# mythos-bio/mythos

Hardware: AMD Instinct MI355X
Metric: MD steps/sec (and ns/day) per GPU, oxDNA2 12 kbp duplex (higher is better)
Workload: dtype f32; 1 GPU; oxDNA2 12000 bp duplex (24000 nt), Debye-Hueckel salt 0.5, Langevin dt 0.005, free space, 1 replica/GPU; half_charged_ends=True, replicas=1, repeats=1, warmup_steps_done=10205, precision=headline f32 (north_star: fp32 at 1e-3); the other precision: --full, full=False

## Files before the change

### include/mythos_hip.h

```cpp
#ifndef MYTHOS_HIP_H
#define MYTHOS_HIP_H

#include <stdint.h>

#ifdef __cplusplus
extern "C" {
#endif

typedef struct mythos_system mythos_system_t;
typedef struct mythos_sim mythos_sim_t;
typedef struct mythos_martini mythos_martini_t;
typedef struct mythos_martini_sim mythos_martini_sim_t;
typedef struct mythos_obs mythos_obs_t;
typedef void* mythos_stream_t;

enum mythos_status {
  MYTHOS_OK = 0,
  MYTHOS_ERR_INVALID_ARGUMENT = -1,
  MYTHOS_ERR_HIP = -2,
  MYTHOS_ERR_NO_DEVICE = -3,
  MYTHOS_ERR_NOT_READY = -4,
  MYTHOS_ERR_OVERFLOW = -5,
  MYTHOS_ERR_NUMERIC = -6
};

enum mythos_dtype { MYTHOS_F32 = 0, MYTHOS_F64 = 1 };

#define MYTHOS_OXDNA_N_TERMS 8

const char* mythos_version(void);
const char* mythos_last_error(void);
int mythos_device_count(void);

int mythos_oxdna_param_count(void);
const char* mythos_oxdna_param_name(int index);

mythos_system_t* mythos_oxdna_create(int model, int n, const int32_t* seq, const uint8_t* is_end, int n_bonded,
                                     const int32_t* bonded, const double* box, int dtype, int device);
void mythos_oxdna_destroy(mythos_system_t* sys);

int mythos_oxdna_set_params(mythos_system_t* sys, const double* flat_params, int n_params);

int mythos_oxdna_set_nucleotide_types(mythos_system_t* sys, const uint8_t* is_rna);

int mythos_oxdna_set_pseq(mythos_system_t* sys, const double* marginals, const int32_t* unit, int n_bp,
                          const double* bp_probs, int terms);

int mythos_oxdna_energy_dpseq(mythos_system_t* sys, const void* center, const void* quat, int n_frames, double* e_terms,
                              void* dU_dcenter, void* dU_dquat, double* dU_dparams, double* dU_dmarginals, double* dU_dbp,
                              mythos_stream_t stream);

int mythos_oxdna_set_neighbors(mythos_system_t* sys, const int32_t* pairs, int n_pairs);

int mythos_oxdna_build_neighbors(mythos_system_t* sys, const void* center, double r_cut, double skin,
                                 mythos_stream_t stream);
int mythos_oxdna_neighbor_stats(mythos_system_t* sys, int* max_row, double* mean_row);

int mythos_oxdna_energy(mythos_system_t* sys, const void* center, const void* quat, int n_frames, double* e_terms,
                        void* dU_dcenter, void* dU_dquat, double* dU_dparams, mythos_stream_t stream);

mythos_obs_t* mythos_observables_create(int model, int n, const double* geometry, const double* box, int n_bp,
                                        const int32_t* base_pairs, int n_quartets, const int32_t* quartets, int skip_ends,
                                        int dtype, int device);
void mythos_observables_destroy(mythos_obs_t* obs);
int mythos_observables_width(const mythos_obs_t* obs);
int mythos_observables_eval(mythos_obs_t* obs, const void* center, const void* quat, int n_frames, double* out,
                            mythos_stream_t stream);
int mythos_oxdna_energy_obs(mythos_system_t* sys, const void* center, const void* quat, int n_frames, double* e_terms,
                            void* dU_dcenter, void* dU_dquat, double* dU_dparams, mythos_obs_t* obs, double* obs_out,
                            mythos_stream_t stream);

mythos_sim_t* mythos_langevin_create(mythos_system_t* sys, double dt, double kT, double gamma_t, double gamma_r,
                                     double mass, const double* inertia, uint64_t seed);
void mythos_langevin_destroy(mythos_sim_t* sim);

int mythos_langevin_set_neighbor_policy(mythos_sim_t* sim, double r_cut, double skin, int every);

int mythos_langevin_init_momenta(mythos_sim_t* sim, void* p_lin, void* p_ang, mythos_stream_t stream);

int mythos_langevin_run(mythos_sim_t* sim, void* center, void* quat, void* p_lin, void* p_ang, int n_steps,
                        int save_every, void* traj_center, void* traj_quat, double* e_trace,
                        mythos_stream_t stream);
int mythos_langevin_load(mythos_sim_t* sim, const void* center, const void* quat, const void* p_lin, const void* p_ang,
                         mythos_stream_t stream);
int mythos_langevin_advance(mythos_sim_t* sim, int n_steps, int save_every, void* traj_center, void* traj_quat,
                            double* e_trace, mythos_stream_t stream);
int mythos_langevin_store(mythos_sim_t* sim, void* center, void* quat, void* p_lin, void* p_ang, mythos_stream_t stream);

int64_t mythos_langevin_get_step(const mythos_sim_t* sim);
int mythos_langevin_set_step(mythos_sim_t* sim, int64_t step);
int mythos_langevin_set_seed(mythos_sim_t* sim, uint64_t seed);

enum mythos_langevin_option { MYTHOS_LANGEVIN_UNFUSED = 0 };
int mythos_langevin_set_option(mythos_sim_t* sim, int option, int64_t value);

int mythos_langevin_set_timing(mythos_sim_t* sim, int samples);
int mythos_langevin_last_kernel_ms(const mythos_sim_t* sim, double* kernel_ms, double* loop_ms_per_launch,
                                   int* launches, int* samples);

int mythos_langevin_last_recoveries(const mythos_sim_t* sim, int* recoveries);
int mythos_langevin_last_rebuilds(const mythos_sim_t* sim, int* scheduled);

int mythos_oxdna_read_trajectory(const char* path, int n, int max_frames, double* times, double* box, double* energies,
                                 double* frames, int* n_frames);

int mythos_oxdna_write_trajectory(const char* path, int n, int n_frames, const double* times, const double* box,
                                  const double* energies, const double* frames, int append);

enum mythos_debug_key {
  MYTHOS_DEBUG_CELL_BUCKET_CAP = 0,
  MYTHOS_DEBUG_ENERGY_LIST_CAP = 1,
  MYTHOS_DEBUG_MD_SEGMENT = 2,
  MYTHOS_DEBUG_MD_OVERFLOW_AT = 3,
  MYTHOS_DEBUG_MD_DENSE = 4,
  MYTHOS_DEBUG_MD_ITEMS_BIG = 5,
  MYTHOS_DEBUG_MD_LANES = 6,
  MYTHOS_DEBUG_KEYS = 7
};
int mythos_debug_set(int key, int64_t value);
int64_t mythos_debug_get(int key);

#define MYTHOS_MARTINI_N_TERMS 3
mythos_martini_t* mythos_martini_create(int n, const int32_t* types, int n_types, const double* sigma,
                                        const double* eps, int n_bonds, const int32_t* bonds, const double* bond_k,
                                        const double* bond_r0, int n_angles, const int32_t* angles,
                                        const double* angle_k, const double* angle_t0, int angle_kind, double r_cut,
                                        int dtype, int device);
void mythos_martini_destroy(mythos_martini_t* m);
int mythos_martini_energy(mythos_martini_t* m, const void* pos, const void* box, int n_frames, double* e_terms,
                          void* dU_dpos, mythos_stream_t stream);

int mythos_martini_param_grads(mythos_martini_t* m, const void* pos, const void* box, int n_frames, double* d_sigma,
                               double* d_eps, double* d_bond_k, double* d_bond_r0, double* d_angle_k,
                               double* d_angle_t0, mythos_stream_t stream);

mythos_martini_sim_t* mythos_martini_langevin_create(mythos_martini_t* sys, double dt, double kT, double gamma,
                                                     const double* mass, uint64_t seed);
void mythos_martini_langevin_destroy(mythos_martini_sim_t* sim);
int mythos_martini_langevin_set_neighbor_policy(mythos_martini_sim_t* sim, double skin, int rebuild_every);
int mythos_martini_langevin_set_inner_list(mythos_martini_sim_t* sim, double margin, int every);
int mythos_martini_langevin_init_velocities(mythos_martini_sim_t* sim, void* vel, mythos_stream_t stream);
int mythos_martini_langevin_run(mythos_martini_sim_t* sim, void* pos, void* vel, const double* box, int n_steps,
                                int save_every, void* traj_pos, double* e_trace, mythos_stream_t stream);
int mythos_martini_langevin_load(mythos_martini_sim_t* sim, const void* pos, const void* vel, const double* box,
                                 mythos_stream_t stream);
int mythos_martini_langevin_advance(mythos_martini_sim_t* sim, int n_steps, int save_every, void* traj_pos, double* e_trace,
                                    mythos_stream_t stream);
int mythos_martini_langevin_store(mythos_martini_sim_t* sim, void* pos, void* vel, mythos_stream_t stream);
int64_t mythos_martini_langevin_get_step(const mythos_martini_sim_t* sim);
int mythos_martini_langevin_last_rebuilds(const mythos_martini_sim_t* sim, int* scheduled);
int mythos_martini_langevin_last_kernel_ms(const mythos_martini_sim_t* sim, double* kernel_ms,
                                           double* loop_ms_per_launch, int* launches, int* samples);
int mythos_martini_langevin_set_timing(mythos_martini_sim_t* sim, int samples);
int mythos_martini_langevin_last_recoveries(const mythos_martini_sim_t* sim, int* recoveries);
int mythos_martini_langevin_neighbor_stats(const mythos_martini_sim_t* sim, int* max_row, double* mean_row);
int mythos_martini_langevin_get_rows(const mythos_martini_sim_t* sim, int which, int32_t* rows, int32_t* row_len, int* stride);

typedef struct mythos_martini_obs mythos_martini_obs_t;
mythos_martini_obs_t* mythos_martini_obs_create(int n, int n_groups, const int32_t* beads_per_item, const int32_t* members,
                                                const int32_t* index, int device);
void mythos_martini_obs_destroy(mythos_martini_obs_t* obs);
int64_t mythos_martini_obs_count(const mythos_martini_obs_t* obs);
int mythos_martini_obs_eval(mythos_martini_obs_t* obs, const void* pos, const void* box, int dtype, int n_frames, double* out,
                            mythos_stream_t stream);

typedef struct mythos_w1_plan mythos_w1_plan_t;
mythos_w1_plan_t* mythos_w1_plan_create(int n_groups, const int32_t* n_frames, const int32_t* members, const double* samples,
                                        const int64_t* n_ref, const double* ref, const double* ref_weights,
                                        const uint8_t* has_ref_weights, const int64_t* order, int device,
                                        mythos_stream_t stream);
void mythos_w1_plan_destroy(mythos_w1_plan_t* plan);
int mythos_w1_eval(mythos_w1_plan_t* plan, const double* weights, double* w1, double* dw1_dweights, mythos_stream_t stream);

#define MYTHOS_MEMBRANE_ROW 7
typedef struct mythos_membrane mythos_membrane_t;
mythos_membrane_t* mythos_membrane_create(int n, int n_lipids, const int32_t* lipid_start, const int32_t* lipid_beads, int n_thick,
                                          const int32_t* thick_beads, const int32_t* thick_lipid, int device);
void mythos_membrane_destroy(mythos_membrane_t* mem);
int mythos_membrane_n_lipids(const mythos_membrane_t* mem);
int mythos_membrane_eval(mythos_membrane_t* mem, const void* pos, const void* box, int dtype, int n_frames, double* out,
                         int8_t* leaflets, mythos_stream_t stream);

#ifdef __cplusplus
}
#endif
#endif
```

### mythos_amd/_lib.py

```python

from __future__ import annotations

import ctypes as C
import os
from pathlib import Path

_LIB_PATH = Path(__file__).resolve().parent / "lib" / "libmythos_hip.so"

c_int_p = C.POINTER(C.c_int32)
c_double_p = C.POINTER(C.c_double)
c_uint8_p = C.POINTER(C.c_uint8)


class MythosHipError(RuntimeError):
    """An error reported by libmythos_hip.so."""


_lib = None


def lib_path() -> Path:
    return Path(os.environ.get("MYTHOS_HIP_LIB", _LIB_PATH))


def load() -> C.CDLL:
    global _lib
    if _lib is not None:
        return _lib
    path = lib_path()
    if not path.exists():
        raise MythosHipError(
            f"{path} not found: the HIP extension is not built (run __graft_entry__.build()). "
            "mythos_amd has no CPU fallback."
        )
    lib = C.CDLL(str(path))
    V = C.c_void_p
    sigs = {
        "mythos_version": (C.c_char_p, []),
        "mythos_last_error": (C.c_char_p, []),
        "mythos_device_count": (C.c_int, []),
        "mythos_debug_set": (C.c_int, [C.c_int, C.c_int64]),
        "mythos_debug_get": (C.c_int64, [C.c_int]),
        "mythos_oxdna_param_count": (C.c_int, []),
        "mythos_oxdna_param_name": (C.c_char_p, [C.c_int]),
        "mythos_oxdna_create": (V, [C.c_int, C.c_int, c_int_p, c_uint8_p, C.c_int, c_int_p, c_double_p, C.c_int, C.c_int]),
        "mythos_oxdna_destroy": (None, [V]),
        "mythos_oxdna_set_params": (C.c_int, [V, c_double_p, C.c_int]),
        "mythos_oxdna_set_pseq": (C.c_int, [V, c_double_p, c_int_p, C.c_int, c_double_p, C.c_int]),
        "mythos_oxdna_set_nucleotide_types": (C.c_int, [V, c_uint8_p]),
        "mythos_oxdna_set_neighbors": (C.c_int, [V, c_int_p, C.c_int]),
        "mythos_oxdna_build_neighbors": (C.c_int, [V, V, C.c_double, C.c_double, V]),
        "mythos_oxdna_neighbor_stats": (C.c_int, [V, C.POINTER(C.c_int), c_double_p]),
        "mythos_oxdna_energy": (C.c_int, [V, V, V, C.c_int, V, V, V, V, V]),
        "mythos_oxdna_energy_obs": (C.c_int, [V, V, V, C.c_int, V, V, V, V, V, V, V]),
        "mythos_oxdna_energy_dpseq": (C.c_int, [V, V, V, C.c_int, V, V, V, V, V, V, V]),
        "mythos_observables_create": (V, [C.c_int, C.c_int, c_double_p, c_double_p, C.c_int, c_int_p, C.c_int, c_int_p, C.c_int, C.c_int, C.c_int]),
        "mythos_observables_destroy": (None, [V]),
        "mythos_observables_width": (C.c_int, [V]),
        "mythos_observables_eval": (C.c_int, [V, V, V, C.c_int, V, V]),
        "mythos_langevin_create": (V, [V, C.c_double, C.c_double, C.c_double, C.c_double, C.c_double, c_double_p, C.c_uint64]),
        "mythos_langevin_destroy": (None, [V]),
        "mythos_langevin_set_neighbor_policy": (C.c_int, [V, C.c_double, C.c_double, C.c_int]),
        "mythos_langevin_init_momenta": (C.c_int, [V, V, V, V]),
        "mythos_langevin_run": (C.c_int, [V, V, V, V, V, C.c_int, C.c_int, V, V, V, V]),
        "mythos_langevin_load": (C.c_int, [V, V, V, V, V, V]),
        "mythos_langevin_advance": (C.c_int, [V, C.c_int, C.c_int, V, V, V, V]),
        "mythos_langevin_store": (C.c_int, [V, V, V, V, V, V]),
        "mythos_langevin_get_step": (C.c_int64, [V]),
        "mythos_langevin_set_step": (C.c_int, [V, C.c_int64]),
        "mythos_langevin_set_seed": (C.c_int, [V, C.c_uint64]),
        "mythos_langevin_last_kernel_ms": (C.c_int, [V, c_double_p, c_double_p, C.POINTER(C.c_int), C.POINTER(C.c_int)]),
        "mythos_langevin_set_option": (C.c_int, [V, C.c_int, C.c_int64]),
        "mythos_langevin_set_timing": (C.c_int, [V, C.c_int]),
        "mythos_martini_langevin_set_timing": (C.c_int, [V, C.c_int]),
        "mythos_langevin_last_recoveries": (C.c_int, [V, C.POINTER(C.c_int)]),
        "mythos_langevin_last_rebuilds": (C.c_int, [V, C.POINTER(C.c_int)]),
        "mythos_oxdna_read_trajectory": (C.c_int, [C.c_char_p, C.c_int, C.c_int, c_double_p, c_double_p, c_double_p, c_double_p, C.POINTER(C.c_int)]),
        "mythos_oxdna_write_trajectory": (C.c_int, [C.c_char_p, C.c_int, C.c_int, c_double_p, c_double_p, c_double_p, c_double_p, C.c_int]),
        "mythos_martini_create": (
            V,
            [C.c_int, c_int_p, C.c_int, c_double_p, c_double_p, C.c_int, c_int_p, c_double_p, c_double_p, C.c_int,
             c_int_p, c_double_p, c_double_p, C.c_int, C.c_double, C.c_int, C.c_int],
        ),
        "mythos_martini_destroy": (None, [V]),
        "mythos_martini_energy": (C.c_int, [V, V, V, C.c_int, V, V, V]),
        "mythos_martini_param_grads": (C.c_int, [V, V, V, C.c_int, V, V, V, V, V, V, V]),
        "mythos_martini_langevin_create": (V, [V, C.c_double, C.c_double, C.c_double, c_double_p, C.c_uint64]),
        "mythos_martini_langevin_destroy": (None, [V]),
        "mythos_martini_langevin_set_neighbor_policy": (C.c_int, [V, C.c_double, C.c_int]),
        "mythos_martini_langevin_set_inner_list": (C.c_int, [V, C.c_double, C.c_int]),
        "mythos_martini_langevin_init_velocities": (C.c_int, [V, V, V]),
        "mythos_martini_langevin_run": (C.c_int, [V, V, V, c_double_p, C.c_int, C.c_int, V, V, V]),
        "mythos_martini_langevin_load": (C.c_int, [V, V, V, c_double_p, V]),
        "mythos_martini_langevin_advance": (C.c_int, [V, C.c_int, C.c_int, V, V, V]),
        "mythos_martini_langevin_store": (C.c_int, [V, V, V, V]),
        "mythos_martini_langevin_get_step": (C.c_int64, [V]),
        "mythos_martini_langevin_last_rebuilds": (C.c_int, [V, C.POINTER(C.c_int)]),
        "mythos_martini_langevin_last_kernel_ms": (C.c_int, [V, c_double_p, c_double_p, C.POINTER(C.c_int), C.POINTER(C.c_int)]),
        "mythos_martini_langevin_last_recoveries": (C.c_int, [V, C.POINTER(C.c_int)]),
        "mythos_martini_langevin_neighbor_stats": (C.c_int, [V, C.POINTER(C.c_int), c_double_p]),
        "mythos_martini_langevin_get_rows": (C.c_int, [V, C.c_int, C.POINTER(C.c_int32), C.POINTER(C.c_int32), C.POINTER(C.c_int)]),
        "mythos_martini_obs_create": (V, [C.c_int, C.c_int, c_int_p, c_int_p, c_int_p, C.c_int]),
        "mythos_martini_obs_destroy": (None, [V]),
        "mythos_martini_obs_count": (C.c_int64, [V]),
        "mythos_martini_obs_eval": (C.c_int, [V, V, V, C.c_int, C.c_int, V, V]),
        "mythos_w1_plan_create": (V, [C.c_int, c_int_p, c_int_p, V, C.POINTER(C.c_int64), V, V, c_uint8_p, V, C.c_int, V]),
        "mythos_w1_plan_destroy": (None, [V]),
        "mythos_w1_eval": (C.c_int, [V, V, V, V, V]),
        "mythos_membrane_create": (V, [C.c_int, C.c_int, c_int_p, c_int_p, C.c_int, c_int_p, c_int_p, C.c_int]),
        "mythos_membrane_destroy": (None, [V]),
        "mythos_membrane_n_lipids": (C.c_int, [V]),
        "mythos_membrane_eval": (C.c_int, [V, V, V, C.c_int, C.c_int, V, V, V]),
    }
    for name, (res, args) in sigs.items():
        fn = getattr(lib, name)
        fn.restype = res
        fn.argtypes = args
    _lib = lib
    return lib


DECLARED_SYMBOLS = (
    "mythos_version",
    "mythos_last_error",
    "mythos_device_count",
    "mythos_debug_set",
    "mythos_debug_get",
    "mythos_oxdna_param_count",
    "mythos_oxdna_param_name",
    "mythos_oxdna_create",
    "mythos_oxdna_destroy",
    "mythos_oxdna_set_params",
    "mythos_oxdna_set_pseq",
    "mythos_oxdna_set_nucleotide_types",
    "mythos_oxdna_set_neighbors",
    "mythos_oxdna_build_neighbors",
    "mythos_oxdna_neighbor_stats",
    "mythos_oxdna_energy",
    "mythos_oxdna_energy_obs",
    "mythos_oxdna_energy_dpseq",
    "mythos_observables_create",
    "mythos_observables_destroy",
    "mythos_observables_width",
    "mythos_observables_eval",
    "mythos_langevin_create",
    "mythos_langevin_destroy",
    "mythos_langevin_set_neighbor_policy",
    "mythos_langevin_init_momenta",
    "mythos_langevin_run",
    "mythos_langevin_load",
    "mythos_langevin_advance",
    "mythos_langevin_store",
    "mythos_langevin_get_step",
    "mythos_langevin_set_step",
    "mythos_langevin_set_seed",
    "mythos_langevin_last_kernel_ms",
    "mythos_langevin_last_recoveries",
    "mythos_langevin_last_rebuilds",
    "mythos_langevin_set_option",
    "mythos_langevin_set_timing",
    "mythos_martini_langevin_set_timing",
    "mythos_oxdna_read_trajectory",
    "mythos_oxdna_write_trajectory",
    "mythos_martini_create",
    "mythos_martini_destroy",
    "mythos_martini_energy",
    "mythos_martini_param_grads",
    "mythos_martini_langevin_create",
    "mythos_martini_langevin_destroy",
    "mythos_martini_langevin_set_neighbor_policy",
    "mythos_martini_langevin_set_inner_list",
    "mythos_martini_langevin_init_velocities",
    "mythos_martini_langevin_run",
    "mythos_martini_langevin_load",
    "mythos_martini_langevin_advance",
    "mythos_martini_langevin_store",
    "mythos_martini_langevin_get_step",
    "mythos_martini_langevin_last_rebuilds",
    "mythos_martini_langevin_last_kernel_ms",
    "mythos_martini_langevin_neighbor_stats",
    "mythos_martini_langevin_get_rows",
    "mythos_martini_langevin_last_recoveries",
    "mythos_martini_obs_create",
    "mythos_martini_obs_destroy",
    "mythos_martini_obs_count",
    "mythos_martini_obs_eval",
    "mythos_w1_plan_create",
    "mythos_w1_plan_destroy",
    "mythos_w1_eval",
    "mythos_membrane_create",
    "mythos_membrane_destroy",
    "mythos_membrane_n_lipids",
    "mythos_membrane_eval",
)


MEMBRANE_ROW = 7


def last_error() -> str:
    return load().mythos_last_error().decode()


def check(rc: int, what: str = "") -> None:
    if rc == 0:
        return
    msg = f"{what}: {last_error()} (status {rc})"
    if rc == -1:
        raise ValueError(msg)
    if rc == -6:
        raise FloatingPointError(msg)
    raise MythosHipError(msg)


DEBUG_KEYS = {"cell_bucket_cap": 0, "energy_list_cap": 1, "md_segment": 2, "md_overflow_at": 3, "md_dense": 4, "md_items_big": 5, "md_lanes": 6}


def debug_set(key: str, value: int) -> None:
    check(load().mythos_debug_set(DEBUG_KEYS[key], int(value)), f"debug_set({key})")


def debug_get(key: str) -> int:
    return int(load().mythos_debug_get(DEBUG_KEYS[key]))


_PARAM_NAMES: list[str] = []


def param_names() -> list[str]:
    if not _PARAM_NAMES:
        lib = load()
        _PARAM_NAMES.extend(lib.mythos_oxdna_param_name(i).decode() for i in range(lib.mythos_oxdna_param_count()))
    return list(_PARAM_NAMES)


def device_count() -> int:
    return int(load().mythos_device_count())


def ptr(t):
    if t is None:
        return None
    if hasattr(t, "data_ptr"):
        return C.c_void_p(t.data_ptr())
    return C.c_void_p(t.ctypes.data)
```

### mythos_amd/csrc/langevin.hip

```cpp
#include "langevin_core.inc"

MYTHOS_MD_DEFINE_PRECISION(float)

extern "C" {

mythos_sim_t* mythos_langevin_create(mythos_system_t* sys, double dt, double kT, double gamma_t, double gamma_r,
                                     double mass, const double* inertia, uint64_t seed) {
  if (!sys || !(dt > 0) || !(kT >= 0) || gamma_t < 0 || gamma_r < 0 || !(mass > 0)) {
    set_error("mythos_langevin_create: invalid argument");
    return nullptr;
  }
  if (hipSetDevice(sys->device) != hipSuccess) {
    set_error("mythos_langevin_create: hipSetDevice failed");
    return nullptr;
  }
  auto* s = new mythos_sim();
  s->sys = sys;
  s->dt = dt;
  s->kT = kT;
  s->gamma_t = gamma_t;
  s->gamma_r = gamma_r;
  s->mass = mass;
  for (int k = 0; k < 3; ++k) s->inertia[k] = inertia ? inertia[k] : 1.0;
  s->seed = seed;
  const size_t v4 = (sys->dtype == MYTHOS_F32 ? sizeof(float4) : sizeof(double4)) * (size_t)sys->n;
  bool ok = md_run_create(*s);
  for (int k = 0; k < 2; ++k)
    for (int a = 0; a < mythos_sim::kFrameArrays; ++a) ok = ok && hipMalloc(&s->frame[k][a], v4) == hipSuccess;
  ok = ok && hipMalloc(&s->keep_hi, v4) == hipSuccess && hipMalloc(&s->keep_lo, v4) == hipSuccess;
  ok = ok && hipMalloc((void**)&s->d_epart, (size_t)((sys->n + 15) / 16) * kTraceWidth * sizeof(double)) == hipSuccess;
  if (ok && !sys->d_ref_pos) ok = hipMalloc(&sys->d_ref_pos, v4) == hipSuccess;
  if (ok && !sys->d_ref_off) ok = hipMalloc(&sys->d_ref_off, v4) == hipSuccess;
  if (ok && !sys->d_ref_a1) ok = hipMalloc(&sys->d_ref_a1, v4) == hipSuccess;
  if (!ok) {
    set_error("mythos_langevin_create: device allocation failed");
    mythos_langevin_destroy(s);
    return nullptr;
  }
  return s;
}

void mythos_langevin_destroy(mythos_sim_t* s) {
  if (!s) return;
  for (int k = 0; k < 2; ++k)
    for (int a = 0; a < mythos_sim::kFrameArrays; ++a)
      if (s->frame[k][a]) (void)hipFree(s->frame[k][a]);
  for (void* u : {s->u_c, s->u_q, s->u_p, s->u_l, s->u_gc, s->u_gq, s->u_ref, (void*)s->u_e})
    if (u) (void)hipFree(u);
  if (s->keep_hi) (void)hipFree(s->keep_hi);
  if (s->keep_lo) (void)hipFree(s->keep_lo);
  if (s->d_chunk_order) (void)hipFree(s->d_chunk_order);
  if (s->d_chunk_keys) (void)hipFree(s->d_chunk_keys);
  if (s->d_epart) (void)hipFree(s->d_epart);
  md_run_destroy(*s);
  delete s;
}

int mythos_langevin_set_neighbor_policy(mythos_sim_t* s, double r_cut, double skin, int every) {
  if (!s || (every > 0 && (!(r_cut > 0) || !(skin > 0)))) {
    set_error("mythos_langevin_set_neighbor_policy: invalid argument");
    return MYTHOS_ERR_INVALID_ARGUMENT;
  }
  s->r_cut = r_cut;
  s->skin = skin;
  s->rebuild_every = every;
  s->list_fitted = false;
  s->list_valid = false;
  return MYTHOS_OK;
}

int mythos_langevin_init_momenta(mythos_sim_t* s, void* p_lin, void* p_ang, mythos_stream_t stream) {
  if (!s || !p_lin || !p_ang) {
    set_error("mythos_langevin_init_momenta: invalid argument");
    return MYTHOS_ERR_INVALID_ARGUMENT;
  }
  MYTHOS_HIP_TRY(hipSetDevice(s->sys->device));
  return s->sys->dtype == MYTHOS_F32 ? mythos_md_init_momenta<float>(s, p_lin, p_ang, (hipStream_t)stream)
                                     : mythos_md_init_momenta<double>(s, p_lin, p_ang, (hipStream_t)stream);
}

namespace {

int md_ready_state(mythos_sim_t* s, const char* who) {
  mythos_system* sys = s->sys;
  if (!sys->params_set) {
    set_error(std::string(who) + ": parameters must be set first");
    return MYTHOS_ERR_NOT_READY;
  }
  if (sys->model == 4 && !sys->types_set) {
    set_error(std::string(who) + ": an oxNA system needs its nucleotide types (mythos_oxdna_set_nucleotide_types)");
    return MYTHOS_ERR_NOT_READY;
  }
  MYTHOS_HIP_TRY(hipSetDevice(sys->device));
  return MYTHOS_OK;
}

int md_ready(mythos_sim_t* s, const char* who) {
  mythos_system* sys = s->sys;
  if (int rc = md_ready_state(s, who)) return rc;
  if (!sys->nbrs_set && s->rebuild_every <= 0) {
    set_error(std::string(who) + ": parameters and neighbours (or a neighbour policy) must be set first");
    return MYTHOS_ERR_NOT_READY;
  }
  if (s->rebuild_every > 0 && sys->list.stride == 0)
    if (int rc = rows_reserve(sys->list, sys->n, 64)) return rc;
  if (s->list_epoch != sys->list_epoch) {
    s->list_valid = false;
    s->list_epoch = sys->list_epoch;
  }
  return MYTHOS_OK;
}


int md_load(mythos_sim_t* s, void* c, void* q, void* p, void* l, hipStream_t st) {
  s->unfused = s->want_unfused && s->sys->model == 4;
  return s->sys->dtype == MYTHOS_F32 ? mythos_md_load<float>(s, c, q, p, l, st) : mythos_md_load<double>(s, c, q, p, l, st);
}

int md_advance(mythos_sim_t* s, int n_steps, int save_every, bool close, void* tc, void* tq, double* e_trace, hipStream_t st) {
  const size_t q_align = s->sys->dtype == MYTHOS_F32 ? sizeof(float4) : sizeof(double4);
  if (save_every > 0 && tq && (reinterpret_cast<uintptr_t>(tq) % q_align) != 0) {
    set_error("mythos_langevin_run / advance: traj_quat must be aligned to 4 elements (" + std::to_string(q_align) + " bytes)");
    return MYTHOS_ERR_INVALID_ARGUMENT;
  }
  return s->sys->dtype == MYTHOS_F32 ? mythos_md_advance<float>(s, n_steps, save_every, close, tc, tq, e_trace, st)
                                     : mythos_md_advance<double>(s, n_steps, save_every, close, tc, tq, e_trace, st);
}

int md_store(mythos_sim_t* s, void* c, void* q, void* p, void* l, hipStream_t st) {
  return s->sys->dtype == MYTHOS_F32 ? mythos_md_store<float>(s, c, q, p, l, st) : mythos_md_store<double>(s, c, q, p, l, st);
}

}

int mythos_langevin_run(mythos_sim_t* s, void* center, void* quat, void* p_lin, void* p_ang, int n_steps,
                        int save_every, void* traj_center, void* traj_quat, double* e_trace,
                        mythos_stream_t stream) {
  if (!s || !center || !quat || !p_lin || !p_ang || n_steps < 0 || save_every < 0) {
    set_error("mythos_langevin_run: invalid argument");
    return MYTHOS_ERR_INVALID_ARGUMENT;
  }
  if (int rc = md_ready(s, "mythos_langevin_run")) return rc;
  hipStream_t st = (hipStream_t)stream;
  if (int rc = md_load(s, center, quat, p_lin, p_ang, st)) return rc;
  const int rc = md_advance(s, n_steps, save_every, true, traj_center, traj_quat, e_trace, st);
  if (int rs = md_store(s, center, quat, p_lin, p_ang, st)) return rc ? rc : rs;
  return rc;
}

int mythos_langevin_load(mythos_sim_t* s, const void* center, const void* quat, const void* p_lin, const void* p_ang,
                         mythos_stream_t stream) {
  if (!s || !center || !quat || !p_lin || !p_ang) {
    set_error("mythos_langevin_load: invalid argument");
    return MYTHOS_ERR_INVALID_ARGUMENT;
  }
  if (int rc = md_ready_state(s, "mythos_langevin_load")) return rc;
  return md_load(s, (void*)center, (void*)quat, (void*)p_lin, (void*)p_ang, (hipStream_t)stream);
}

int mythos_langevin_advance(mythos_sim_t* s, int n_steps, int save_every, void* traj_center, void* traj_quat,
                            double* e_trace, mythos_stream_t stream) {
  if (!s || n_steps < 0 || save_every < 0) {
    set_error("mythos_langevin_advance: invalid argument");
    return MYTHOS_ERR_INVALID_ARGUMENT;
  }
  if (!s->resident) {
    set_error("mythos_langevin_advance: no resident state (call mythos_langevin_load first; a run that ended in a numeric "
              "error drops its state)");
    return MYTHOS_ERR_NOT_READY;
  }
  if (int rc = md_ready(s, "mythos_langevin_advance")) return rc;
  return md_advance(s, n_steps, save_every, false, traj_center, traj_quat, e_trace, (hipStream_t)stream);
}

int mythos_langevin_store(mythos_sim_t* s, void* center, void* quat, void* p_lin, void* p_ang, mythos_stream_t stream) {
  if (!s || !center || !quat || !p_lin || !p_ang) {
    set_error("mythos_langevin_store: invalid argument");
    return MYTHOS_ERR_INVALID_ARGUMENT;
  }
  if (!s->resident) {
    set_error("mythos_langevin_store: no resident state");
    return MYTHOS_ERR_NOT_READY;
  }
  if (s->open) {
    if (int rc = md_ready(s, "mythos_langevin_store")) return rc;
  } else {
    MYTHOS_HIP_TRY(hipSetDevice(s->sys->device));
  }
  return md_store(s, center, quat, p_lin, p_ang, (hipStream_t)stream);
}

int64_t mythos_langevin_get_step(const mythos_sim_t* s) { return md_get_step(s); }

int mythos_langevin_set_step(mythos_sim_t* s, int64_t step) {
  if (!s || step < 0) {
    set_error("mythos_langevin_set_step: invalid argument");
    return MYTHOS_ERR_INVALID_ARGUMENT;
  }
  s->step = step;
  return MYTHOS_OK;
}

int mythos_langevin_set_seed(mythos_sim_t* s, uint64_t seed) {
  if (!s) {
    set_error("mythos_langevin_set_seed: invalid argument");
    return MYTHOS_ERR_INVALID_ARGUMENT;
  }
  s->seed = seed;
  return MYTHOS_OK;
}

int mythos_langevin_last_kernel_ms(const mythos_sim_t* s, double* kernel_ms, double* loop_ms_per_launch,
                                   int* launches, int* samples) {
  return md_last_kernel_ms(s, kernel_ms, loop_ms_per_launch, launches, samples, "mythos_langevin_last_kernel_ms");
}

int mythos_langevin_last_recoveries(const mythos_sim_t* s, int* recoveries) {
  return md_last_count(s, &MdRun::last_recoveries, recoveries, "mythos_langevin_last_recoveries");
}

int mythos_langevin_last_rebuilds(const mythos_sim_t* s, int* scheduled) {
  return md_last_count(s, &MdRun::last_rebuilds, scheduled, "mythos_langevin_last_rebuilds");
}

int mythos_langevin_set_option(mythos_sim_t* s, int option, int64_t value) {
  if (!s || option != MYTHOS_LANGEVIN_UNFUSED || (value != 0 && value != 1)) {
    set_error("mythos_langevin_set_option: invalid argument");
    return MYTHOS_ERR_INVALID_ARGUMENT;
  }
  if (value == 1 && s->sys->model != 4) {
    set_error("mythos_langevin_set_option: the unfused path exists for oxNA systems (model 4) only");
    return MYTHOS_ERR_INVALID_ARGUMENT;
  }
  s->want_unfused = value == 1;
  return MYTHOS_OK;
}

int mythos_langevin_set_timing(mythos_sim_t* s, int samples) { return md_set_timing(s, samples, "mythos_langevin_set_timing"); }

}
```

### mythos_amd/csrc/langevin_core.inc

```
#include <algorithm>
#include <cmath>
#include <type_traits>

#include <hip/hip_ext.h>

#ifndef MYTHOS_LEAN_MATH
#define MYTHOS_LEAN_MATH 1
#endif

#include "cell_list.h"
#include "chunk_order.h"
#include "md_driver.h"
#include "oxdna_gather.h"
#include "philox.h"

namespace mythos {

template <typename R>
struct LangevinConst {
  R dt, half_dt;
  R inv_mass;
  R inv_inertia[3];
  R c1_t, c2_t;
  R c1_r, c2_r[3];
// ... 651 lines not shown
  MD_PRIO(3);

  SelfGrad<R> sg;
  sg.dc = sg.g1 = sg.g2 = sg.g3 = V3<R>{R(0), R(0), R(0)};
  const int fw = kPooled ? (int)(threadIdx.x >> 6) : 0;
  const int rb = kPooled ? row_base[fw][grp] : 0;
  const bool pool_ok = !kPooled || row_base[fw][PPB] <= kPool;
  const int n_bonded_fold = extra_bonds ? ROW_BONDED_SLOTS : 2;
  if (valid && pool_ok) {
    const int total = kPooled ? row_base[fw][grp + 1] - rb : n_bonded_fold + item_cnt[0][grp] + item_cnt[1][grp];
    for (int u = lane; u < total; u += G) {
      const R* rr = kPooled ? pool_row(rb + u) : fixed_row(grp, u);
      sg.dc = sg.dc + V3<R>{rr[0], rr[1], rr[2]};
      sg.g1 = sg.g1 + V3<R>{rr[3], rr[4], rr[5]};
      sg.g2 = sg.g2 + V3<R>{rr[6], rr[7], rr[8]};
      sg.g3 = sg.g3 + V3<R>{rr[9], rr[10], rr[11]};
      if constexpr (SAVE) {
#pragma unroll
        for (int k = 0; k < T_COUNT; ++k) e[k] += rr[12 + k];
      }
    }
  }
  if (lane == 0) {
    const R* rl = rad_lds[grp];
    const V3<R> rbk{rl[0], rl[1], rl[2]}, rba{rl[3], rl[4], rl[5]};
    sg.dc = sg.dc - (rbk + rba);
    if constexpr (MODEL == 4) {
      const bool r = self.rna != 0;
      axpy(sg.g1, -(r ? Prna[GEO_BACK_A1] : P[GEO_BACK_A1]), rbk);
      axpy(sg.g1, -(r ? Prna[GEO_BASE] : P[GEO_BASE]), rba);
      axpy(sg.g2, r ? R(0) : -P[GEO_BACK_A2], rbk);
      axpy(sg.g3, r ? -Prna[GEO_BACK_A2] : R(0), rbk);
    } else {
    axpy(sg.g1, -P[GEO_BACK_A1], rbk);
    axpy(sg.g1, -P[GEO_BASE], rba);
    if constexpr (MODEL == 2) axpy(sg.g2, -P[GEO_BACK_A2], rbk);
    if constexpr (MODEL == 3) axpy(sg.g3, -P[GEO_BACK_A2], rbk);
    }
  }
  if constexpr (SAVE) {
    group_reduce<G, R, true>(e, sg);
  } else {
    group_reduce_v3<G>(sg.dc);
    group_reduce_v3<G>(sg.g1);
    group_reduce_v3<G>(sg.g2);
    group_reduce_v3<G>(sg.g3);
  }

  if (lane == 0) {
    Nuc<R> own;
    const R* ms = self_lds[grp];
    own.a1 = V3<R>{ms[3], ms[4], ms[5]};
    own.a3 = V3<R>{ms[6], ms[7], ms[8]};
    own.a2 = cross(own.a3, own.a1);
    const V3<R> tl = axes_grad_to_torque(own, sg);
    R* fr = kPooled ? pool_row(pool_ok ? rb : grp * 2) : fixed_row(grp, 0);
    fr[0] = -sg.dc.x, fr[1] = -sg.dc.y, fr[2] = -sg.dc.z;
    fr[3] = dot(own.a1, tl), fr[4] = dot(own.a2, tl), fr[5] = dot(own.a3, tl);
  }
  __syncthreads();
  MD_PRIO(4);
  double ke_t = 0.0, ke_r = 0.0;
  if (integrates) {
    const int i = i_int;
    Nuc<R> self;
    {
      const R* ms = self_lds[il];
      self.c = V3<R>{ms[0], ms[1], ms[2]};
      self.a1 = V3<R>{ms[3], ms[4], ms[5]};
      self.a3 = V3<R>{ms[6], ms[7], ms[8]};
      self.a2 = cross(self.a3, self.a1);
    }
    const R* fr = kPooled ? pool_row(row_base[fw][PPB] <= kPool ? row_base[fw][il] : il * 2) : fixed_row(il, 0);
    const V3<R> F{fr[0], fr[1], fr[2]};
    const R tb[3] = {fr[3], fr[4], fr[5]};
    const bool int_rna = (MODEL == 4) && ((((int)self_lds[il][9]) >> 3) & 1);
    const R g_k1 = int_rna ? Prna[GEO_BACK_A1] : P[GEO_BACK_A1];
    const R g_k2 = (MODEL >= 2) ? (int_rna ? Prna[GEO_BACK_A2] : P[GEO_BACK_A2]) : R(0);
    R p[3] = {pm.x, pm.y, pm.z}, L[3] = {lm.x, lm.y, lm.z};
    R qs[4] = {qv.x, qv.y, qv.z, qv.w};
    const R kc = kick_close * K.dt;
    p[0] += kc * F.x;
    p[1] += kc * F.y;
    p[2] += kc * F.z;
    L[0] += kc * tb[0];
    L[1] += kc * tb[1];
    L[2] += kc * tb[2];
    if constexpr (SAVE) {
      ke_t = 0.5 * double(K.inv_mass) * (double(p[0]) * p[0] + double(p[1]) * p[1] + double(p[2]) * p[2]);
      ke_r = 0.5 * (double(K.inv_inertia[0]) * L[0] * L[0] + double(K.inv_inertia[1]) * L[1] * L[1] +
                    double(K.inv_inertia[2]) * L[2] * L[2]);
      if (traj_c) {
        traj_c[3 * i + 0] = self.c.x;
        traj_c[3 * i + 1] = self.c.y;
        traj_c[3 * i + 2] = self.c.z;
      }
      if (traj_q) {
        traj_q[4 * i + 0] = qs[0];
        traj_q[4 * i + 1] = qs[1];
        traj_q[4 * i + 2] = qs[2];
        traj_q[4 * i + 3] = qs[3];
      }
    }
    R x[3] = {self.c.x, self.c.y, self.c.z};
    R xl[3] = {self_lds[il][10], self_lds[il][11], self_lds[il][12]};
    R dxa[3] = {R(0), R(0), R(0)};
    R* const xd = kHiLo<R> ? dxa : x;
    V3<R> n1 = self.a1, n2 = self.a2, n3 = self.a3;
    const bool bk3 = MODEL == 3 || int_rna;
    V3<R> nbk{bk3 ? n3.x : n2.x, bk3 ? n3.y : n2.y, bk3 ? n3.z : n2.z};
    if (do_step) {
      p[0] += K.half_dt * F.x;
      p[1] += K.half_dt * F.y;
      p[2] += K.half_dt * F.z;
      L[0] += K.half_dt * tb[0];
      L[1] += K.half_dt * tb[1];
      L[2] += K.half_dt * tb[2];
      drift(xd, qs, p, L, K.half_dt, K);
      p[0] = K.c1_t * p[0] + K.c2_t * z[0];
      p[1] = K.c1_t * p[1] + K.c2_t * z[1];
      p[2] = K.c1_t * p[2] + K.c2_t * z[2];
      L[0] = K.c1_r * L[0] + K.c2_r[0] * z[3];
      L[1] = K.c1_r * L[1] + K.c2_r[1] * z[4];
      L[2] = K.c1_r * L[2] + K.c2_r[2] * z[5];
      drift(xd, qs, p, L, K.half_dt, K);
      if constexpr (kHiLo<R>) {
#pragma unroll
        for (int k = 0; k < 3; ++k) {
          const R sdl = xl[k] + dxa[k];
          const R t = x[k] + sdl;
          xl[k] = sdl - (t - x[k]);
          x[k] = t;
        }
      }
      const R inv = m_rsqrt(qs[0] * qs[0] + qs[1] * qs[1] + qs[2] * qs[2] + qs[3] * qs[3]);
      qs[0] *= inv;
      qs[1] *= inv;
      qs[2] *= inv;
      qs[3] *= inv;
      if (!(x[0] == x[0]) || !(qs[0] == qs[0])) atomicOr(flags, 2);
      quat_axes(qs[0], qs[1], qs[2], qs[3], n1, n2, n3);
      nbk = V3<R>{bk3 ? n3.x : n2.x, bk3 ? n3.y : n2.y, bk3 ? n3.z : n2.z};
      if (K.skin_half_sq > R(0)) {
        const R dx = x[0] - r0.x, dy = x[1] - r0.y, dz = x[2] - r0.z;
        const R bx = dx + (g_k1 * n1.x + g_k2 * nbk.x - f0.x), by = dy + (g_k1 * n1.y + g_k2 * nbk.y - f0.y),
                bz = dz + (g_k1 * n1.z + g_k2 * nbk.z - f0.z);
        const R gb = int_rna ? Prna[GEO_BASE] : P[GEO_BASE];
        const R sx = dx + gb * (n1.x - a0.x), sy = dy + gb * (n1.y - a0.y), sz = dz + gb * (n1.z - a0.z);
        if (dx * dx + dy * dy + dz * dz > K.skin_half_sq || bx * bx + by * by + bz * bz > K.skin_half_sq ||
            sx * sx + sy * sy + sz * sz > K.skin_half_sq)
          atomicMax(flags + 1, k_index + 1);
      }
    }
    if constexpr (!SAVE) {
      if (traj_c) {
        traj_c[3 * i + 0] = x[0];
        traj_c[3 * i + 1] = x[1];
        traj_c[3 * i + 2] = x[2];
      }
      if (traj_q) reinterpret_cast<V4*>(traj_q)[i] = V4{qs[0], qs[1], qs[2], qs[3]};
    }
    out.p0[i] = V4{x[0], x[1], x[2], self_lds[il][9]};
    if constexpr (kHiLo<R>) out.pl[i] = V4{xl[0], xl[1], xl[2], R(0)};
    out.p1[i] = V4{n1.x, n1.y, n1.z, R(0)};
    out.p2[i] = V4{n3.x, n3.y, n3.z, R(0)};
    out.p3[i] = do_step ? V4{g_k1 * n1.x + g_k2 * nbk.x, g_k1 * n1.y + g_k2 * nbk.y, g_k1 * n1.z + g_k2 * nbk.z, R(0)} : in.p3[i];
    out.q[i] = V4{qs[0], qs[1], qs[2], qs[3]};
    out.mom[i] = V4{p[0], p[1], p[2], R(0)};
    out.ang[i] = V4{L[0], L[1], L[2], R(0)};
  }
  if constexpr (SAVE) {
    if (lane == 0) {
#pragma unroll
      for (int k = 0; k < T_COUNT; ++k) e_lds[grp][k] = valid ? double(e[k]) : 0.0;
    }
    if ((int)(threadIdx.x >> 6) == int_wave && il < PPB) {
      e_lds[il][T_COUNT] = ke_t;
      e_lds[il][T_COUNT + 1] = ke_r;
    }
    __syncthreads();
    if (threadIdx.x < kTraceWidth) {
      double s = 0.0;
      for (int g = 0; g < PPB; ++g) s += e_lds[g][threadIdx.x];
      e_part[(size_t)bid * kTraceWidth + threadIdx.x] = s;
    }
  }
}

template <typename R, int BX>
__global__ void pack_state_kernel(int n, R g_k1, R g_k2, R r_k1, R r_k2, const R* __restrict__ c, const R* __restrict__ q,
                                  const R* __restrict__ p, const R* __restrict__ l, const int* __restrict__ meta,
                                  const Frame<R> f, const R* __restrict__ keep_hi, const R* __restrict__ keep_lo) {
  using V4 = typename Vec4T<R>::type;
  const int i = blockIdx.x * blockDim.x + threadIdx.x;
  if (i >= n) return;
  if constexpr (kHiLo<R>) {
    R lo[3] = {R(0), R(0), R(0)};
    if (keep_hi) {
#pragma unroll
      for (int k = 0; k < 3; ++k)
        if (c[3 * i + k] == keep_hi[3 * i + k]) lo[k] = keep_lo[3 * i + k];
    }
    f.pl[i] = V4{lo[0], lo[1], lo[2], R(0)};
  }
  R q0 = q[4 * i], q1 = q[4 * i + 1], q2 = q[4 * i + 2], q3 = q[4 * i + 3];
  const R inv = m_rsqrt(q0 * q0 + q1 * q1 + q2 * q2 + q3 * q3);
  q0 *= inv, q1 *= inv, q2 *= inv, q3 *= inv;
  V3<R> a1, a2, a3;
  quat_axes(q0, q1, q2, q3, a1, a2, a3);
  f.p0[i] = V4{c[3 * i], c[3 * i + 1], c[3 * i + 2], R(meta[i])};
  f.p1[i] = V4{a1.x, a1.y, a1.z, R(0)};
  f.p2[i] = V4{a3.x, a3.y, a3.z, R(0)};
  const bool rna = BX == 0 && ((meta[i] >> 3) & 1);
  const V3<R> ab = (BX == 3 || rna) ? a3 : a2;
  const R k1 = rna ? r_k1 : g_k1, k2 = rna ? r_k2 : g_k2;
  f.p3[i] = V4{k1 * a1.x + k2 * ab.x, k1 * a1.y + k2 * ab.y, k1 * a1.z + k2 * ab.z, R(0)};
  f.q[i] = V4{q0, q1, q2, q3};
  f.mom[i] = V4{p[3 * i], p[3 * i + 1], p[3 * i + 2], R(0)};
  f.ang[i] = V4{l[3 * i], l[3 * i + 1], l[3 * i + 2], R(0)};
}
template <typename R>
__global__ void unpack_state_kernel(int n, const Frame<R> f, R* __restrict__ c, R* __restrict__ q,
                                    R* __restrict__ p, R* __restrict__ l, R* __restrict__ keep_hi,
                                    R* __restrict__ keep_lo) {
  const int i = blockIdx.x * blockDim.x + threadIdx.x;
  if (i >= n) return;
  const auto a = f.p0[i];
  if constexpr (kHiLo<R>) {
    const auto lo = f.pl[i];
    keep_hi[3 * i] = a.x, keep_hi[3 * i + 1] = a.y, keep_hi[3 * i + 2] = a.z;
    keep_lo[3 * i] = lo.x, keep_lo[3 * i + 1] = lo.y, keep_lo[3 * i + 2] = lo.z;
  }
  const auto b = f.q[i];
  const auto m = f.mom[i];
  const auto w = f.ang[i];
  c[3 * i] = a.x, c[3 * i + 1] = a.y, c[3 * i + 2] = a.z;
  q[4 * i] = b.x, q[4 * i + 1] = b.y, q[4 * i + 2] = b.z, q[4 * i + 3] = b.w;
  p[3 * i] = m.x, p[3 * i + 1] = m.y, p[3 * i + 2] = m.z;
  l[3 * i] = w.x, l[3 * i + 1] = w.y, l[3 * i + 2] = w.z;
}

template <typename R, int BX>
__global__ void rederive_frame_kernel(int n, R g_k1, R g_k2, R r_k1, R r_k2, const int* __restrict__ meta, const Frame<R> f) {
  using V4 = typename Vec4T<R>::type;
  const int i = blockIdx.x * blockDim.x + threadIdx.x;
  if (i >= n) return;
  const V4 q = f.q[i];
  V3<R> a1, a2, a3;
  quat_axes(q.x, q.y, q.z, q.w, a1, a2, a3);
  V4 c = f.p0[i];
  c.w = R(meta[i]);
  f.p0[i] = c;
  const bool rna = BX == 0 && ((meta[i] >> 3) & 1);
  const V3<R> ab = (BX == 3 || rna) ? a3 : a2;
  const R k1 = rna ? r_k1 : g_k1, k2 = rna ? r_k2 : g_k2;
  f.p3[i] = V4{k1 * a1.x + k2 * ab.x, k1 * a1.y + k2 * ab.y, k1 * a1.z + k2 * ab.z, R(0)};
}

template <typename R>
__global__ void init_momenta_kernel(int n, R sd_t, R sd_r0, R sd_r1, R sd_r2, uint64_t seed, R* __restrict__ p,
                                    R* __restrict__ l) {
  __shared__ double sum[3][256];
  double s0 = 0, s1 = 0, s2 = 0;
  for (int i = threadIdx.x; i < n; i += blockDim.x) {
    R z[6];
    normals6(seed, (uint32_t)i, 0xFFFFFFFFFFFFFFFFull, 7u, z);
    p[3 * i] = sd_t * z[0], p[3 * i + 1] = sd_t * z[1], p[3 * i + 2] = sd_t * z[2];
    l[3 * i] = sd_r0 * z[3], l[3 * i + 1] = sd_r1 * z[4], l[3 * i + 2] = sd_r2 * z[5];
    s0 += p[3 * i], s1 += p[3 * i + 1], s2 += p[3 * i + 2];
  }
  sum[0][threadIdx.x] = s0, sum[1][threadIdx.x] = s1, sum[2][threadIdx.x] = s2;
  __syncthreads();
  for (int o = blockDim.x / 2; o > 0; o >>= 1) {
    if ((int)threadIdx.x < o)
      for (int k = 0; k < 3; ++k) sum[k][threadIdx.x] += sum[k][threadIdx.x + o];
    __syncthreads();
  }
  const R m0 = R(sum[0][0] / n), m1 = R(sum[1][0] / n), m2 = R(sum[2][0] / n);
  for (int i = threadIdx.x; i < n; i += blockDim.x) {
    p[3 * i] -= m0, p[3 * i + 1] -= m1, p[3 * i + 2] -= m2;
  }
}

}

using namespace mythos;

struct mythos_sim : mythos::MdRun {
  mythos_system* sys = nullptr;
  double dt = 0, kT = 0, gamma_t = 0, gamma_r = 0, mass = 1, inertia[3] = {1, 1, 1};
  double r_cut = 0, skin = 0;
  static constexpr int kFrameArrays = 8;
  void* frame[2][kFrameArrays] = {};
  int builds = 0;
  int list_epoch = 0;
  void *keep_hi = nullptr, *keep_lo = nullptr;
  bool keep_valid = false;
  bool items_big = false;
  bool want_unfused = false;
  bool unfused = false;
  int param_epoch = 0;
  int lanes = kMdG;
  int chunk_cap = 0;
  int* d_chunk_order = nullptr;
  unsigned long long* d_chunk_keys = nullptr;
  double* d_epart = nullptr;
  void *u_c = nullptr, *u_q = nullptr, *u_p = nullptr, *u_l = nullptr, *u_gc = nullptr, *u_gq = nullptr, *u_ref = nullptr;
  double* u_e = nullptr;
  bool u_forces_valid = false;
};

namespace mythos {

template <typename R>
static LangevinConst<R> make_const(const mythos_sim* s) {
  LangevinConst<R> K;
  K.dt = R(s->dt);
  K.half_dt = R(0.5 * s->dt);
  K.inv_mass = R(1.0 / s->mass);
  const double c1t = std::exp(-s->gamma_t * s->dt), c1r = std::exp(-s->gamma_r * s->dt);
  K.c1_t = R(c1t);
  K.c2_t = R(std::sqrt(s->kT * (1.0 - c1t * c1t) * s->mass));
  K.c1_r = R(c1r);
  for (int k = 0; k < 3; ++k) {
    K.inv_inertia[k] = R(1.0 / s->inertia[k]);
    K.c2_r[k] = R(std::sqrt(s->kT * (1.0 - c1r * c1r) * s->inertia[k]));
  }
  K.skin_half_sq = R(s->rebuild_every > 0 ? 0.25 * s->skin * s->skin : -1.0);
  return K;
}

template <typename R>
static MdCut<R> make_cut(const mythos_system* sys) {
  const OxParams<double>& P = sys->pd;
  double rbb = oxdna_param_max(sys, NEXC_BACKBONE_RC);
  if (sys->model >= 2) rbb = std::max(rbb, oxdna_param_max(sys, DH_RCUT));
  const double rcom = oxdna_close_range(sys);
  MdCut<R> c;
  c.rbb2 = R(rbb * rbb);
  c.rcom2 = R(rcom * rcom);
  auto sq = [](double v) { return R(v * v); };
  c.hb_lo2 = sq(P[HYDR_RCLOW]), c.hb_hi2 = sq(P[HYDR_RCHIGH]);
  c.cr_lo2 = sq(P[CRST_RCLOW]), c.cr_hi2 = sq(P[CRST_RCHIGH]);
  c.cx_lo2 = sq(P[CXST_RCLOW]), c.cx_hi2 = sq(P[CXST_RCHIGH]);
  c.hb_mask = 0;
  for (int k = 0; k < 16; ++k)
    if (P[HYDR_EPS_00 + k] != 0.0) c.hb_mask |= 1u << k;
  return c;
}

template <typename R>
static Frame<R> frame_of(const mythos_sim* sim, int k) {
  using V4 = typename Vec4T<R>::type;
  return Frame<R>{(V4*)sim->frame[k][0], (V4*)sim->frame[k][1], (V4*)sim->frame[k][2], (V4*)sim->frame[k][3],
                  (V4*)sim->frame[k][4], (V4*)sim->frame[k][5], (V4*)sim->frame[k][6], (V4*)sim->frame[k][7]};
}

template <typename R>
static int update_chunk_order(mythos_sim* sim, const typename Vec4T<R>::type* p0, int blocks, hipStream_t st) {
  if (blocks < 64) {
    if (sim->d_chunk_order) (void)hipFree(sim->d_chunk_order), sim->d_chunk_order = nullptr;
    if (sim->d_chunk_keys) (void)hipFree(sim->d_chunk_keys), sim->d_chunk_keys = nullptr;
    sim->chunk_cap = 0;
    return 0;
  }
  if (blocks > sim->chunk_cap) {
    if (sim->d_chunk_order) (void)hipFree(sim->d_chunk_order), sim->d_chunk_order = nullptr;
    if (sim->d_chunk_keys) (void)hipFree(sim->d_chunk_keys), sim->d_chunk_keys = nullptr;
    sim->chunk_cap = 0;
    MYTHOS_HIP_TRY(hipMalloc((void**)&sim->d_chunk_keys, (size_t)blocks * sizeof(unsigned long long)));
    MYTHOS_HIP_TRY(hipMalloc((void**)&sim->d_chunk_order, (size_t)blocks * sizeof(int)));
    sim->chunk_cap = blocks;
  }
  MYTHOS_HIP_TRY(chunk_order_device(p0, blocks, kMdBlock / sim->lanes, std::max(1.0, sim->r_cut > 0 ? sim->r_cut : 4.0), sim->d_chunk_keys,
                                    sim->d_chunk_order, st));
  return 0;
}

static int md_lanes_for(const mythos_system* sys) {
  const long long dbg = debug_value(MYTHOS_DEBUG_MD_LANES);
  if (dbg == 8 || dbg == 16) return (int)dbg;
  int cus = 256;
  (void)hipDeviceGetAttribute(&cus, hipDeviceAttributeMultiprocessorCount, sys->device);
  const int grid16 = (sys->n + 15) / 16;
  return 2 * grid16 <= 3 * cus ? 16 : 8;
}

template <typename R, int MODEL>
static int load_typed(mythos_sim* sim, const R* center, const R* quat, const R* p_lin, const R* p_ang, hipStream_t st) {
  mythos_system* sys = sim->sys;
  const int n = sys->n;
  const int tb = (n + 255) / 256;
  const OxParams<R>& P = params_of<R>(sys);
  const R g_k1 = P[GEO_BACK_A1], g_k2 = (MODEL >= 2) ? P[GEO_BACK_A2] : R(0);
  sim->cur = 0;
  const Frame<R> f0 = frame_of<R>(sim, 0);
  const double* Prna = oxdna_param_set(sys, sys->param_sets() == 1 ? 0 : 1);
  hipLaunchKernelGGL((pack_state_kernel<R, (MODEL == 4 ? 0 : back_axis<MODEL>())>), dim3(tb), dim3(256), 0, st, n, g_k1, g_k2,
                     R(Prna[GEO_BACK_A1]), R(Prna[GEO_BACK_A2]), center, quat, p_lin, p_ang,
                     sys->d_meta, f0, sim->keep_valid ? (const R*)sim->keep_hi : nullptr,
                     (const R*)sim->keep_lo);
  MYTHOS_HIP_TRY(hipGetLastError());
  sim->resident = true;
  sim->list_valid = false;
  sim->since_build = 0;
  sim->items_big = false;
  sim->open = false;
  sim->param_epoch = sys->param_epoch;
  sim->lanes = md_lanes_for(sys);
  const int ppb = kMdBlock / sim->lanes;
  return update_chunk_order<R>(sim, f0.p0, (n + ppb - 1) / ppb, st);
}

template <typename R>
static int unpack_typed(mythos_sim* sim, R* center, R* quat, R* p_lin, R* p_ang, hipStream_t st) {
  const int n = sim->sys->n;
  hipLaunchKernelGGL(unpack_state_kernel<R>, dim3((n + 255) / 256), dim3(256), 0, st, n, frame_of<R>(sim, sim->cur),
                     center, quat, p_lin, p_ang, (R*)sim->keep_hi, (R*)sim->keep_lo);
  MYTHOS_HIP_TRY(hipGetLastError());
  sim->keep_valid = true;
  return 0;
}

template <typename R, int MODEL>
static int advance_typed(mythos_sim* sim, int n_steps, int save_every, bool close, R* traj_center, R* traj_quat, double* e_trace,
                         hipStream_t st) {
  using V4 = typename Vec4T<R>::type;
  mythos_system* sys = sim->sys;
  const int n = sys->n;
  const bool lanes16 = sim->lanes == 16;
  const int ppb = kMdBlock / sim->lanes;
  const int blocks = (n + ppb - 1) / ppb;
  const int grid = 8 * ((blocks + 7) / 8);
  int sim_cus = 256;
  (void)hipDeviceGetAttribute(&sim_cus, hipDeviceAttributeMultiprocessorCount, sys->device);
  const long long dbg_dense = debug_value(MYTHOS_DEBUG_MD_DENSE);
  const bool dense_grid = !lanes16 && (dbg_dense == 1 || (dbg_dense != 2 && grid > 4 * sim_cus));
  const int prio_on = (sizeof(R) == 8 && grid > 3 * sim_cus) ? 0 : 1;
  const R* Pdev = device_params_of<R>(sys);
  const BoxT<R> box = make_box<R>(sys);
  const LangevinConst<R> K = make_const<R>(sim);
  const MdCut<R> cut = make_cut<R>(sys);
  const Frame<R> fr[2] = {frame_of<R>(sim, 0), frame_of<R>(sim, 1)};
  if (sim->param_epoch != sys->param_epoch) {
    const OxParams<R>& Ph = params_of<R>(sys);
    const double* Prna = oxdna_param_set(sys, sys->param_sets() == 1 ? 0 : 1);
    hipLaunchKernelGGL((rederive_frame_kernel<R, (MODEL == 4 ? 0 : back_axis<MODEL>())>), dim3((n + 255) / 256), dim3(256), 0, st, n,
                       Ph[GEO_BACK_A1], (MODEL >= 2) ? Ph[GEO_BACK_A2] : R(0), R(Prna[GEO_BACK_A1]), R(Prna[GEO_BACK_A2]),
                       (const int*)sys->d_meta, fr[sim->cur]);
    MYTHOS_HIP_TRY(hipGetLastError());
    sim->param_epoch = sys->param_epoch;
  }
  const bool dynamic_list = sim->rebuild_every > 0;
  PseqView<R> pseq;
  const bool use_pseq = sys->pseq_terms != 0;
  if (debug_value(MYTHOS_DEBUG_MD_ITEMS_BIG) == 1) sim->items_big = true;
  if (use_pseq) pseq.marg = (const R*)sys->d_ps_marg, pseq.unit = sys->d_ps_unit, pseq.bp = (const R*)sys->d_ps_bp, pseq.terms = sys->pseq_terms;
  int* halt_words = dynamic_list ? sys->list.d_overflow : nullptr;
  auto launch_step = [&](int k, const LaunchRow& row) {
    const int cur = row.cur;
    const bool save = row.save;
    const R kick_close = R(row.kick_close);
    R* tc = ((save || row.save_next) && traj_center) ? traj_center + (size_t)row.sidx * n * 3 : nullptr;
    R* tq = ((save || row.save_next) && traj_quat) ? traj_quat + (size_t)row.sidx * n * 4 : nullptr;
    const V4* ref = (const V4*)sys->d_ref_pos;
    const V4* ref_off = (const V4*)sys->d_ref_off;
    const V4* ref_a1 = (const V4*)sys->d_ref_a1;
    auto launch_pseq = [&](auto save_tag, auto items_tag, hipEvent_t ea, hipEvent_t eb) {
      constexpr bool SV = decltype(save_tag)::value;
      constexpr int IT = decltype(items_tag)::value;
      auto go = [&](auto lanes_tag) {
        hipExtLaunchKernelGGL((md_step_kernel<R, MODEL, SV, IT, true, false, decltype(lanes_tag)::value>), dim3(grid), dim3(kMdBlock), 0, st, ea, eb, 0,
                              Pdev, box, K, cut, n, fr[cur], fr[cur ^ 1], sys->list.d_rows, sys->d_row_len, row_close_of(sys),
                              sys->list.stride, sys->extra_bonds ? 1 : 0, kick_close, row.do_step, sim->seed, (uint64_t)(sim->step + k), ref,
                              ref_off, ref_a1, sim->d_flags, tc, tq, sim->d_epart, sim->d_chunk_order, halt_words, k, 0, prio_on, pseq);
      };
      if (lanes16) go(std::integral_constant<int, 16>{}); else go(std::integral_constant<int, 8>{});
    };
    auto launch = [&](auto save_tag, auto items_tag, hipEvent_t ea, hipEvent_t eb) {
      constexpr bool SV = decltype(save_tag)::value;
      constexpr int IT = decltype(items_tag)::value;
      auto go = [&](auto dense_tag, auto lanes_tag) {
        hipExtLaunchKernelGGL((md_step_kernel<R, MODEL, SV, IT, false, decltype(dense_tag)::value, decltype(lanes_tag)::value>), dim3(grid), dim3(kMdBlock), 0, st, ea, eb, 0,
                              Pdev, box, K, cut, n, fr[cur], fr[cur ^ 1], sys->list.d_rows, sys->d_row_len, row_close_of(sys),
                              sys->list.stride, sys->extra_bonds ? 1 : 0, kick_close, row.do_step, sim->seed, (uint64_t)(sim->step + k), ref,
                              ref_off, ref_a1, sim->d_flags, tc, tq, sim->d_epart, sim->d_chunk_order, halt_words, k, 0, prio_on, PseqView<R>{});
      };
      using L8 = std::integral_constant<int, 8>;
      using L16 = std::integral_constant<int, 16>;
      if (lanes16) {
        go(std::false_type{}, L16{});
      } else if constexpr (sizeof(R) == 4 && !SV && IT == kMdItems && MODEL <= 2) {
        if (dense_grid) go(std::true_type{}, L8{}); else go(std::false_type{}, L8{});
      } else {
        go(std::false_type{}, L8{});
      }
    };
    using T = std::true_type;
    using F = std::false_type;
    using Small = std::integral_constant<int, kMdItems>;
    using BigS = std::integral_constant<int, md_items_big<R, true>()>;
    using BigN = std::integral_constant<int, md_items_big<R, false>()>;
    const hipEvent_t ea = row.ea, eb = row.eb;
    if (use_pseq) {
      if (save) {
        if (sim->items_big) launch_pseq(T{}, BigS{}, ea, eb); else launch_pseq(T{}, Small{}, ea, eb);
      } else {
        if (sim->items_big) launch_pseq(F{}, BigN{}, ea, eb); else launch_pseq(F{}, Small{}, ea, eb);
      }
    } else if (save) {
      if (sim->items_big) launch(T{}, BigS{}, ea, eb); else launch(T{}, Small{}, ea, eb);
    } else {
      if (sim->items_big) launch(F{}, BigN{}, ea, eb); else launch(F{}, Small{}, ea, eb);
    }
    if (save)
      hipLaunchKernelGGL(reduce_trace_kernel<kTraceWidth>, dim3(1), dim3(256), 0, st, sim->d_epart, blocks,
                         e_trace + (size_t)row.sidx * kTraceWidth);
  };
  auto rebuild = [&](int buf) -> int {
    if ((++sim->builds & 63) == 0)
      if (int rc = update_chunk_order<R>(sim, fr[buf].p0, blocks, st)) return rc;
    return rows_build_device(sys, fr[buf].p0, true, sim->r_cut, sim->skin, fr[buf].p3, fr[buf].p1, true, st);
  };
  auto rebuild_until_fit = [&](int buf) -> int {
    return rows_build_until_fit(sys, fr[buf].p0, true, sim->r_cut, sim->skin, fr[buf].p3, fr[buf].p1, true, true, st);
  };
  auto on_abort = [&]() -> int {
    if (!sim->items_big) {
      sim->items_big = true;
      return 0;
    }
    set_error("mythos_langevin_run: more than " + std::to_string(md_items_big<R, false>()) + " (" + std::to_string(md_items_big<R, true>()) +
              " on steps that save energies)"
              " neighbours of one nucleotide are inside the range of an angular term (overlapping bases?)");
    return MYTHOS_ERR_OVERFLOW;
  };
  MdDrive d;
  d.who = "mythos_langevin_run";
  d.n_steps = n_steps, d.save_every = save_every, d.close = close;
  d.energy_rows = save_every > 0 && e_trace != nullptr;
  d.plain_rows = save_every > 0 && e_trace == nullptr && (traj_center != nullptr || traj_quat != nullptr);
  d.dynamic_list = dynamic_list;
  d.halt_words = halt_words;
  d.row_stride = &sys->list.stride;
  d.skin = sim->skin;
  d.st = st;
  return md_drive(*sim, d, launch_step, rebuild, rebuild_until_fit, on_abort);
}

template <typename R>
__global__ void unfused_integrate_kernel(int n, const LangevinConst<R> K, R* __restrict__ c, R* __restrict__ q, R* __restrict__ p,
                                         R* __restrict__ L, const R* __restrict__ gc, const R* __restrict__ gq, R kick_close,
                                         int do_step, uint64_t seed, uint64_t step, const R* __restrict__ ref, R site_reach,
                                         int* __restrict__ flags, R* __restrict__ traj_c, R* __restrict__ traj_q,
                                         double* __restrict__ ke ) {
  const int i = blockIdx.x * blockDim.x + threadIdx.x;
  double ke_t = 0.0, ke_r = 0.0;
  if (i < n) {
    R x[3] = {c[3 * i], c[3 * i + 1], c[3 * i + 2]};
    R qs[4] = {q[4 * i], q[4 * i + 1], q[4 * i + 2], q[4 * i + 3]};
    R pp[3] = {p[3 * i], p[3 * i + 1], p[3 * i + 2]}, LL[3] = {L[3 * i], L[3 * i + 1], L[3 * i + 2]};
    const R F[3] = {-gc[3 * i], -gc[3 * i + 1], -gc[3 * i + 2]};
    const R g0 = gq[4 * i], g1 = gq[4 * i + 1], g2 = gq[4 * i + 2], g3 = gq[4 * i + 3];
    const R tb[3] = {R(-0.5) * (-qs[1] * g0 + qs[0] * g1 + qs[3] * g2 - qs[2] * g3),
                     R(-0.5) * (-qs[2] * g0 - qs[3] * g1 + qs[0] * g2 + qs[1] * g3),
                     R(-0.5) * (-qs[3] * g0 + qs[2] * g1 - qs[1] * g2 + qs[0] * g3)};
    const R kc = kick_close * K.dt;
#pragma unroll
    for (int k = 0; k < 3; ++k) pp[k] += kc * F[k], LL[k] += kc * tb[k];
    if (ke) {
      ke_t = 0.5 * double(K.inv_mass) * (double(pp[0]) * pp[0] + double(pp[1]) * pp[1] + double(pp[2]) * pp[2]);
      ke_r = 0.5 * (double(K.inv_inertia[0]) * LL[0] * LL[0] + double(K.inv_inertia[1]) * LL[1] * LL[1] +
                    double(K.inv_inertia[2]) * LL[2] * LL[2]);
    }
    if (traj_c) traj_c[3 * i] = x[0], traj_c[3 * i + 1] = x[1], traj_c[3 * i + 2] = x[2];
    if (traj_q) traj_q[4 * i] = qs[0], traj_q[4 * i + 1] = qs[1], traj_q[4 * i + 2] = qs[2], traj_q[4 * i + 3] = qs[3];
    if (do_step) {
      R z[6];
      normals6(seed, (uint32_t)i, step, 0u, z);
#pragma unroll
      for (int k = 0; k < 3; ++k) pp[k] += K.half_dt * F[k], LL[k] += K.half_dt * tb[k];
      drift(x, qs, pp, LL, K.half_dt, K);
#pragma unroll
      for (int k = 0; k < 3; ++k) pp[k] = K.c1_t * pp[k] + K.c2_t * z[k], LL[k] = K.c1_r * LL[k] + K.c2_r[k] * z[3 + k];
      drift(x, qs, pp, LL, K.half_dt, K);
      const R inv = m_rsqrt(qs[0] * qs[0] + qs[1] * qs[1] + qs[2] * qs[2] + qs[3] * qs[3]);
#pragma unroll
      for (int k = 0; k < 4; ++k) qs[k] *= inv;
      if (!(x[0] == x[0]) || !(qs[0] == qs[0])) atomicOr(flags, 2);
      if (ref != nullptr) {
        V3<R> a1, a2, a3;
        quat_axes(qs[0], qs[1], qs[2], qs[3], a1, a2, a3);
        const R* rr = ref + 12 * (size_t)i;
        const V3<R> dx{x[0] - rr[0], x[1] - rr[1], x[2] - rr[2]};
        const V3<R> d1{a1.x - rr[3], a1.y - rr[4], a1.z - rr[5]}, d2{a2.x - rr[6], a2.y - rr[7], a2.z - rr[8]},
            d3{a3.x - rr[9], a3.y - rr[10], a3.z - rr[11]};
        const R da = m_sqrt(fmax(dot(d1, d1), fmax(dot(d2, d2), dot(d3, d3))));
        const R moved = m_sqrt(dot(dx, dx)) + site_reach * da;
        if (moved * moved > K.skin_half_sq) atomicOr(flags + 1, 1);
      }
      c[3 * i] = x[0], c[3 * i + 1] = x[1], c[3 * i + 2] = x[2];
      q[4 * i] = qs[0], q[4 * i + 1] = qs[1], q[4 * i + 2] = qs[2], q[4 * i + 3] = qs[3];
    }
    p[3 * i] = pp[0], p[3 * i + 1] = pp[1], p[3 * i + 2] = pp[2];
    L[3 * i] = LL[0], L[3 * i + 1] = LL[1], L[3 * i + 2] = LL[2];
  }
  if (ke) {
    for (int o = 32; o > 0; o >>= 1) ke_t += __shfl_down(ke_t, o, 64), ke_r += __shfl_down(ke_r, o, 64);
    if ((threadIdx.x & 63) == 0) atomicAdd(ke, ke_t), atomicAdd(ke + 1, ke_r);
  }
}

template <typename R>
__global__ void unfused_ref_kernel(int n, const R* __restrict__ c, const R* __restrict__ q, R* __restrict__ ref) {
  const int i = blockIdx.x * blockDim.x + threadIdx.x;
  if (i >= n) return;
  V3<R> a1, a2, a3;
  quat_axes(q[4 * i], q[4 * i + 1], q[4 * i + 2], q[4 * i + 3], a1, a2, a3);
  R* rr = ref + 12 * (size_t)i;
  rr[0] = c[3 * i], rr[1] = c[3 * i + 1], rr[2] = c[3 * i + 2];
  rr[3] = a1.x, rr[4] = a1.y, rr[5] = a1.z, rr[6] = a2.x, rr[7] = a2.y, rr[8] = a2.z, rr[9] = a3.x, rr[10] = a3.y, rr[11] = a3.z;
}

static __global__ void unfused_trace_kernel(const double* __restrict__ e, double* __restrict__ row) {
  if (threadIdx.x < kTraceWidth) row[threadIdx.x] = e[threadIdx.x];
}

template <typename R>
static int unfused_alloc(mythos_sim* sim) {
  if (sim->u_c) return 0;
  const size_t n = (size_t)sim->sys->n;
  MYTHOS_HIP_TRY(hipMalloc(&sim->u_c, 3 * n * sizeof(R)));
  MYTHOS_HIP_TRY(hipMalloc(&sim->u_q, 4 * n * sizeof(R)));
  MYTHOS_HIP_TRY(hipMalloc(&sim->u_p, 3 * n * sizeof(R)));
  MYTHOS_HIP_TRY(hipMalloc(&sim->u_l, 3 * n * sizeof(R)));
  MYTHOS_HIP_TRY(hipMalloc(&sim->u_gc, 3 * n * sizeof(R)));
  MYTHOS_HIP_TRY(hipMalloc(&sim->u_gq, 4 * n * sizeof(R)));
  MYTHOS_HIP_TRY(hipMalloc(&sim->u_ref, 12 * n * sizeof(R)));
  MYTHOS_HIP_TRY(hipMalloc((void**)&sim->u_e, kTraceWidth * sizeof(double)));
  return 0;
}

template <typename R>
static int unfused_load(mythos_sim* sim, const R* c, const R* q, const R* p, const R* l, hipStream_t st) {
  if (int rc = unfused_alloc<R>(sim)) return rc;
  const size_t n = (size_t)sim->sys->n;
  MYTHOS_HIP_TRY(hipMemcpyAsync(sim->u_c, c, 3 * n * sizeof(R), hipMemcpyDeviceToDevice, st));
  MYTHOS_HIP_TRY(hipMemcpyAsync(sim->u_q, q, 4 * n * sizeof(R), hipMemcpyDeviceToDevice, st));
  MYTHOS_HIP_TRY(hipMemcpyAsync(sim->u_p, p, 3 * n * sizeof(R), hipMemcpyDeviceToDevice, st));
  MYTHOS_HIP_TRY(hipMemcpyAsync(sim->u_l, l, 3 * n * sizeof(R), hipMemcpyDeviceToDevice, st));
  sim->resident = true;
  sim->list_valid = false;
  sim->since_build = 0;
  sim->u_forces_valid = false;
  return 0;
}

template <typename R>
static int unfused_store(mythos_sim* sim, R* c, R* q, R* p, R* l, hipStream_t st) {
  const size_t n = (size_t)sim->sys->n;
  MYTHOS_HIP_TRY(hipMemcpyAsync(c, sim->u_c, 3 * n * sizeof(R), hipMemcpyDeviceToDevice, st));
  MYTHOS_HIP_TRY(hipMemcpyAsync(q, sim->u_q, 4 * n * sizeof(R), hipMemcpyDeviceToDevice, st));
  MYTHOS_HIP_TRY(hipMemcpyAsync(p, sim->u_p, 3 * n * sizeof(R), hipMemcpyDeviceToDevice, st));
  MYTHOS_HIP_TRY(hipMemcpyAsync(l, sim->u_l, 3 * n * sizeof(R), hipMemcpyDeviceToDevice, st));
  return 0;
}

template <typename R>
static int unfused_advance(mythos_sim* sim, int n_steps, int save_every, R* traj_c, R* traj_q, double* e_trace, hipStream_t st) {
  mythos_system* sys = sim->sys;
  const int n = sys->n, tb = (n + 255) / 256;
  const LangevinConst<R> K = make_const<R>(sim);
  R *c = (R*)sim->u_c, *q = (R*)sim->u_q, *p = (R*)sim->u_p, *l = (R*)sim->u_l, *gc = (R*)sim->u_gc, *gq = (R*)sim->u_gq;
  R* ref = (R*)sim->u_ref;
  const bool dynamic = sim->rebuild_every > 0;
  sim->last_recoveries = 0;
  double reach = 0.0;
  for (int k = 0; k < 2; ++k) {
    const double* P = sys->pd_sets.data() + (size_t)k * OXP_COUNT;
    reach = std::max({reach, std::fabs(P[GEO_BACK_A1]) + std::fabs(P[GEO_BACK_A2]), std::fabs(P[GEO_BASE]), std::fabs(P[GEO_STACK]),
                      std::fabs(P[GEO_STACK3_A1]) + std::fabs(P[GEO_STACK3_A2]), std::fabs(P[GEO_STACK5_A1]) + std::fabs(P[GEO_STACK5_A2])});
  }
  auto build = [&]() -> int {
    if (int rc = rows_build_until_fit(sys, c, false, sim->r_cut, sim->skin, nullptr, nullptr, false, true, st)) return rc;
    hipLaunchKernelGGL(unfused_ref_kernel<R>, dim3(tb), dim3(256), 0, st, n, (const R*)c, (const R*)q, ref);
    sim->since_build = 0;
    sim->list_valid = true;
    sim->list_epoch = ++sys->list_epoch;
    return 0;
  };
  auto forces = [&]() -> int {
    return oxdna_energy_launch(sys, c, q, 1, sim->u_e, gc, gq, nullptr, nullptr, nullptr, st);
  };
  auto check_flags = [&](const char* when) -> int {
    int fl[2] = {0, 0};
    MYTHOS_HIP_TRY(hipMemcpyAsync(fl, sim->d_flags, sizeof(fl), hipMemcpyDeviceToHost, st));
    MYTHOS_HIP_TRY(hipStreamSynchronize(st));
    MYTHOS_HIP_TRY(hipMemsetAsync(sim->d_flags, 0, 2 * sizeof(int), st));
    if (fl[0] & 2) {
      sim->resident = false;
      set_error(std::string("mythos_langevin_run (oxNA, unfused): NaN in the state ") + when);
      return MYTHOS_ERR_NUMERIC;
    }
    if (fl[1] != 0) {
      sim->resident = false;
      set_error("mythos_langevin_run (oxNA, unfused): a site moved more than skin / 2 between two list rebuilds; shorten "
                "rebuild_every or widen the skin (this path does not halt and resume)");
      return MYTHOS_ERR_OVERFLOW;
    }
    return 0;
  };
  MYTHOS_HIP_TRY(hipMemsetAsync(sim->d_flags, 0, mythos_sim::kCtlWords * sizeof(int), st));
  if (!sim->list_valid) sim->u_forces_valid = false;
  if (dynamic && !sim->list_valid)
    if (int rc = build()) return rc;
  if (!sim->u_forces_valid) {
    if (int rc = forces()) return rc;
    sim->u_forces_valid = true;
  }
  int saved = 0;
  for (int k = 0; k <= n_steps; ++k) {
    const bool do_step = k < n_steps;
    const bool save = save_every > 0 && k > 0 && k % save_every == 0;
    if (k == 0 && !do_step) break;
    R* tc = (save && traj_c) ? traj_c + (size_t)saved * n * 3 : nullptr;
    R* tq = (save && traj_q) ? traj_q + (size_t)saved * n * 4 : nullptr;
    double* ke = save ? sim->u_e + T_COUNT : nullptr;
    if (save) MYTHOS_HIP_TRY(hipMemsetAsync(sim->u_e + T_COUNT, 0, 2 * sizeof(double), st));
    hipLaunchKernelGGL(unfused_integrate_kernel<R>, dim3(tb), dim3(256), 0, st, n, K, c, q, p, l, (const R*)gc, (const R*)gq,
                       R(k > 0 ? 0.5 : 0.0), do_step ? 1 : 0, sim->seed, (uint64_t)(sim->step + k), dynamic ? (const R*)ref : nullptr,
                       R(reach), sim->d_flags, tc, tq, ke);
    if (save) {
      if (e_trace) hipLaunchKernelGGL(unfused_trace_kernel, dim3(1), dim3(64), 0, st, (const double*)sim->u_e, e_trace + (size_t)saved * kTraceWidth);
      ++saved;
    }
    if (!do_step) break;
    ++sim->since_build;
    if (dynamic && sim->since_build >= sim->rebuild_every) {
      if (int rc = check_flags("before a list rebuild")) return rc;
      if (int rc = build()) return rc;
    }
    if (int rc = forces()) return rc;
  }
  MYTHOS_HIP_TRY(hipGetLastError());
  if (int rc = check_flags("at the end of the run")) return rc;
  sim->step += n_steps;
  return 0;
}

}


template <typename R>
int mythos_md_load(mythos_sim* s, void* c, void* q, void* p, void* l, hipStream_t st);
template <typename R>
int mythos_md_advance(mythos_sim* s, int n_steps, int save_every, bool close, void* tc, void* tq, double* e_trace, hipStream_t st);
template <typename R>
int mythos_md_store(mythos_sim* s, void* c, void* q, void* p, void* l, hipStream_t st);
template <typename R>
int mythos_md_init_momenta(mythos_sim* s, void* p_lin, void* p_ang, hipStream_t st);

#define MYTHOS_MD_DEFINE_PRECISION(R)                                                                                        \
  template <>                                                                                                                 \
  int mythos_md_load<R>(mythos_sim * s, void* c, void* q, void* p, void* l, hipStream_t st) {                                  \
    mythos_system* sys = s->sys;                                                                                              \
    if (s->unfused) return mythos::unfused_load<R>(s, (R*)c, (R*)q, (R*)p, (R*)l, st);                                        \
    return sys->model == 1   ? mythos::load_typed<R, 1>(s, (R*)c, (R*)q, (R*)p, (R*)l, st)                                   \
           : sys->model == 2 ? mythos::load_typed<R, 2>(s, (R*)c, (R*)q, (R*)p, (R*)l, st)                                   \
           : sys->model == 3 ? mythos::load_typed<R, 3>(s, (R*)c, (R*)q, (R*)p, (R*)l, st)                                   \
                             : mythos::load_typed<R, 4>(s, (R*)c, (R*)q, (R*)p, (R*)l, st);                                  \
  }                                                                                                                           \
  template <>                                                                                                                 \
  int mythos_md_advance<R>(mythos_sim * s, int n_steps, int save_every, bool close, void* tc, void* tq, double* e_trace,      \
                           hipStream_t st) {                                                                                  \
    mythos_system* sys = s->sys;                                                                                              \
    if (s->unfused) return mythos::unfused_advance<R>(s, n_steps, save_every, (R*)tc, (R*)tq, e_trace, st);                   \
    return sys->model == 1   ? mythos::advance_typed<R, 1>(s, n_steps, save_every, close, (R*)tc, (R*)tq, e_trace, st)        \
           : sys->model == 2 ? mythos::advance_typed<R, 2>(s, n_steps, save_every, close, (R*)tc, (R*)tq, e_trace, st)        \
           : sys->model == 3 ? mythos::advance_typed<R, 3>(s, n_steps, save_every, close, (R*)tc, (R*)tq, e_trace, st)        \
                             : mythos::advance_typed<R, 4>(s, n_steps, save_every, close, (R*)tc, (R*)tq, e_trace, st);       \
  }                                                                                                                           \
  template <>                                                                                                                 \
  int mythos_md_store<R>(mythos_sim * s, void* c, void* q, void* p, void* l, hipStream_t st) {                                 \
    if (s->unfused) return mythos::unfused_store<R>(s, (R*)c, (R*)q, (R*)p, (R*)l, st);                                       \
         \
         \
    const int rc = s->open ? mythos_md_advance<R>(s, 0, 0, true, nullptr, nullptr, nullptr, st) : MYTHOS_OK;                   \
    const int ru = mythos::unpack_typed<R>(s, (R*)c, (R*)q, (R*)p, (R*)l, st);                                                \
    return rc ? rc : ru;                                                                                                      \
  }                                                                                                                           \
  template <>                                                                                                                 \
  int mythos_md_init_momenta<R>(mythos_sim * s, void* p_lin, void* p_ang, hipStream_t st) {                                    \
    const double sd_t = std::sqrt(s->mass * s->kT);                                                                           \
    double sd_r[3];                                                                                                           \
    for (int k = 0; k < 3; ++k) sd_r[k] = std::sqrt(s->inertia[k] * s->kT);                                                   \
    hipLaunchKernelGGL(mythos::init_momenta_kernel<R>, dim3(1), dim3(256), 0, st, s->sys->n, R(sd_t), R(sd_r[0]), R(sd_r[1]), \
                       R(sd_r[2]), s->seed, (R*)p_lin, (R*)p_ang);                                                            \
    MYTHOS_HIP_TRY(hipGetLastError());                                                                                        \
    return MYTHOS_OK;                                                                                                         \
  }
```

### mythos_amd/csrc/martini_md.hip

```cpp
#include <algorithm>
#include <cmath>
#include <string>
#include <vector>

#include <hip/hip_ext.h>

#include "cell_list.h"
#include "martini_internal.h"
#include "md_driver.h"
#include "philox.h"
#include "wave_ops.h"

namespace mythos {

#ifndef MYTHOS_MM_BLOCK
#define MYTHOS_MM_BLOCK 256
#endif
constexpr int kMmBlock = MYTHOS_MM_BLOCK;
#ifndef MYTHOS_MM_G
#define MYTHOS_MM_G 16
#endif
#ifndef MYTHOS_MM_BATCH
#define MYTHOS_MM_BATCH 4
#endif
// ... 300 lines not shown

template <typename R>
__device__ __forceinline__ bool mm_excluded(const int* __restrict__ ex, int j) {
  bool hit = false;
#pragma unroll
  for (int q = 0; q < kMaxExcl; ++q) hit = hit || (ex[q] == j);
  return hit;
}

#ifndef MYTHOS_MM_ROW_G
#define MYTHOS_MM_ROW_G 16
#endif
constexpr int kMmRowG = MYTHOS_MM_ROW_G;

template <typename R, int G>
__global__ __launch_bounds__(256) void mm_build_rows_cells_kernel(
    int n, const typename Real4<R>::type* __restrict__ pos, const MmConst<R> K, const CellGrid<R> g, R rl2,
    const int* __restrict__ excl, const int* __restrict__ cell_cnt,
    const typename CellPlace<R>::type* __restrict__ place, int cell_cap, const int* __restrict__ spill, int cell_H,
    int* __restrict__ rows, int* __restrict__ row_len, int row_stride, int* __restrict__ overflow,
    typename Real4<R>::type* __restrict__ ref_pos) {
  constexpr int NG = 256 / G;
  __shared__ int s_pre[NG][29], s_st[NG][28], s_c[NG][28][3];
  const int grp = threadIdx.x / G, l = threadIdx.x % G;
  const int gshift = (threadIdx.x & 63) & ~(G - 1);
  const int i = blockIdx.x * NG + grp;
  if (i >= n) return;
  const auto pi = pos[i];
  const int total = cell_candidates<R, G>(g, pi.x, pi.y, pi.z, cell_cnt, cell_cap, cell_H, s_pre[grp], s_st[grp], s_c[grp], l);
  int ex[kMaxExcl];
#pragma unroll
  for (int q = 0; q < kMaxExcl; ++q) ex[q] = excl[(size_t)i * kMaxExcl + q];
  int ex_lo = 0x7fffffff, ex_hi = -1;
#pragma unroll
  for (int q = 0; q < kMaxExcl; ++q)
    if (ex[q] >= 0) ex_lo = min(ex_lo, ex[q]), ex_hi = max(ex_hi, ex[q]);
  int* row = rows + (size_t)i * row_stride;
  constexpr unsigned int kGroupMask = (G == 32) ? 0xffffffffu : ((1u << G) - 1u);
  const unsigned int below = (1u << l) - 1u;
  int out = 0;
  int lo = 0;
  const int n_direct = s_pre[grp][27];
#ifndef MYTHOS_MM_SWEEPS
#define MYTHOS_MM_SWEEPS 4
#endif
  constexpr int kSweeps = MYTHOS_MM_SWEEPS;
  for (int t0 = 0; t0 < total; t0 += kSweeps * G) {
    typename CellPlace<R>::type pj[kSweeps];
    int cell[kSweeps], tcs[kSweeps];
#pragma unroll
    for (int u = 0; u < kSweeps; ++u) {
      const int t = t0 + u * G + l;
      const int tc = t < total ? t : total - 1;
      while (s_pre[grp][lo + 1] <= tc) ++lo;
      cell[u] = lo;
      tcs[u] = tc;
      pj[u] = place[tc < n_direct ? s_st[grp][lo] + (tc - s_pre[grp][lo]) : 0];
    }
#pragma unroll
    for (int u = 0; u < kSweeps; ++u) {
      const int t = t0 + u * G + l;
      const bool live = t < total;
      const bool from_bucket = tcs[u] < n_direct;
      int j = cell_index_of(pj[u].w);
      if (!from_bucket) {
        j = spill[tcs[u] - n_direct];
        const auto q = pos[j];
        pj[u].x = q.x, pj[u].y = q.y, pj[u].z = q.z;
      }
      bool keep = live & (j != i);
      if (j >= ex_lo && j <= ex_hi) keep = keep & !mm_excluded<R>(ex, j);
      if (!g.direct) {
        int jx, jy, jz;
        cell_of(g, pj[u].x, pj[u].y, pj[u].z, jx, jy, jz);
        const int c = cell[u];
        keep = keep & (!from_bucket | (jx == s_c[grp][c][0] & jy == s_c[grp][c][1] & jz == s_c[grp][c][2]));
      }
      const R dx = wrap(pj[u].x - pi.x, K.lx, K.ilx), dy = wrap(pj[u].y - pi.y, K.ly, K.ily), dz = wrap(pj[u].z - pi.z, K.lz, K.ilz);
      const bool hit = keep & (dx * dx + dy * dy + dz * dz < rl2);
      const unsigned int m = (unsigned int)(__ballot(hit) >> gshift) & kGroupMask;
      const int slot = out + __popc(m & below);
      if (hit & (slot < row_stride)) row[slot] = j;
      out += __popc(m);
    }
  }
  if (l == 0) {
    if (out > row_stride) {
      atomicMax(overflow, out);
      out = row_stride;
    }
    row_len[i] = out;
    ref_pos[i] = pi;
  }
}

template <typename R>
__global__ __launch_bounds__(256) void mm_build_rows_allpairs_kernel(
    int n, const typename Real4<R>::type* __restrict__ pos, const MmConst<R> K, R rl2, const int* __restrict__ excl,
    int* __restrict__ rows, int* __restrict__ row_len, int row_stride, int* __restrict__ overflow,
    typename Real4<R>::type* __restrict__ ref_pos) {
  const int w = threadIdx.x >> 6, lane = threadIdx.x & 63;
  const int i = blockIdx.x * 4 + w;
  if (i >= n) return;
  const auto pi = pos[i];
  int ex[kMaxExcl];
#pragma unroll
  for (int q = 0; q < kMaxExcl; ++q) ex[q] = excl[(size_t)i * kMaxExcl + q];
  int* row = rows + (size_t)i * row_stride;
  int out = 0;
  for (int j0 = 0; j0 < n; j0 += 64) {
    const int j = j0 + lane;
    bool hit = false;
    if (j < n && j != i && !mm_excluded<R>(ex, j)) {
      const auto pj = pos[j];
      const R dx = wrap(pj.x - pi.x, K.lx, K.ilx), dy = wrap(pj.y - pi.y, K.ly, K.ily), dz = wrap(pj.z - pi.z, K.lz, K.ilz);
      hit = dx * dx + dy * dy + dz * dz < rl2;
    }
    const unsigned long long m = __ballot(hit);
    if (hit) {
      const int slot = out + __popcll(m & ((1ull << lane) - 1ull));
      if (slot < row_stride) row[slot] = j;
    }
    out += __popcll(m);
  }
  if (lane == 0) {
    if (out > row_stride) {
      atomicMax(overflow, out);
      out = row_stride;
    }
    row_len[i] = out;
    ref_pos[i] = pi;
  }
}

}

using namespace mythos;

struct mythos_martini_sim : mythos::MdRun {
  mythos_martini* sys = nullptr;
  double dt = 0.02, kT = 2.27, gamma = 1.0;
  double skin = 0.2;
  void* frame[2] = {nullptr, nullptr};
  void *vel = nullptr, *ref_pos = nullptr, *d_inv_mass = nullptr;
  int n_ctypes = 0;
  int* d_ctypes = nullptr;
  void *d_csig2 = nullptr, *d_ceps = nullptr;
  int* d_bb_partner = nullptr;
  int2* d_ba_partner = nullptr;
  void* d_angle_ref = nullptr;
  mythos::VerletRows list{64};
  int* d_row_len = nullptr;
  int *d_rows_in = nullptr, *d_row_len_in = nullptr;
  int rows_in_stride = 0;
  double inner_margin = 0.0;
  int inner_every = 4;
  double* d_epart = nullptr;
  double box[3] = {0, 0, 0};
};

namespace mythos {

template <typename R>
static int mm_rebuild(mythos_martini_sim* sim, const typename Real4<R>::type* pos, const MmConst<R>& K, const double box[3],
                      hipStream_t st) {
  mythos_martini* m = sim->sys;
  VerletRows& L = sim->list;
  const int n = m->n;
  const double rl = m->r_cut + sim->skin;
  CellGrid<R> g;
  if (!cell_grid(g, n, rl, box)) {
    hipLaunchKernelGGL(mm_build_rows_allpairs_kernel<R>, dim3((n + 3) / 4), dim3(256), 0, st, n, pos, K, R(rl * rl), m->d_excl,
                       L.d_rows, sim->d_row_len, L.stride, L.d_overflow, (typename Real4<R>::type*)sim->ref_pos);
    return 0;
  }
  const long long n_cells = (long long)g.nc[0] * g.nc[1] * g.nc[2];
  g.direct = n_cells <= 8LL * n ? 1 : 0;
  CellBins bins;
  if (int rc = cell_table<R>(L, g.direct ? (int)n_cells : next_pow2(2 * n), false, st, bins)) return rc;
  cell_bins_build<R, true>(n, reinterpret_cast<const R*>(pos), g, bins, L.d_overflow, true, st);
  hipLaunchKernelGGL((mm_build_rows_cells_kernel<R, kMmRowG>), dim3((n + 256 / kMmRowG - 1) / (256 / kMmRowG)), dim3(256), 0, st, n, pos, K, g,
                     R(rl * rl), m->d_excl, bins.cnt_cur, (const typename CellPlace<R>::type*)bins.place, bins.cap, bins.spill, bins.H,
                     L.d_rows, sim->d_row_len, L.stride, L.d_overflow, (typename Real4<R>::type*)sim->ref_pos);
  return 0;
}

static bool mm_inner_on(const mythos_martini_sim* sim) {
  return sim->inner_margin > 0 && sim->inner_margin < sim->skin && sim->inner_every >= 2;
}

template <typename R>
static MmConst<R> mm_const(const mythos_martini_sim* sim) {
  const mythos_martini* m = sim->sys;
  const double* box = sim->box;
  MmConst<R> K;
  K.lx = R(box[0]), K.ly = R(box[1]), K.lz = R(box[2]);
  K.ilx = R(1.0 / box[0]), K.ily = R(1.0 / box[1]), K.ilz = R(1.0 / box[2]);
  K.rc2 = R(m->r_cut * m->r_cut);
  K.dt = R(sim->dt), K.half_dt = R(0.5 * sim->dt), K.c1 = R(std::exp(-sim->gamma * sim->dt)), K.kT = R(sim->kT);
  K.skin_half_sq = R(0.25 * sim->skin * sim->skin);
  const bool inner = mm_inner_on(sim);
  const double rin = m->r_cut + sim->inner_margin, smax = 0.5 * sim->inner_margin / std::max(1, sim->inner_every - 1);
  K.rin2 = inner ? R(rin * rin) : R(0);
  K.step_max_sq = inner ? R(smax * smax) : R(0);
  K.n_types = sim->n_ctypes, K.angle_kind = m->angle_kind;
  return K;
}

template <typename R>
static int mm_load_typed(mythos_martini_sim* sim, const R* pos, const R* v, const double box[3], hipStream_t st) {
  using V4 = typename Real4<R>::type;
  mythos_martini* m = sim->sys;
  const int n = m->n, tb = (n + 255) / 256;
  for (int k = 0; k < 3; ++k) sim->box[k] = box[k];
  hipLaunchKernelGGL(mm_pack_kernel<R>, dim3(tb), dim3(256), 0, st, n, pos, v, sim->d_ctypes, (const R*)sim->d_inv_mass,
                     (V4*)sim->frame[0], (V4*)sim->vel);
  MYTHOS_HIP_TRY(hipGetLastError());
  sim->cur = 0;
  sim->resident = true;
  sim->list_valid = false;
  sim->open = false;
  sim->since_build = 0;
  return MYTHOS_OK;
}

template <typename R>
static int mm_advance_typed(mythos_martini_sim* sim, int n_steps, int save_every, bool close, R* traj_pos, double* e_trace,
                            hipStream_t st) {
  using V4 = typename Real4<R>::type;
  mythos_martini* m = sim->sys;
  const int n = m->n;
  const int blocks = (n + kMmPPB - 1) / kMmPPB, grid = 8 * ((blocks + 7) / 8);
  const MmConst<R> K = mm_const<R>(sim);
  const double* box = sim->box;
  V4* fr[2] = {(V4*)sim->frame[0], (V4*)sim->frame[1]};
  V4* vel = (V4*)sim->vel;
  const bool inner_on = mm_inner_on(sim);
  auto ensure_inner = [&]() -> int {
    if (!inner_on) return 0;
    if (!sim->d_row_len_in) MYTHOS_HIP_TRY(hipMalloc((void**)&sim->d_row_len_in, (size_t)n * sizeof(int)));
    if (!sim->d_rows_in || sim->rows_in_stride != sim->list.stride) {
      if (sim->d_rows_in) (void)hipFree(sim->d_rows_in);
      sim->d_rows_in = nullptr;
      MYTHOS_HIP_TRY(hipMalloc((void**)&sim->d_rows_in, (size_t)n * sim->list.stride * sizeof(int)));
      sim->rows_in_stride = sim->list.stride;
    }
    return 0;
  };
  if (int rc = ensure_inner()) return rc;
  const size_t lds = (size_t)2 * sim->n_ctypes * sim->n_ctypes * sizeof(R);
  auto launch_step = [&](int k, const LaunchRow& row) {
    const int cur = row.cur;
    const R kick_close = R(row.kick_close);
    const int do_step = row.do_step;
    R* tp = ((row.save || row.save_next) && traj_pos) ? traj_pos + (size_t)row.sidx * n * 3 : nullptr;
    const bool emit = inner_on && ((k - row.built_at) % sim->inner_every == 0);
    const int* walk_rows = (inner_on && !emit) ? sim->d_rows_in : sim->list.d_rows;
    const int* walk_len = (inner_on && !emit) ? sim->d_row_len_in : sim->d_row_len;
    int* emit_rows = emit ? sim->d_rows_in : nullptr;
    int* emit_len = emit ? sim->d_row_len_in : nullptr;
#define MM_ARGS                                                                                                    \
  n, K, (const V4*)fr[cur], fr[cur ^ 1], vel, walk_rows, walk_len, sim->list.stride, (const R*)sim->d_csig2,          \
      (const R*)sim->d_ceps, m->d_bead_bonds, m->d_bead_angles, m->d_bonds, (const R*)m->d_bond_k,                      \
      (const R*)m->d_bond_r0, m->d_angles, (const R*)m->d_angle_k, (const R*)sim->d_angle_ref, kick_close, do_step,  \
      sim->seed, (uint64_t)(sim->step + k), (const V4*)sim->ref_pos, sim->d_flags, tp, sim->d_epart, sim->list.d_overflow, k, \
      emit_rows, emit_len, sim->d_bb_partner, sim->d_ba_partner
    auto go = [&](auto save_tag, auto emit_tag) {
      constexpr bool SV = decltype(save_tag)::value, EM = decltype(emit_tag)::value;
      if (row.ea) {
        hipExtLaunchKernelGGL((martini_md_step_kernel<R, SV, EM>), dim3(grid), dim3(kMmBlock), lds, st, row.ea, row.eb, 0, MM_ARGS);
      } else {
        hipLaunchKernelGGL((martini_md_step_kernel<R, SV, EM>), dim3(grid), dim3(kMmBlock), lds, st, MM_ARGS);
      }
    };
#undef MM_ARGS
    if (row.save) {
      if (emit) go(std::true_type{}, std::true_type{}); else go(std::true_type{}, std::false_type{});
      hipLaunchKernelGGL(reduce_trace_kernel<kMmTrace>, dim3(1), dim3(256), 0, st, sim->d_epart, blocks,
                         e_trace + (size_t)row.sidx * kMmTrace);
    } else {
      if (emit) go(std::false_type{}, std::true_type{}); else go(std::false_type{}, std::false_type{});
    }
  };
  MdDrive d;
  d.who = "mythos_martini_langevin_run";
  d.n_steps = n_steps, d.save_every = save_every, d.close = close;
  d.energy_rows = save_every > 0 && e_trace != nullptr;
  d.plain_rows = save_every > 0 && e_trace == nullptr && traj_pos != nullptr;
  d.dynamic_list = true;
  d.halt_words = sim->list.d_overflow;
  d.row_stride = &sim->list.stride;
  d.skin = sim->skin;
  if (inner_on)
    d.give_up_hint = ", or the margin of the pruned rows (" + std::to_string(sim->inner_margin) + ") for one pruning in " +
                     std::to_string(sim->inner_every) + " steps";
  d.st = st;
  return md_drive(
      *sim, d, launch_step, [&](int buf) { return mm_rebuild<R>(sim, fr[buf], K, box, st); },
      [&](int buf) -> int {
        auto build = [&] { return mm_rebuild<R>(sim, fr[buf], K, box, st); };
        if (int rc = list_build_until_fit(sim->list, n, build, true, "mythos_martini_langevin_run: neighbour build", st)) return rc;
        return ensure_inner();
      },
      [] { return 0; });
}

template <typename R>
static int mm_store_typed(mythos_martini_sim* sim, R* pos, R* v, hipStream_t st) {
  using V4 = typename Real4<R>::type;
  const int n = sim->sys->n;
  const int rc = sim->open ? mm_advance_typed<R>(sim, 0, 0, true, nullptr, nullptr, st) : MYTHOS_OK;
  hipLaunchKernelGGL(mm_unpack_kernel<R>, dim3((n + 255) / 256), dim3(256), 0, st, n, (const V4*)sim->frame[sim->cur], (const V4*)sim->vel, pos, v);
  MYTHOS_HIP_TRY(hipGetLastError());
  return rc;
}

}

extern "C" {

void mythos_martini_langevin_destroy(mythos_martini_sim_t* s) {
  if (!s) return;
  (void)hipSetDevice(s->sys->device);
  void* ptrs[] = {s->frame[0], s->frame[1], s->vel, s->ref_pos, s->d_inv_mass, s->list.d_rows, s->d_row_len,
                  s->list.d_cell, s->list.d_overflow, s->d_epart, s->d_rows_in, s->d_row_len_in, s->d_angle_ref, s->d_ctypes, s->d_csig2, s->d_ceps, s->d_bb_partner, s->d_ba_partner};
  for (void* p : ptrs)
    if (p) (void)hipFree(p);
  md_run_destroy(*s);
  delete s;
}

mythos_martini_sim_t* mythos_martini_langevin_create(mythos_martini_t* sys, double dt, double kT, double gamma,
                                                     const double* mass, uint64_t seed) {
  if (!sys || !(dt > 0) || !(kT > 0) || !(gamma >= 0)) {
    set_error("mythos_martini_langevin_create: invalid argument");
    return nullptr;
  }
  if (hipSetDevice(sys->device) != hipSuccess) {
    set_error("mythos_martini_langevin_create: hipSetDevice failed");
    return nullptr;
  }
  auto* s = new mythos_martini_sim();
  s->sys = sys, s->dt = dt, s->kT = kT, s->gamma = gamma, s->seed = seed;
  s->rebuild_every = 10;
  const int n = sys->n;
  const size_t w = sys->dtype == MYTHOS_F32 ? sizeof(float) : sizeof(double);
  std::vector<double> im(n);
  for (int i = 0; i < n; ++i) {
    const double mi = mass ? mass[i] : 72.0;
    if (!(mi > 0)) {
      set_error("mythos_martini_langevin_create: masses must be positive");
      delete s;
      return nullptr;
    }
    im[i] = 1.0 / mi;
  }
  const int blocks = (n + kMmPPB - 1) / kMmPPB;
  bool ok = md_run_create(*s) && hipMalloc(&s->frame[0], (size_t)n * 4 * w) == hipSuccess && hipMalloc(&s->frame[1], (size_t)n * 4 * w) == hipSuccess &&
            hipMalloc(&s->vel, (size_t)n * 4 * w) == hipSuccess && hipMalloc(&s->ref_pos, (size_t)n * 4 * w) == hipSuccess &&
            rows_reserve(s->list, n, 256) == 0 && hipMalloc((void**)&s->d_row_len, (size_t)n * sizeof(int)) == hipSuccess &&
            hipMalloc((void**)&s->list.d_overflow, kOverflowWords * sizeof(int)) == hipSuccess &&
            hipMalloc((void**)&s->d_epart, (size_t)blocks * kMmTrace * sizeof(double)) == hipSuccess;
  ok = ok && upload_real(sys->dtype, &s->d_inv_mass, im.data(), im.size());
  if (ok) {
    std::vector<int> bb((size_t)n * kMaxBeadBonds), ba((size_t)n * kMaxBeadAngles), bonds((size_t)2 * std::max(sys->n_bonds, 0)),
        angles((size_t)3 * std::max(sys->n_angles, 0));
    ok = hipMemcpy(bb.data(), sys->d_bead_bonds, bb.size() * sizeof(int), hipMemcpyDeviceToHost) == hipSuccess &&
         hipMemcpy(ba.data(), sys->d_bead_angles, ba.size() * sizeof(int), hipMemcpyDeviceToHost) == hipSuccess &&
         (bonds.empty() || hipMemcpy(bonds.data(), sys->d_bonds, bonds.size() * sizeof(int), hipMemcpyDeviceToHost) == hipSuccess) &&
         (angles.empty() || hipMemcpy(angles.data(), sys->d_angles, angles.size() * sizeof(int), hipMemcpyDeviceToHost) == hipSuccess);
    std::vector<int> pb(bb.size(), -1);
    std::vector<int2> pa(ba.size(), int2{-1, -1});
    for (size_t k = 0; ok && k < bb.size(); ++k)
      if (bb[k] >= 0) pb[k] = bonds[2 * (size_t)(bb[k] >> 1) + (1 - (bb[k] & 1))];
    for (size_t k = 0; ok && k < ba.size(); ++k)
      if (ba[k] >= 0) {
        const int* t = &angles[3 * (size_t)(ba[k] >> 2)];
        const int role = ba[k] & 3;
        pa[k] = role == 0 ? int2{t[1], t[2]} : (role == 1 ? int2{t[0], t[2]} : int2{t[0], t[1]});
      }
    ok = ok && hipMalloc((void**)&s->d_bb_partner, std::max<size_t>(pb.size(), 1) * sizeof(int)) == hipSuccess &&
         hipMalloc((void**)&s->d_ba_partner, std::max<size_t>(pa.size(), 1) * sizeof(int2)) == hipSuccess &&
         hipMemcpy(s->d_bb_partner, pb.data(), pb.size() * sizeof(int), hipMemcpyHostToDevice) == hipSuccess &&
         hipMemcpy(s->d_ba_partner, pa.data(), pa.size() * sizeof(int2), hipMemcpyHostToDevice) == hipSuccess;
  }
  if (ok) {
    const int T = sys->n_types;
    std::vector<int> types(n), cmap(T, -1), used;
    ok = hipMemcpy(types.data(), sys->d_types, (size_t)n * sizeof(int), hipMemcpyDeviceToHost) == hipSuccess;
    std::vector<double> sig((size_t)T * T), ep((size_t)T * T);
    if (sys->dtype == MYTHOS_F32) {
      std::vector<float> a((size_t)T * T), b((size_t)T * T);
      ok = ok && hipMemcpy(a.data(), sys->d_sigma, a.size() * sizeof(float), hipMemcpyDeviceToHost) == hipSuccess &&
           hipMemcpy(b.data(), sys->d_eps, b.size() * sizeof(float), hipMemcpyDeviceToHost) == hipSuccess;
      for (size_t k = 0; k < a.size(); ++k) sig[k] = a[k], ep[k] = b[k];
    } else {
      ok = ok && hipMemcpy(sig.data(), sys->d_sigma, sig.size() * sizeof(double), hipMemcpyDeviceToHost) == hipSuccess &&
           hipMemcpy(ep.data(), sys->d_eps, ep.size() * sizeof(double), hipMemcpyDeviceToHost) == hipSuccess;
    }
    if (ok) {
      for (int t : types)
        if (t >= 0 && t < T && cmap[t] < 0) cmap[t] = 0;
      for (int t = 0; t < T; ++t)
        if (cmap[t] == 0) cmap[t] = (int)used.size(), used.push_back(t);
      const int C = std::max<int>(1, (int)used.size());
      std::vector<double> cs((size_t)C * C, 0.0), ce((size_t)C * C, 0.0);
      for (size_t p = 0; p < used.size(); ++p)
        for (size_t q = 0; q < used.size(); ++q) {
          const double sg = sig[(size_t)used[p] * T + used[q]];
          cs[p * C + q] = sys->dtype == MYTHOS_F32 ? double(float(sg) * float(sg)) : sg * sg;
          ce[p * C + q] = ep[(size_t)used[p] * T + used[q]];
        }
      for (int& t : types) t = (t >= 0 && t < T) ? cmap[t] : 0;
      s->n_ctypes = C;
      ok = hipMalloc((void**)&s->d_ctypes, (size_t)n * sizeof(int)) == hipSuccess &&
           hipMemcpy(s->d_ctypes, types.data(), (size_t)n * sizeof(int), hipMemcpyHostToDevice) == hipSuccess &&
           upload_real(sys->dtype, &s->d_csig2, cs.data(), cs.size()) && upload_real(sys->dtype, &s->d_ceps, ce.data(), ce.size());
    }
  }
  {
    std::vector<double> ref((size_t)std::max(sys->n_angles, 0));
    if (ok && sys->n_angles > 0) {
      if (sys->dtype == MYTHOS_F32) {
        std::vector<float> t0(ref.size());
        ok = hipMemcpy(t0.data(), sys->d_angle_t0, t0.size() * sizeof(float), hipMemcpyDeviceToHost) == hipSuccess;
        for (size_t a = 0; a < ref.size(); ++a) ref[a] = sys->angle_kind == 0 ? std::cos(double(t0[a])) : double(t0[a]);
      } else {
        ok = hipMemcpy(ref.data(), sys->d_angle_t0, ref.size() * sizeof(double), hipMemcpyDeviceToHost) == hipSuccess;
        if (sys->angle_kind == 0)
          for (double& v : ref) v = std::cos(v);
      }
    }
    ok = ok && upload_real(sys->dtype, &s->d_angle_ref, ref.data(), ref.size());
  }
  ok = ok && hipMemset(s->list.d_overflow, 0, kOverflowWords * sizeof(int)) == hipSuccess;
  if (!ok) {
    set_error("mythos_martini_langevin_create: device allocation failed");
    mythos_martini_langevin_destroy(s);
    return nullptr;
  }
  return s;
}

int mythos_martini_langevin_set_neighbor_policy(mythos_martini_sim_t* s, double skin, int rebuild_every) {
  if (!s || !(skin > 0) || rebuild_every < 1) {
    set_error("mythos_martini_langevin_set_neighbor_policy: skin > 0 and rebuild_every >= 1 required");
    return MYTHOS_ERR_INVALID_ARGUMENT;
  }
  s->skin = skin;
  s->rebuild_every = rebuild_every;
  s->list_fitted = false;
  s->list_valid = false;
  return MYTHOS_OK;
}

int mythos_martini_langevin_set_inner_list(mythos_martini_sim_t* s, double margin, int every) {
  if (!s || every < 0) {
    set_error("mythos_martini_langevin_set_inner_list: invalid argument");
    return MYTHOS_ERR_INVALID_ARGUMENT;
  }
  s->inner_margin = margin;
  s->inner_every = every;
  s->list_valid = false;
  return MYTHOS_OK;
}

int mythos_martini_langevin_init_velocities(mythos_martini_sim_t* s, void* vel, mythos_stream_t stream) {
  if (!s || !vel) {
    set_error("mythos_martini_langevin_init_velocities: invalid argument");
    return MYTHOS_ERR_INVALID_ARGUMENT;
  }
  MYTHOS_HIP_TRY(hipSetDevice(s->sys->device));
  if (s->sys->dtype == MYTHOS_F32)
    hipLaunchKernelGGL(mm_init_velocities_kernel<float>, dim3(1), dim3(256), 0, (hipStream_t)stream, s->sys->n, float(s->kT),
                       (const float*)s->d_inv_mass, s->seed, (float*)vel);
  else
    hipLaunchKernelGGL(mm_init_velocities_kernel<double>, dim3(1), dim3(256), 0, (hipStream_t)stream, s->sys->n, s->kT,
                       (const double*)s->d_inv_mass, s->seed, (double*)vel);
  MYTHOS_HIP_TRY(hipGetLastError());
  return MYTHOS_OK;
}

namespace {

int mm_check_box(const mythos_martini_sim_t* s, const double* box, const char* who) {
  if (!box || !(box[0] > 0) || !(box[1] > 0) || !(box[2] > 0)) {
    set_error(std::string(who) + ": invalid argument");
    return MYTHOS_ERR_INVALID_ARGUMENT;
  }
  const double rl = s->sys->r_cut + s->skin;
  if (2.0 * rl > std::min(box[0], std::min(box[1], box[2]))) {
    set_error(std::string(who) + ": the box is smaller than twice (r_cut + skin): minimum image breaks down");
    return MYTHOS_ERR_INVALID_ARGUMENT;
  }
  return MYTHOS_OK;
}

int mm_load(mythos_martini_sim_t* s, const void* pos, const void* vel, const double* box, hipStream_t st) {
  return s->sys->dtype == MYTHOS_F32 ? mm_load_typed<float>(s, (const float*)pos, (const float*)vel, box, st)
                                     : mm_load_typed<double>(s, (const double*)pos, (const double*)vel, box, st);
}
int mm_advance(mythos_martini_sim_t* s, int n_steps, int save_every, bool close, void* traj, double* e_trace, hipStream_t st) {
  return s->sys->dtype == MYTHOS_F32 ? mm_advance_typed<float>(s, n_steps, save_every, close, (float*)traj, e_trace, st)
                                     : mm_advance_typed<double>(s, n_steps, save_every, close, (double*)traj, e_trace, st);
}
int mm_store(mythos_martini_sim_t* s, void* pos, void* vel, hipStream_t st) {
  return s->sys->dtype == MYTHOS_F32 ? mm_store_typed<float>(s, (float*)pos, (float*)vel, st) : mm_store_typed<double>(s, (double*)pos, (double*)vel, st);
}

}

int mythos_martini_langevin_run(mythos_martini_sim_t* s, void* pos, void* vel, const double* box, int n_steps,
                                int save_every, void* traj_pos, double* e_trace, mythos_stream_t stream) {
  if (!s || !pos || !vel || n_steps < 0 || save_every < 0) {
    set_error("mythos_martini_langevin_run: invalid argument");
    return MYTHOS_ERR_INVALID_ARGUMENT;
  }
  if (int rc = mm_check_box(s, box, "mythos_martini_langevin_run")) return rc;
  MYTHOS_HIP_TRY(hipSetDevice(s->sys->device));
  hipStream_t st = (hipStream_t)stream;
  if (int rc = mm_load(s, pos, vel, box, st)) return rc;
  const int rc = mm_advance(s, n_steps, save_every, true, traj_pos, e_trace, st);
  if (s->resident) {
    if (int rs = mm_store(s, pos, vel, st)) return rc ? rc : rs;
    MYTHOS_HIP_TRY(hipStreamSynchronize(st));
  }
  return rc;
}

int mythos_martini_langevin_load(mythos_martini_sim_t* s, const void* pos, const void* vel, const double* box, mythos_stream_t stream) {
  if (!s || !pos || !vel) {
    set_error("mythos_martini_langevin_load: invalid argument");
    return MYTHOS_ERR_INVALID_ARGUMENT;
  }
  if (int rc = mm_check_box(s, box, "mythos_martini_langevin_load")) return rc;
  MYTHOS_HIP_TRY(hipSetDevice(s->sys->device));
  return mm_load(s, pos, vel, box, (hipStream_t)stream);
}

int mythos_martini_langevin_advance(mythos_martini_sim_t* s, int n_steps, int save_every, void* traj_pos, double* e_trace,
                                    mythos_stream_t stream) {
  if (!s || n_steps < 0 || save_every < 0) {
    set_error("mythos_martini_langevin_advance: invalid argument");
    return MYTHOS_ERR_INVALID_ARGUMENT;
  }
  if (!s->resident) {
    set_error("mythos_martini_langevin_advance: no resident state (call mythos_martini_langevin_load first; a run that ended in a "
              "numeric error drops its state)");
    return MYTHOS_ERR_NOT_READY;
  }
  MYTHOS_HIP_TRY(hipSetDevice(s->sys->device));
  return mm_advance(s, n_steps, save_every, false, traj_pos, e_trace, (hipStream_t)stream);
}

int mythos_martini_langevin_store(mythos_martini_sim_t* s, void* pos, void* vel, mythos_stream_t stream) {
  if (!s || !pos || !vel) {
    set_error("mythos_martini_langevin_store: invalid argument");
    return MYTHOS_ERR_INVALID_ARGUMENT;
  }
  if (!s->resident) {
    set_error("mythos_martini_langevin_store: no resident state");
    return MYTHOS_ERR_NOT_READY;
  }
  MYTHOS_HIP_TRY(hipSetDevice(s->sys->device));
  return mm_store(s, pos, vel, (hipStream_t)stream);
}

int64_t mythos_martini_langevin_get_step(const mythos_martini_sim_t* s) { return md_get_step(s); }

int mythos_martini_langevin_last_rebuilds(const mythos_martini_sim_t* s, int* scheduled) {
  return md_last_count(s, &MdRun::last_rebuilds, scheduled, "mythos_martini_langevin_last_rebuilds");
}

int mythos_martini_langevin_last_kernel_ms(const mythos_martini_sim_t* s, double* kernel_ms, double* loop_ms_per_launch,
                                           int* launches, int* samples) {
  return md_last_kernel_ms(s, kernel_ms, loop_ms_per_launch, launches, samples, "mythos_martini_langevin_last_kernel_ms");
}

int mythos_martini_langevin_neighbor_stats(const mythos_martini_sim_t* s, int* max_row, double* mean_row) {
  if (!s) {
    set_error("mythos_martini_langevin_neighbor_stats: invalid argument");
    return MYTHOS_ERR_INVALID_ARGUMENT;
  }
  MYTHOS_HIP_TRY(hipSetDevice(s->sys->device));
  return row_stats(s->d_row_len, s->sys->n, 0, max_row, mean_row);
}

int mythos_martini_langevin_get_rows(const mythos_martini_sim_t* s, int which, int32_t* rows, int32_t* row_len, int* stride) {
  if (!s || (which != 0 && which != 1)) {
    set_error("mythos_martini_langevin_get_rows: invalid argument");
    return MYTHOS_ERR_INVALID_ARGUMENT;
  }
  const int* d_rows = which == 0 ? s->list.d_rows : s->d_rows_in;
  const int* d_len = which == 0 ? s->d_row_len : s->d_row_len_in;
  if (stride) *stride = s->list.stride;
  if (!rows && !row_len) return MYTHOS_OK;
  if (!d_rows || !d_len || !s->list_valid) {
    set_error(which == 0 ? "mythos_martini_langevin_get_rows: no list has been built"
                         : "mythos_martini_langevin_get_rows: no pruned rows (switched off, or no step taken yet)");
    return MYTHOS_ERR_INVALID_ARGUMENT;
  }
  MYTHOS_HIP_TRY(hipSetDevice(s->sys->device));
  MYTHOS_HIP_TRY(hipDeviceSynchronize());
  if (rows) MYTHOS_HIP_TRY(hipMemcpy(rows, d_rows, (size_t)s->sys->n * s->list.stride * sizeof(int), hipMemcpyDeviceToHost));
  if (row_len) MYTHOS_HIP_TRY(hipMemcpy(row_len, d_len, (size_t)s->sys->n * sizeof(int), hipMemcpyDeviceToHost));
  return MYTHOS_OK;
}
// ... 11 lines not shown
```

### mythos_amd/csrc/md_driver.h

```cpp
#ifndef MYTHOS_MD_DRIVER_H
#define MYTHOS_MD_DRIVER_H

#include <algorithm>
#include <string>

#include "mythos_internal.h"

namespace mythos {

struct MdRun {
  static constexpr int kCtlWords = 4;
  static constexpr int kMaxSamples = 16;
  uint64_t seed = 0;
  int64_t step = 0;
  int cur = 0;
  bool open = false;
  bool resident = false;
  bool list_valid = false;
  bool list_fitted = false;
  int since_build = 0;
  int rebuild_every = 0;
  int timing_samples = 0;
  hipEvent_t ev0 = nullptr, ev1 = nullptr;
  hipEvent_t sa[kMaxSamples] = {}, sb[kMaxSamples] = {};
  int* d_flags = nullptr;
  int* h_ctl = nullptr;
  int* d_ctl = nullptr;
  double last_avg_ms = 0;
  double last_kernel_ms = 0;
  int last_launches = 0, last_samples = 0;
  int last_recoveries = 0;
  int last_rebuilds = 0;
};

inline bool md_run_create(MdRun& r) {
  bool ok = hipMalloc((void**)&r.d_flags, MdRun::kCtlWords * sizeof(int)) == hipSuccess &&
            hipMemset(r.d_flags, 0, MdRun::kCtlWords * sizeof(int)) == hipSuccess &&
            hipHostMalloc((void**)&r.h_ctl, 8 * sizeof(int), hipHostMallocDefault) == hipSuccess &&
            hipHostGetDevicePointer((void**)&r.d_ctl, r.h_ctl, 0) == hipSuccess &&
            hipEventCreate(&r.ev0) == hipSuccess && hipEventCreate(&r.ev1) == hipSuccess;
  if (ok) std::fill(r.h_ctl, r.h_ctl + 8, 0);
  for (int k = 0; ok && k < MdRun::kMaxSamples; ++k)
    ok = hipEventCreate(&r.sa[k]) == hipSuccess && hipEventCreate(&r.sb[k]) == hipSuccess;
  return ok;
}

inline void md_run_destroy(MdRun& r) {
  if (r.d_flags) (void)hipFree(r.d_flags);
  if (r.h_ctl) (void)hipHostFree(r.h_ctl);
  for (hipEvent_t e : {r.ev0, r.ev1})
    if (e) (void)hipEventDestroy(e);
  for (int k = 0; k < MdRun::kMaxSamples; ++k) {
    if (r.sa[k]) (void)hipEventDestroy(r.sa[k]);
    if (r.sb[k]) (void)hipEventDestroy(r.sb[k]);
  }
}

static __global__ void publish_ctl_kernel(int* __restrict__ flags, const int* __restrict__ overflow, int* __restrict__ out) {
  if (threadIdx.x != 0 || blockIdx.x != 0) return;
  out[0] = flags[0], out[1] = flags[1], out[2] = flags[2], out[3] = flags[3];
  out[4] = overflow ? overflow[0] : 0, out[5] = overflow ? overflow[1] : 0, out[6] = overflow ? overflow[2] : 0;
  flags[0] = 0, flags[2] = 0;
}

template <int WIDTH>
static __global__ __launch_bounds__(256) void reduce_trace_kernel(const double* __restrict__ part, int n_blocks, double* __restrict__ out) {
  static_assert(WIDTH <= 16, "one column per trace entry");
  __shared__ double acc[16][17];
  const int k = threadIdx.x & 15, g = threadIdx.x >> 4;
  double s = 0.0;
  if (k < WIDTH)
    for (int b = g; b < n_blocks; b += 16) s += part[(size_t)b * WIDTH + k];
  acc[g][k] = s;
  __syncthreads();
  if (g == 0 && k < WIDTH && out) {
    double t = 0.0;
#pragma unroll
    for (int j = 0; j < 16; ++j) t += acc[j][k];
    out[k] = t;
  }
}

struct MdDrive {
  const char* who;
  int n_steps, save_every;
  bool close;
  bool energy_rows;
  bool plain_rows;
  bool dynamic_list;
  int* halt_words;
  const int* row_stride;
  double skin;
  std::string give_up_hint;
  hipStream_t st;
};

struct LaunchRow {
  int cur;
  bool save;
  bool save_next;
  int sidx;
  float kick_close;
  int do_step;
  int built_at;
  hipEvent_t ea, eb;
};

template <class Launch, class Rebuild, class RebuildUntilFit, class OnAbort>
static int md_drive(MdRun& run, const MdDrive& d, Launch&& launch, Rebuild&& rebuild, RebuildUntilFit&& rebuild_until_fit,
                    OnAbort&& on_abort) {
  const bool closes = d.close || (d.energy_rows && d.n_steps > 0 && d.n_steps % d.save_every == 0);
  const int n_launch = closes ? d.n_steps + 1 : d.n_steps;
  if (n_launch == 0) return MYTHOS_OK;
  const hipStream_t st = d.st;
  const bool was_open = run.open;
  const int cur0 = run.cur;
  int built_at = 0;
  if (d.dynamic_list) {
    if (!run.list_fitted) {
      if (int rc = rebuild_until_fit(cur0)) return rc;
      run.list_fitted = true;
    } else if (!run.list_valid) {
      if (int rc = rebuild(cur0)) return rc;
    } else {
      built_at = -run.since_build;
    }
    run.list_valid = true;
  }
  const bool timing = run.timing_samples > 0;
  if (timing) MYTHOS_HIP_TRY(hipEventRecord(run.ev0, st));
  int launches = 0, samples = 0, recoveries = 0, scheduled = 0;
  const int max_samples = std::min(run.timing_samples, MdRun::kMaxSamples);
  const int sample_stride = std::max(1, n_launch / std::max(1, max_samples));
  auto drop_list = [&]() {
    run.list_valid = false;
    run.since_build = 0;
    run.last_recoveries = recoveries;
    run.last_rebuilds = scheduled;
    (void)hipMemsetAsync(run.d_flags + 1, 0, 3 * sizeof(int), st);
    if (d.halt_words) (void)hipMemsetAsync(d.halt_words, 0, kOverflowWords * sizeof(int), st);
  };
  auto fail = [&](int ran, int rc) -> int {
    run.cur = cur0 ^ (ran & 1);
    run.step += ran;
    run.open = was_open || ran > 0;
    drop_list();
    return rc;
  };
  constexpr int kMaxRecoveries = 64;
  const long long dbg_seg = debug_value(MYTHOS_DEBUG_MD_SEGMENT);
  const int kSegment = dbg_seg > 0 ? (int)std::min<long long>(dbg_seg, 1 << 20) : 8192;
  int k = 0, seg_len = kSegment;
  int cur = cur0;
  while (k < n_launch) {
    const int seg_start = k, seg_end = std::min(n_launch - 1, k + seg_len - 1);
    for (; k <= seg_end; ++k) {
      const bool last = (k == d.n_steps);
      LaunchRow row;
      row.cur = cur;
      row.save = d.energy_rows && k > 0 && (k % d.save_every == 0);
      row.save_next = d.plain_rows && !last && ((k + 1) % d.save_every == 0);
      row.sidx = row.save ? (k / d.save_every - 1) : (row.save_next ? ((k + 1) / d.save_every - 1) : 0);
      if (d.dynamic_list && k - built_at >= run.rebuild_every) {
        if (int rc = rebuild(cur)) return fail(k, rc);
        built_at = k;
        ++scheduled;
        if (debug_value(MYTHOS_DEBUG_MD_OVERFLOW_AT) == k + 1) {
          debug_clear(MYTHOS_DEBUG_MD_OVERFLOW_AT);
          MYTHOS_HIP_TRY(hipMemsetD32Async((hipDeviceptr_t)d.halt_words, *d.row_stride + 1, 1, st));
        }
      }
      row.kick_close = (k == 0 && !was_open) ? 0.0f : 0.5f;
      row.do_step = last ? 0 : 1;
      row.built_at = built_at;
      row.ea = row.eb = nullptr;
      if (!row.save && (k % sample_stride == sample_stride / 2) && samples < max_samples)
        row.ea = run.sa[samples], row.eb = run.sb[samples], ++samples;
      launch(k, row);
      ++launches;
      cur ^= 1;
    }
    if (timing && k >= n_launch) MYTHOS_HIP_TRY(hipEventRecord(run.ev1, st));
    hipLaunchKernelGGL(publish_ctl_kernel, dim3(1), dim3(1), 0, st, run.d_flags, (const int*)d.halt_words, run.d_ctl);
    MYTHOS_HIP_TRY(hipGetLastError());
    MYTHOS_HIP_TRY(hipStreamSynchronize(st));
    const int* ctl = run.h_ctl;
    if (ctl[0] & 2) {
      drop_list();
      run.resident = false;
      run.step += d.n_steps;
      run.last_avg_ms = run.last_kernel_ms = 0.0;
      run.last_launches = launches;
      run.last_samples = samples;
      set_error(std::string(d.who) + ": NaN in the state (time step too large or overlapping start configuration)");
      return MYTHOS_ERR_NUMERIC;
    }
    const int aborted = ctl[3];
    if (ctl[1] == 0 && ctl[4] == 0 && ctl[5] == 0 && aborted == 0) continue;
    if (aborted != 0) {
      if (int rc = on_abort()) return fail(aborted - 1, rc);
    } else if (!d.dynamic_list) {
      break;
    }
    const int progressed = std::max(ctl[2], seg_start);
    const int ran = aborted != 0 ? std::min(progressed, aborted - 1) : progressed;
    if (++recoveries > kMaxRecoveries) {
      set_error(std::string(d.who) + ": the neighbour list had to be rebuilt out of turn more than " + std::to_string(kMaxRecoveries) +
                " times in one run: the skin (" + std::to_string(d.skin) + ") is too small for a rebuild every " +
                std::to_string(run.rebuild_every) + " steps" + d.give_up_hint);
      return fail(ran, MYTHOS_ERR_OVERFLOW);
    }
    cur = cur0 ^ (ran & 1);
    k = ran;
    seg_len = std::max(std::min(256, kSegment), seg_len / 4);
    MYTHOS_HIP_TRY(hipMemsetAsync(run.d_flags + 1, 0, 3 * sizeof(int), st));
    if (d.dynamic_list) {
      if (int rc = rebuild_until_fit(cur)) return fail(ran, rc);
      built_at = k;
    }
  }
  run.last_recoveries = recoveries;
  run.last_rebuilds = scheduled;
  run.cur = cur;
  run.open = !closes;
  run.since_build = d.n_steps - built_at;
  if (timing) {
    float ms = 0;
    MYTHOS_HIP_TRY(hipEventElapsedTime(&ms, run.ev0, run.ev1));
    run.last_avg_ms = launches ? double(ms) / launches : 0.0;
    double acc = 0;
    for (int s = 0; s < samples; ++s) {
      float t = 0;
      MYTHOS_HIP_TRY(hipEventElapsedTime(&t, run.sa[s], run.sb[s]));
      acc += t;
    }
    run.last_kernel_ms = samples ? acc / samples : 0.0;
  } else {
    run.last_avg_ms = run.last_kernel_ms = 0.0;
  }
  run.last_launches = launches;
  run.last_samples = samples;
  run.step += d.n_steps;
  return MYTHOS_OK;
}

inline int md_set_timing(MdRun* r, int samples, const char* who) {
  if (!r || samples < 0) {
    set_error(std::string(who) + ": invalid argument");
    return MYTHOS_ERR_INVALID_ARGUMENT;
  }
  r->timing_samples = std::min(samples, MdRun::kMaxSamples);
  return MYTHOS_OK;
}

inline int md_last_kernel_ms(const MdRun* r, double* kernel_ms, double* loop_ms_per_launch, int* launches, int* samples,
                             const char* who) {
  if (!r) {
    set_error(std::string(who) + ": invalid argument");
    return MYTHOS_ERR_INVALID_ARGUMENT;
  }
  if (kernel_ms) *kernel_ms = r->last_kernel_ms;
  if (loop_ms_per_launch) *loop_ms_per_launch = r->last_avg_ms;
  if (launches) *launches = r->last_launches;
  if (samples) *samples = r->last_samples;
  return MYTHOS_OK;
}

inline int md_last_count(const MdRun* r, int MdRun::*field, int* out, const char* who) {
  if (!r || !out) {
    set_error(std::string(who) + ": invalid argument");
    return MYTHOS_ERR_INVALID_ARGUMENT;
  }
  *out = r->*field;
  return MYTHOS_OK;
}

inline int64_t md_get_step(const MdRun* r) { return r ? r->step : -1; }

}

#endif
```

### mythos_amd/csrc/mythos_internal.h

```cpp
#pragma once
#include <hip/hip_runtime.h>

#include <algorithm>
#include <cmath>
#include <cstdint>
#include <string>
#include <vector>

#include "../../include/mythos_hip.h"
#include "oxdna_math.h"

namespace mythos {

void set_error(const std::string& msg);
int hip_fail(hipError_t e, const char* what);
long long debug_value(int key);
void debug_clear(int key);

#define MYTHOS_HIP_TRY(expr)                                   \
  do {                                                         \
    hipError_t _e = (expr);                                    \
    if (_e != hipSuccess) return ::mythos::hip_fail(_e, #expr); \
  } while (0)

constexpr int ROW_ROLE_Q = 1 << 30;
constexpr int ROW_INDEX_MASK = ROW_ROLE_Q - 1;
constexpr int ROW_BONDED_SLOTS = 4;

template <typename R>
struct BoxT {
  R l[3];
  R il[3];
  int on;
};

template <typename T>
inline int grow_buffer(T*& ptr, size_t& cap, size_t need) {
  if (need <= cap) return 0;
  if (ptr) (void)hipFree(ptr);
  ptr = nullptr;
  cap = 0;
  MYTHOS_HIP_TRY(hipMalloc((void**)&ptr, need * sizeof(T)));
  cap = need;
  return 0;
}

constexpr int kOverflowWords = 3;

struct VerletRows {
  int* d_rows = nullptr;
  size_t rows_cap = 0;
  int stride = 0;
  int* d_overflow = nullptr;
  int* d_cell = nullptr;
  size_t cell_cap = 0;
  int cell_H = 0;
  int cell_alloc_bucket_cap = 0;
  bool cell_sites = false;
  int cell_bucket_cap;
  int cell_phase = 0;
  explicit VerletRows(int bucket_cap) : cell_bucket_cap(bucket_cap) {}
};

}

struct mythos_obs;

struct mythos_system {
  int model = 0;
  int n = 0;
  int dtype = 0;
  int device = 0;
  int n_bonded = 0;
  bool has_box = false;
  double box[3] = {0, 0, 0};

  int* d_meta = nullptr;

  mythos::VerletRows list{32};
  int* d_row_len = nullptr;
  bool nbrs_set = false;
  int list_epoch = 0;
  int param_epoch = 0;
  std::vector<int> h_partners;
  bool extra_bonds = false;

  void* d_ref_pos = nullptr;
  void* d_ref_off = nullptr;
  void* d_ref_a1 = nullptr;

  bool params_set = false;
  mythos::OxParams<float> pf;
  mythos::OxParams<double> pd;
  std::vector<double> pd_sets;
  int param_sets() const { return model == 4 ? 3 : 1; }
  bool types_set = false;
  std::vector<int> h_meta;
  float* d_pf = nullptr;
  double* d_pd = nullptr;

  void* d_ps_marg = nullptr;
  int* d_ps_unit = nullptr;
  void* d_ps_bp = nullptr;
  int ps_bp_cap = 0;
  int pseq_terms = 0;
  int ps_n_bp = 0;
  double* ps_gmarg = nullptr;
  double* ps_gbp = nullptr;

  double* d_epart = nullptr;
  size_t epart_cap = 0;
  double* d_pgpart = nullptr;
  size_t pgpart_cap = 0;
};

namespace mythos {

template <typename R>
BoxT<R> make_box(const mythos_system* s) {
  BoxT<R> b;
  b.on = s->has_box ? 1 : 0;
  for (int k = 0; k < 3; ++k) {
    b.l[k] = R(s->has_box ? s->box[k] : 1.0);
    b.il[k] = R(s->has_box ? 1.0 / s->box[k] : 1.0);
  }
  return b;
}

template <typename R>
const OxParams<R>& params_of(const mythos_system* s);
template <>
inline const OxParams<float>& params_of<float>(const mythos_system* s) { return s->pf; }
template <>
inline const OxParams<double>& params_of<double>(const mythos_system* s) { return s->pd; }
template <typename R>
const R* device_params_of(const mythos_system* s);
template <>
inline const float* device_params_of<float>(const mythos_system* s) { return s->d_pf; }
template <>
inline const double* device_params_of<double>(const mythos_system* s) { return s->d_pd; }

static_assert(ROW_BONDED_SLOTS == 4, "the row builders copy four partner slots");
inline int* row_close_of(const mythos_system* sys) { return sys->d_row_len + (size_t)(1 + ROW_BONDED_SLOTS) * sys->n; }

inline const double* oxdna_param_set(const mythos_system* sys, int k) {
  return sys->param_sets() == 1 ? sys->pd.v : sys->pd_sets.data() + (size_t)k * OXP_COUNT;
}
inline double oxdna_param_max(const mythos_system* sys, int idx) {
  double m = oxdna_param_set(sys, 0)[idx];
  for (int k = 1; k < sys->param_sets(); ++k) m = std::max(m, oxdna_param_set(sys, k)[idx]);
  return m;
}

inline double oxdna_close_range(const mythos_system* sys) {
  double off_back = 0.0, off_base = 0.0, off_stack = 0.0;
  for (int k = 0; k < std::min(sys->param_sets(), 2); ++k) {
    const double* P = oxdna_param_set(sys, k);
    off_back = std::max(off_back, std::sqrt(P[GEO_BACK_A1] * P[GEO_BACK_A1] + (sys->model >= 2 ? P[GEO_BACK_A2] * P[GEO_BACK_A2] : 0.0)));
    off_base = std::max(off_base, std::fabs(P[GEO_BASE]));
    off_stack = std::max(off_stack, std::fabs(P[GEO_STACK]));
  }
  auto mx = [&](int idx) { return oxdna_param_max(sys, idx); };
  double rcom = std::max(mx(NEXC_BACK_BASE_RC), mx(NEXC_BASE_BACK_RC)) + off_back + off_base;
  rcom = std::max(rcom, mx(NEXC_BASE_RC) + 2 * off_base);
  rcom = std::max(rcom, std::max(mx(HYDR_RCHIGH), mx(CRST_RCHIGH)) + 2 * off_base);
  rcom = std::max(rcom, mx(CXST_RCHIGH) + 2 * off_stack);
  return rcom * (1.0 + 1e-6);
}

int oxdna_energy_launch(mythos_system* sys, const void* center, const void* quat, int n_frames, double* e_terms,
                        void* dU_dcenter, void* dU_dquat, double* dU_dparams, mythos_obs* obs, double* obs_out,
                        hipStream_t stream);
int rows_from_pairs(mythos_system* sys, const int32_t* pairs, int n_pairs);
int rows_build_device(mythos_system* sys, const void* center, bool center_is_vec4, double r_cut, double skin,
                      const void* backbone_offsets, const void* base_vectors, bool write_refs, hipStream_t stream);
int rows_build_until_fit(mythos_system* sys, const void* center, bool center_is_vec4, double r_cut, double skin,
                         const void* backbone_offsets, const void* base_vectors, bool write_refs, bool headroom,
                         hipStream_t stream);

}
```

### mythos_amd/csrc/neighbors.hip

```cpp
#include <algorithm>
#include <cmath>

#include "cell_list.h"
#include "oxdna_gather.h"

namespace mythos {

int rows_from_pairs(mythos_system* sys, const int32_t* pairs, int n_pairs) {
  const int n = sys->n;
  std::vector<int> count(n, 0);
  for (int k = 0; k < n_pairs; ++k) {
    const int i = pairs[2 * k], j = pairs[2 * k + 1];
    if (i < 0 || j < 0 || i >= n || j >= n || i == j) {
      set_error("set_neighbors: pair index out of range or i == j");
      return MYTHOS_ERR_INVALID_ARGUMENT;
    }
    ++count[i];
    ++count[j];
  }
  int mx = 0;
  for (int c : count) mx = std::max(mx, c);
  const int stride = ((mx + ROW_BONDED_SLOTS + 15) / 16) * 16;
  std::vector<int> rows((size_t)n * stride, -1), len(n, ROW_BONDED_SLOTS);
  for (int i = 0; i < n; ++i) {
    for (int k = 0; k < ROW_BONDED_SLOTS; ++k) rows[(size_t)i * stride + k] = sys->h_partners[(size_t)ROW_BONDED_SLOTS * i + k];
  }
  for (int k = 0; k < n_pairs; ++k) {
    const int i = pairs[2 * k], j = pairs[2 * k + 1];
    rows[(size_t)i * stride + len[i]++] = j;
    rows[(size_t)j * stride + len[j]++] = i | ROW_ROLE_Q;
  }
  if (int rc = rows_reserve(sys->list, n, stride)) return rc;
  MYTHOS_HIP_TRY(hipMemcpy(sys->list.d_rows, rows.data(), rows.size() * sizeof(int), hipMemcpyHostToDevice));
  MYTHOS_HIP_TRY(hipMemcpy(sys->d_row_len, len.data(), n * sizeof(int), hipMemcpyHostToDevice));
  MYTHOS_HIP_TRY(hipMemcpy(row_close_of(sys), len.data(), n * sizeof(int), hipMemcpyHostToDevice));
  sys->nbrs_set = true;
  return 0;
}

template <typename R>
struct SiteCrit {
  const R* off;
  const R* a1;
  R rbb2;
  R rbase2, rstack2, rkb2;
  R g_ba, g_st;
};

template <typename R, class A>
__device__ __forceinline__ bool far_in_range_v(const SiteCrit<R>& sc, const A& oi, const A& oj, const V3<R>& d) {
  const V3<R> e{d.x + oj[0] - oi[0], d.y + oj[1] - oi[1], d.z + oj[2] - oi[2]};
  return dot(e, e) < sc.rbb2;
}
template <typename R>
__device__ __forceinline__ bool far_in_range(const SiteCrit<R>& sc, int i, int j, const V3<R>& d) {
  if (!sc.off) return true;
  return far_in_range_v(sc, sc.off + 4 * i, sc.off + 4 * j, d);
}

template <typename R, class A>
__device__ __forceinline__ bool site_close_v(const SiteCrit<R>& sc, const A& ai, const A& oi, const A& aj, const A& oj, const V3<R>& d) {
  const V3<R> da{aj[0] - ai[0], aj[1] - ai[1], aj[2] - ai[2]};
  V3<R> e = d;
  axpy(e, sc.g_ba, da);
  if (dot(e, e) < sc.rbase2) return true;
  e = d;
  axpy(e, sc.g_st, da);
  if (dot(e, e) < sc.rstack2) return true;
  e = V3<R>{d.x + sc.g_ba * aj[0] - oi[0], d.y + sc.g_ba * aj[1] - oi[1], d.z + sc.g_ba * aj[2] - oi[2]};
  if (dot(e, e) < sc.rkb2) return true;
  e = V3<R>{d.x + oj[0] - sc.g_ba * ai[0], d.y + oj[1] - sc.g_ba * ai[1], d.z + oj[2] - sc.g_ba * ai[2]};
  return dot(e, e) < sc.rkb2;
}
template <typename R>
__device__ __forceinline__ bool site_close(const SiteCrit<R>& sc, int i, int j, const V3<R>& d) {
  if (!sc.off) return true;
  return site_close_v(sc, sc.a1 + 4 * i, sc.off + 4 * i, sc.a1 + 4 * j, sc.off + 4 * j, d);
}

template <typename R, bool VEC4>
__global__ __launch_bounds__(256) void build_rows_allpairs_kernel(int n, const R* __restrict__ pos,
                                                                   const BoxT<R> box, R rc2, R rcl2,
                                                                   const SiteCrit<R> sc,
                                                                   const int* __restrict__ partners_rows_in,
                                                                   int* __restrict__ rows, int* __restrict__ row_len,
                                                                   int* __restrict__ row_close, int row_stride,
                                                                   int* __restrict__ overflow) {
  const int wave = (blockIdx.x * blockDim.x + threadIdx.x) >> 6;
  const int lane = threadIdx.x & 63;
  if (wave >= n) return;
  const int i = wave;
  constexpr int S = VEC4 ? 4 : 3;
  const V3<R> ci{pos[S * i], pos[S * i + 1], pos[S * i + 2]};
  int* row = rows + (size_t)i * row_stride;
  const int* bq = partners_rows_in + (size_t)ROW_BONDED_SLOTS * i;
  const int4 bp = make_int4(bq[0], bq[1], bq[2], bq[3]);
  int cnt = ROW_BONDED_SLOTS, n_close = 0;
  for (int pass = 0; pass < 2; ++pass) {
    for (int j0 = 0; j0 < n; j0 += 64) {
      const int j = j0 + lane;
      bool hit = false;
      if (j < n && j != i && j != bp.x && j != bp.y && j != bp.z && j != bp.w) {
        V3<R> d{pos[S * j] - ci.x, pos[S * j + 1] - ci.y, pos[S * j + 2] - ci.z};
        d = min_image(d, box);
        const R r2 = dot(d, d);
        if (r2 < rc2) {
          const bool cl = r2 < rcl2 && site_close(sc, i, j, d);
          hit = (pass == 0) ? cl : (!cl && far_in_range(sc, i, j, d));
        }
      }
      const unsigned long long m = __ballot(hit);
      if (hit) {
        const int slot = cnt + __popcll(m & ((1ull << lane) - 1ull));
        if (slot < row_stride) row[slot] = (j < i) ? (j | ROW_ROLE_Q) : j;
      }
      cnt += __popcll(m);
    }
    if (pass == 0) n_close = cnt;
  }
  if (lane == 0) {
    row[0] = bp.x, row[1] = bp.y, row[2] = bp.z, row[3] = bp.w;
    if (cnt > row_stride) {
      atomicMax(overflow, cnt);
      cnt = row_stride;
    }
    row_len[i] = cnt;
    row_close[i] = min(n_close, cnt);
  }
}

template <int G>
__device__ __forceinline__ void group_sort_to_row(const int* buf, int cnt, int* __restrict__ dst, int room, int l) {
  for (int b = 0; b < cnt; b += G) {
    const int k = b + l;
    const int e = (k < cnt) ? buf[k] : 0;
    const int key = e & ROW_INDEX_MASK;
    int rank = 0;
    for (int q = 0; q < cnt; ++q) rank += ((buf[q] & ROW_INDEX_MASK) < key) ? 1 : 0;
    if (k < cnt && rank < room) dst[rank] = e;
  }
}

#ifndef MYTHOS_ROW_G
#define MYTHOS_ROW_G 16
#endif
constexpr int kRowG = MYTHOS_ROW_G;

template <typename R, bool VEC4, int G>
__global__ __launch_bounds__(256) void build_rows_cells_kernel(int n, const R* __restrict__ pos, const BoxT<R> box,
                                                                const CellGrid<R> g, R rc2, R rcl2,
                                                                const SiteCrit<R> sc,
                                                                const int* __restrict__ partners,
                                                                const int* __restrict__ cell_cnt,
                                                                const typename CellPlace<R>::type* __restrict__ place,
                                                                int cell_cap, const int* __restrict__ spill, int cell_H,
                                                                size_t site_stride,
                                                                int* __restrict__ rows,
                                                                int* __restrict__ row_len, int* __restrict__ row_close,
                                                                int row_stride, int* __restrict__ overflow,
                                                                R* __restrict__ ref_pos, R* __restrict__ ref_off,
                                                                R* __restrict__ ref_a1) {
  constexpr int NG = 256 / G;
  __shared__ int s_pre[NG][29], s_st[NG][28], s_c[NG][28][3];
  extern __shared__ int s_seg_all[];
  const int kSegCap = row_stride;
  const int grp = threadIdx.x / G, l = threadIdx.x % G;
  const int gshift = (threadIdx.x & 63) & ~(G - 1);
  const int i = blockIdx.x * NG + grp;
  if (i >= n) return;
  int* s_close = s_seg_all + (size_t)grp * 2 * row_stride;
  int* s_far = s_close + row_stride;
  constexpr int S = VEC4 ? 4 : 3;
  const V3<R> ci{pos[S * i], pos[S * i + 1], pos[S * i + 2]};
  using PL = typename CellPlace<R>::type;
  R oi[3] = {R(0), R(0), R(0)}, ai[3] = {R(0), R(0), R(0)};
  if (sc.off) {
#pragma unroll
    for (int a = 0; a < 3; ++a) oi[a] = sc.off[4 * (size_t)i + a], ai[a] = sc.a1[4 * (size_t)i + a];
  }
  const int total = cell_candidates<R, G>(g, ci.x, ci.y, ci.z, cell_cnt, cell_cap, cell_H, s_pre[grp], s_st[grp], s_c[grp], l);
  int* row = rows + (size_t)i * row_stride;
  const int* bq = partners + (size_t)ROW_BONDED_SLOTS * i;
  const int4 bp = make_int4(bq[0], bq[1], bq[2], bq[3]);
  int out_c = 0, out_f = 0;
  int lo = 0;
  constexpr unsigned int kGroupMask = (G == 32) ? 0xffffffffu : ((1u << G) - 1u);
  for (int t0 = 0; t0 < total; t0 += G) {
    const int t = t0 + l;
    bool hit_c = false, hit_f = false;
    int j = -1;
    if (t < total) {
      while (s_pre[grp][lo + 1] <= t) ++lo;
      R xj, yj, zj;
      R oj[3] = {R(0), R(0), R(0)}, aj[3] = {R(0), R(0), R(0)};
      if (lo < 27) {
        const size_t at = (size_t)s_st[grp][lo] + (t - s_pre[grp][lo]);
        const PL pl = place[at];
        if (site_stride) {
          const PL po = place[site_stride + at], pa = place[2 * site_stride + at];
          oj[0] = po.x, oj[1] = po.y, oj[2] = po.z, aj[0] = pa.x, aj[1] = pa.y, aj[2] = pa.z;
        }
        xj = pl.x, yj = pl.y, zj = pl.z;
        j = cell_index_of(pl.w);
      } else {
        j = spill[t - s_pre[grp][27]];
        xj = pos[S * j], yj = pos[S * j + 1], zj = pos[S * j + 2];
        if (site_stride) {
#pragma unroll
          for (int a = 0; a < 3; ++a) oj[a] = sc.off[4 * (size_t)j + a], aj[a] = sc.a1[4 * (size_t)j + a];
        }
      }
      if (j != i && j != bp.x && j != bp.y && j != bp.z && j != bp.w) {
        bool mine = true;
        if (!g.direct && lo < 27) {
          int jx, jy, jz;
          cell_of(g, xj, yj, zj, jx, jy, jz);
          mine = jx == s_c[grp][lo][0] && jy == s_c[grp][lo][1] && jz == s_c[grp][lo][2];
        }
        if (mine) {
          V3<R> d{xj - ci.x, yj - ci.y, zj - ci.z};
          d = min_image(d, box);
          const R r2 = dot(d, d);
          if (r2 < rc2) {
            if (site_stride) {
              hit_c = r2 < rcl2 && site_close_v(sc, ai, oi, aj, oj, d);
              hit_f = !hit_c && far_in_range_v(sc, oi, oj, d);
            } else {
              hit_c = r2 < rcl2 && site_close(sc, i, j, d);
              hit_f = !hit_c && far_in_range(sc, i, j, d);
            }
          }
        }
      }
    }
    const int e = (j < i) ? (j | ROW_ROLE_Q) : j;
    const unsigned int mc = (unsigned int)(__ballot(hit_c) >> gshift) & kGroupMask;
    const unsigned int mf = (unsigned int)(__ballot(hit_f) >> gshift) & kGroupMask;
    const unsigned int below = (1u << l) - 1u;
    if (hit_c) {
      const int k = out_c + __popc(mc & below);
      if (k < kSegCap) s_close[k] = e;
    }
    if (hit_f) {
      const int k = out_f + __popc(mf & below);
      if (k < kSegCap) s_far[k] = e;
    }
    out_c += __popc(mc);
    out_f += __popc(mf);
  }
  __builtin_amdgcn_wave_barrier();
  __builtin_amdgcn_fence(__ATOMIC_ACQ_REL, "wavefront");
  const int n_close = ROW_BONDED_SLOTS + out_c;
  int out = n_close + out_f;
  group_sort_to_row<G>(s_close, min(out_c, kSegCap), row + ROW_BONDED_SLOTS, row_stride - ROW_BONDED_SLOTS, l);
  if (n_close < row_stride) group_sort_to_row<G>(s_far, min(out_f, kSegCap), row + n_close, row_stride - n_close, l);
  if (l == 0) {
    row[0] = bp.x, row[1] = bp.y, row[2] = bp.z, row[3] = bp.w;
    if (out > row_stride) {
      atomicMax(overflow, out);
      out = row_stride;
    }
    row_len[i] = out;
    row_close[i] = min(n_close, out);
    if (ref_pos) {
      R* rp = ref_pos + 4 * (size_t)i;
      rp[0] = ci.x, rp[1] = ci.y, rp[2] = ci.z, rp[3] = VEC4 ? pos[S * i + 3] : R(0);
      if (sc.off) {
        R* ro = ref_off + 4 * (size_t)i;
        R* ra = ref_a1 + 4 * (size_t)i;
#pragma unroll
        for (int k = 0; k < 4; ++k) ro[k] = sc.off[4 * (size_t)i + k], ra[k] = sc.a1[4 * (size_t)i + k];
      }
    }
  }
}

template <typename R>
static int build_cells_typed(mythos_system* sys, const R* pos, bool vec4, double rl, double skin, const R* off,
                             const R* a1, bool write_refs, hipStream_t st) {
  R* ref_pos = write_refs ? (R*)sys->d_ref_pos : nullptr;
  R* ref_off = write_refs ? (R*)sys->d_ref_off : nullptr;
  R* ref_a1 = write_refs ? (R*)sys->d_ref_a1 : nullptr;
  const int n = sys->n;
  const double rcl = sys->params_set ? std::min(rl, oxdna_close_range(sys) + skin) : rl;
  int* d_close = row_close_of(sys);
  double rbb = rl;
  if (off && sys->params_set) {
    rbb = oxdna_param_max(sys, NEXC_BACKBONE_RC);
    if (sys->model >= 2) rbb = std::max(rbb, oxdna_param_max(sys, DH_RCUT));
    rbb = std::min(rl, rbb + skin);
  }
  if (!sys->params_set || !a1) off = nullptr;
  SiteCrit<R> sc{off, a1, R(rbb * rbb), R(0), R(0), R(0), R(0), R(0)};
  if (off) {
    auto mx = [&](int idx) { return oxdna_param_max(sys, idx); };
    const double* Pd = oxdna_param_set(sys, 0);
    const double* Pr = oxdna_param_set(sys, sys->param_sets() == 1 ? 0 : 1);
    const double slack_ba = std::fabs(Pd[GEO_BASE] - Pr[GEO_BASE]), slack_st = std::fabs(Pd[GEO_STACK] - Pr[GEO_STACK]);
    auto sq = [&](double r) { return R((r + skin) * (r + skin)); };
    sc.rbase2 = sq(std::max({mx(HYDR_RCHIGH), mx(CRST_RCHIGH), mx(NEXC_BASE_RC)}) + slack_ba);
    sc.rstack2 = sq(mx(CXST_RCHIGH) + slack_st);
    sc.rkb2 = sq(std::max(mx(NEXC_BACK_BASE_RC), mx(NEXC_BASE_BACK_RC)) + 0.5 * slack_ba);
    sc.g_ba = R(0.5 * (Pd[GEO_BASE] + Pr[GEO_BASE]));
    sc.g_st = R(0.5 * (Pd[GEO_STACK] + Pr[GEO_STACK]));
  }
  VerletRows& L = sys->list;
  CellGrid<R> g;
  const bool cells = cell_grid(g, n, rl, sys->has_box ? sys->box : nullptr);
  const int blocks_ap = (n * 64 + 255) / 256;
  int* d_partners = sys->d_row_len + n;
  const BoxT<R> box = make_box<R>(sys);
  if (!cells) {
    if (vec4)
      hipLaunchKernelGGL((build_rows_allpairs_kernel<R, true>), dim3(blocks_ap), dim3(256), 0, st, n, pos, box,
                         R(rl * rl), R(rcl * rcl), sc, d_partners, L.d_rows, sys->d_row_len, d_close, L.stride, L.d_overflow);
    else
      hipLaunchKernelGGL((build_rows_allpairs_kernel<R, false>), dim3(blocks_ap), dim3(256), 0, st, n, pos, box,
                         R(rl * rl), R(rcl * rcl), sc, d_partners, L.d_rows, sys->d_row_len, d_close, L.stride, L.d_overflow);
    if (write_refs && vec4) {
      const size_t bytes = (size_t)n * 4 * sizeof(R);
      MYTHOS_HIP_TRY(hipMemcpyAsync(ref_pos, pos, bytes, hipMemcpyDeviceToDevice, st));
      if (sc.off) {
        MYTHOS_HIP_TRY(hipMemcpyAsync(ref_off, sc.off, bytes, hipMemcpyDeviceToDevice, st));
        MYTHOS_HIP_TRY(hipMemcpyAsync(ref_a1, sc.a1, bytes, hipMemcpyDeviceToDevice, st));
      }
    }
    return 0;
  }
  const bool sites = sc.off != nullptr && vec4;
  CellBins bins;
  if (int rc = cell_table<R>(L, next_pow2(2 * n), sites, st, bins)) return rc;
  const size_t site_stride = sites ? (size_t)bins.H * bins.cap : 0;
  if (vec4)
    cell_bins_build<R, true>(n, pos, g, bins, L.d_overflow, false, st, sc.off, sc.a1);
  else
    cell_bins_build<R, false>(n, pos, g, bins, L.d_overflow, false, st);
  constexpr int kPerBlock = 256 / kRowG;
  const int wb = (n + kPerBlock - 1) / kPerBlock;
  const size_t far_lds = (size_t)kPerBlock * 2 * L.stride * sizeof(int);
  if (vec4)
    hipLaunchKernelGGL((build_rows_cells_kernel<R, true, kRowG>), dim3(wb), dim3(256), far_lds, st, n, pos, box, g, R(rl * rl),
                       R(rcl * rcl), sc, d_partners, bins.cnt_cur, (const typename CellPlace<R>::type*)bins.place, bins.cap, bins.spill, bins.H, site_stride, L.d_rows, sys->d_row_len, d_close, L.stride,
                       L.d_overflow, ref_pos, ref_off, ref_a1);
  else
    hipLaunchKernelGGL((build_rows_cells_kernel<R, false, kRowG>), dim3(wb), dim3(256), far_lds, st, n, pos, box, g, R(rl * rl),
                       R(rcl * rcl), sc, d_partners, bins.cnt_cur, (const typename CellPlace<R>::type*)bins.place, bins.cap, bins.spill, bins.H, site_stride, L.d_rows, sys->d_row_len, d_close, L.stride,
                       L.d_overflow, ref_pos, ref_off, ref_a1);
  return 0;
}

int rows_build_device(mythos_system* sys, const void* center, bool center_is_vec4, double r_cut, double skin,
                      const void* backbone_offsets, const void* base_vectors, bool write_refs, hipStream_t stream) {
  if (sys->list.stride == 0)
    if (int rc = rows_reserve(sys->list, sys->n, 64)) return rc;
  const double rl = r_cut + skin;
  int rc;
  if (sys->dtype == MYTHOS_F32)
    rc = build_cells_typed<float>(sys, (const float*)center, center_is_vec4, rl, skin, (const float*)backbone_offsets, (const float*)base_vectors, write_refs, stream);
  else
    rc = build_cells_typed<double>(sys, (const double*)center, center_is_vec4, rl, skin, (const double*)backbone_offsets, (const double*)base_vectors, write_refs, stream);
  if (rc) return rc;
  MYTHOS_HIP_TRY(hipGetLastError());
  sys->nbrs_set = true;
  return 0;
}

int rows_build_until_fit(mythos_system* sys, const void* center, bool center_is_vec4, double r_cut, double skin,
                         const void* backbone_offsets, const void* base_vectors, bool write_refs, bool headroom,
                         hipStream_t stream) {
  return list_build_until_fit(
      sys->list, sys->n,
      [&] { return rows_build_device(sys, center, center_is_vec4, r_cut, skin, backbone_offsets, base_vectors, write_refs, stream); },
      headroom, "neighbour build", stream);
}

}
```

### mythos_amd/hip_system.py

```python

from __future__ import annotations

import ctypes as C

import numpy as np
import torch

from mythos_amd import _lib

N_TERMS = 8
TRACE_WIDTH = 10
TERM_NAMES = (
    "fene",
    "bonded_excluded_volume",
    "stacking",
    "unbonded_excluded_volume",
    "hydrogen_bonding",
    "cross_stacking",
    "coaxial_stacking",
    "debye",
)


def _stream(device) -> C.c_void_p:
    return C.c_void_p(torch.cuda.current_stream(device).cuda_stream)


def _dtype_code(dtype: torch.dtype) -> int:
    if dtype == torch.float32:
        return 0
    if dtype == torch.float64:
        return 1
    raise ValueError(f"unsupported dtype {dtype}: use torch.float32 or torch.float64")


class OxdnaSystem:

    def __init__(self, model: int, seq, is_end, bonded, box=None, dtype=torch.float32, device=None, is_rna=None):
        lib = _lib.load()
        if _lib.device_count() == 0 or not torch.cuda.is_available():
            raise _lib.MythosHipError("no HIP device visible: the mythos_amd HIP path has no CPU fallback")
        self.device = torch.device("cuda", torch.cuda.current_device()) if device is None else torch.device(device)
        if self.device.type != "cuda":
            raise ValueError("OxdnaSystem needs a cuda (HIP) device")
        self.dtype = dtype
        self.model = int(model)
        seq = np.ascontiguousarray(seq, dtype=np.int32)
        self.n = int(seq.shape[0])
        is_end = np.zeros(self.n, np.uint8) if is_end is None else np.ascontiguousarray(is_end, dtype=np.uint8)
        bonded = np.ascontiguousarray(bonded, dtype=np.int32).reshape(-1, 2)
        box_arr = None if box is None else np.ascontiguousarray(np.broadcast_to(np.asarray(box, np.float64), (3,)))
        self.box = box_arr
        self._h = lib.mythos_oxdna_create(
            self.model,
            self.n,
            seq.ctypes.data_as(_lib.c_int_p),
            is_end.ctypes.data_as(_lib.c_uint8_p),
            int(bonded.shape[0]),
            bonded.ctypes.data_as(_lib.c_int_p),
            None if box_arr is None else box_arr.ctypes.data_as(_lib.c_double_p),
            _dtype_code(dtype),
            self.device.index or 0,
        )
        if not self._h:
            raise _lib.MythosHipError(f"mythos_oxdna_create: {_lib.last_error()}")
        self._lib = lib
        self._pseq_n_bp = 0
        self._pseq_terms = 0
        self.n_params = lib.mythos_oxdna_param_count() * (3 if self.model == 4 else 1)
        if self.model == 4:
            if is_rna is None:
                raise ValueError("an oxNA system (model 4) needs is_rna, the type of every nucleotide")
            t = np.ascontiguousarray(is_rna, dtype=np.uint8)
            if t.shape != (self.n,):
                raise ValueError(f"is_rna must have shape ({self.n},)")
            _lib.check(lib.mythos_oxdna_set_nucleotide_types(self._h, t.ctypes.data_as(_lib.c_uint8_p)), "set_nucleotide_types")

    def close(self):
        if getattr(self, "_h", None):
            self._lib.mythos_oxdna_destroy(self._h)
            self._h = None

    def __del__(self):
        try:
            self.close()
        except Exception:
            pass

    def set_params(self, flat) -> None:
        flat = np.ascontiguousarray(torch.as_tensor(flat).detach().cpu().numpy(), dtype=np.float64)
        _lib.check(
            self._lib.mythos_oxdna_set_params(self._h, flat.ctypes.data_as(_lib.c_double_p), int(flat.shape[0])),
            "set_params",
        )

    def set_pseq(self, marginals=None, unit=None, bp_probs=None, terms: int = 0) -> None:
        if not terms:
            _lib.check(self._lib.mythos_oxdna_set_pseq(self._h, None, None, 0, None, 0), "set_pseq")
            self._pseq_terms = 0
            return
        marg = np.ascontiguousarray(marginals, dtype=np.float64)
        unit = np.ascontiguousarray(unit, dtype=np.int32)
        bp = np.ascontiguousarray(bp_probs, dtype=np.float64).reshape(-1, 4)
        if marg.shape != (self.n, 4) or unit.shape != (self.n,):
            raise ValueError(f"marginals must be ({self.n}, 4) and unit ({self.n},)")
        n_bp = int(bp.shape[0]) if (unit >= 0).any() else 0
        self._pseq_n_bp = n_bp
        if (unit >= 0).any() and int(unit.max()) >= 2 * n_bp:
            raise ValueError("bp_probs has fewer rows than the base pairs named in unit")
        _lib.check(self._lib.mythos_oxdna_set_pseq(self._h, marg.ctypes.data_as(_lib.c_double_p), unit.ctypes.data_as(_lib.c_int_p),
                                                   n_bp, bp.ctypes.data_as(_lib.c_double_p), int(terms)), "set_pseq")
        self._pseq_terms = int(terms)

    def set_neighbors(self, pairs) -> None:
        pairs = np.ascontiguousarray(pairs, dtype=np.int32)
        if pairs.ndim != 2 or (pairs.size and pairs.shape[1] != 2):
            raise ValueError("pairs must have shape (P, 2)")
        _lib.check(
            self._lib.mythos_oxdna_set_neighbors(self._h, pairs.ctypes.data_as(_lib.c_int_p), int(pairs.shape[0])),
            "set_neighbors",
        )

    def build_neighbors(self, center: torch.Tensor, r_cut: float, skin: float) -> None:
        c = self._check(center, (self.n, 3), "center")
        _lib.check(
            self._lib.mythos_oxdna_build_neighbors(self._h, _lib.ptr(c), float(r_cut), float(skin), _stream(self.device)),
            "build_neighbors",
        )

    def neighbor_stats(self) -> tuple[int, float]:
        mx, mean = C.c_int(0), C.c_double(0.0)
        _lib.check(self._lib.mythos_oxdna_neighbor_stats(self._h, C.byref(mx), C.byref(mean)), "neighbor_stats")
        return mx.value, mean.value

    def _check(self, t: torch.Tensor, tail: tuple, name: str) -> torch.Tensor:
        if not isinstance(t, torch.Tensor) or t.device != self.device:
            raise ValueError(f"{name} must be a torch tensor on {self.device}")
        if t.dtype != self.dtype:
            raise ValueError(f"{name} must have dtype {self.dtype}, got {t.dtype}")
        if tuple(t.shape[-len(tail):]) != tail:
            raise ValueError(f"{name} must have trailing shape {tail}, got {tuple(t.shape)}")
        return t.contiguous()

    def energy(self, center, quat, *, grads=False, param_grads=False, observables=None, pseq_grads=False):
        single = center.dim() == 2
        c = self._check(center, (self.n, 3), "center")
        q = self._check(quat, (self.n, 4), "quat")
        if single:
            c, q = c[None], q[None]
        nf = c.shape[0]
        if q.shape[0] != nf:
            raise ValueError("center and quat disagree on the number of frames")
        e = torch.empty((nf, N_TERMS), dtype=torch.float64, device=self.device)
        gc = torch.empty_like(c) if grads else None
        gq = torch.empty_like(q) if grads else None
        gp = torch.empty((nf, self.n_params), dtype=torch.float64, device=self.device) if param_grads else None
        if pseq_grads:
            if not param_grads or observables is not None:
                raise ValueError("pseq_grads comes with param_grads and without fused observables")
            gm = torch.empty((nf, self.n, 4), dtype=torch.float64, device=self.device)
            gb = torch.empty((nf, max(self._pseq_n_bp, 1), 4), dtype=torch.float64, device=self.device)
            _lib.check(
                self._lib.mythos_oxdna_energy_dpseq(
                    self._h, _lib.ptr(c), _lib.ptr(q), nf, _lib.ptr(e), _lib.ptr(gc), _lib.ptr(gq), _lib.ptr(gp), _lib.ptr(gm),
                    _lib.ptr(gb), _stream(self.device),
                ),
                "energy_dpseq",
            )
            if single:
                return e[0], (gc[0] if grads else None), (gq[0] if grads else None), gp[0], gm[0], gb[0]
            return e, gc, gq, gp, gm, gb
        if observables is None:
            _lib.check(
                self._lib.mythos_oxdna_energy(
                    self._h, _lib.ptr(c), _lib.ptr(q), nf, _lib.ptr(e), _lib.ptr(gc), _lib.ptr(gq), _lib.ptr(gp),
                    _stream(self.device),
                ),
                "energy",
            )
            rows = None
        else:
            rows = torch.empty((nf, observables.width), dtype=torch.float64, device=self.device)
            _lib.check(
                self._lib.mythos_oxdna_energy_obs(
                    self._h, _lib.ptr(c), _lib.ptr(q), nf, _lib.ptr(e), _lib.ptr(gc), _lib.ptr(gq), _lib.ptr(gp),
                    observables._h, _lib.ptr(rows), _stream(self.device),
                ),
                "energy_obs",
            )
        if single:
            e = e[0]
            gc = gc[0] if grads else None
            gq = gq[0] if grads else None
            gp = gp[0] if param_grads else None
        if observables is not None:
            return e, gc, gq, gp, rows
        return e, gc, gq, gp


def _touched(*tensors) -> None:
    for t in tensors:
        if t is not None:
            torch.autograd.graph.increment_version(t)


class _MdIntegrator:

    _prefix = ""

    def _fn(self, name):
        return getattr(self._lib, f"{self._prefix}_{name}")

    def close(self):
        if getattr(self, "_h", None):
            self._fn("destroy")(self._h)
            self._h = None

    def __del__(self):
        try:
            self.close()
        except Exception:
            pass

    @property
    def step(self) -> int:
        return int(self._fn("get_step")(self._h))

    def set_timing(self, samples: int) -> None:
        _lib.check(self._fn("set_timing")(self._h, int(samples)), "set_timing")

    def _count(self, name: str) -> int:
        r = C.c_int(0)
        _lib.check(self._fn(name)(self._h, C.byref(r)), name)
        return int(r.value)

    def last_recoveries(self) -> int:
        return self._count("last_recoveries")

    def last_rebuilds(self) -> int:
        return self._count("last_rebuilds")

    def last_kernel_ms(self) -> dict:
        k, loop, n, ns = C.c_double(0.0), C.c_double(0.0), C.c_int(0), C.c_int(0)
        _lib.check(self._fn("last_kernel_ms")(self._h, C.byref(k), C.byref(loop), C.byref(n), C.byref(ns)), "last_kernel_ms")
        return {"kernel_ms": k.value, "loop_ms_per_launch": loop.value, "launches": n.value, "samples": ns.value}


class LangevinIntegrator(_MdIntegrator):

    _prefix = "mythos_langevin"

    def __init__(self, system: OxdnaSystem, dt, kT, gamma_t, gamma_r, mass=1.0, inertia=(1.0, 1.0, 1.0), seed=0):
        self.system = system
        self._lib = system._lib
        inertia = np.ascontiguousarray(inertia, dtype=np.float64)
        self._h = self._lib.mythos_langevin_create(
            system._h, float(dt), float(kT), float(gamma_t), float(gamma_r), float(mass),
            inertia.ctypes.data_as(_lib.c_double_p), C.c_uint64(int(seed) & (2**64 - 1)),
        )
        if not self._h:
            raise _lib.MythosHipError(f"mythos_langevin_create: {_lib.last_error()}")
        self.dt, self.kT = float(dt), float(kT)

    def set_neighbor_policy(self, r_cut: float, skin: float, every: int) -> None:
        _lib.check(
            self._lib.mythos_langevin_set_neighbor_policy(self._h, float(r_cut), float(skin), int(every)),
            "set_neighbor_policy",
        )

    def set_unfused(self, on: bool = True) -> None:
        _lib.check(self._lib.mythos_langevin_set_option(self._h, 0, 1 if on else 0), "set_option(unfused)")

    def init_momenta(self):
        s = self.system
        p = torch.empty((s.n, 3), dtype=s.dtype, device=s.device)
        ang = torch.empty((s.n, 3), dtype=s.dtype, device=s.device)
        _lib.check(self._lib.mythos_langevin_init_momenta(self._h, _lib.ptr(p), _lib.ptr(ang), _stream(s.device)), "init_momenta")
        return p, ang

    def run(self, center, quat, p_lin, p_ang, n_steps: int, save_every: int = 0, want_energy: bool = True):
        s = self.system
        for t, tail, name in ((center, (s.n, 3), "center"), (quat, (s.n, 4), "quat"), (p_lin, (s.n, 3), "p_lin"), (p_ang, (s.n, 3), "p_ang")):
            if s._check(t, tail, name).data_ptr() != t.data_ptr():
                raise ValueError(f"{name} must be contiguous (it is updated in place)")
        n_save = n_steps // save_every if save_every > 0 else 0
        tc = torch.empty((n_save, s.n, 3), dtype=s.dtype, device=s.device) if n_save else None
        tq = torch.empty((n_save, s.n, 4), dtype=s.dtype, device=s.device) if n_save else None
        et = torch.zeros((n_save, TRACE_WIDTH), dtype=torch.float64, device=s.device) if (n_save and want_energy) else None
        rc = self._lib.mythos_langevin_run(
            self._h, _lib.ptr(center), _lib.ptr(quat), _lib.ptr(p_lin), _lib.ptr(p_ang), int(n_steps),
            int(save_every), _lib.ptr(tc), _lib.ptr(tq), _lib.ptr(et), _stream(s.device),
        )
        _touched(center, quat, p_lin, p_ang)
        _lib.check(rc, "langevin_run")
        return tc, tq, et

    def _state_ptrs(self, center, quat, p_lin, p_ang):
        s = self.system
        for t, tail, name in ((center, (s.n, 3), "center"), (quat, (s.n, 4), "quat"), (p_lin, (s.n, 3), "p_lin"), (p_ang, (s.n, 3), "p_ang")):
            if s._check(t, tail, name).data_ptr() != t.data_ptr():
                raise ValueError(f"{name} must be contiguous")
        return _lib.ptr(center), _lib.ptr(quat), _lib.ptr(p_lin), _lib.ptr(p_ang)

    def load(self, center, quat, p_lin, p_ang) -> None:
        _lib.check(self._lib.mythos_langevin_load(self._h, *self._state_ptrs(center, quat, p_lin, p_ang), _stream(self.system.device)), "langevin_load")

    def advance(self, n_steps: int, save_every: int = 0, want_energy: bool = True, out=None):
        s = self.system
        n_save = n_steps // save_every if save_every > 0 else 0
        if out is not None and n_save:
            tc, tq = out
            for t, w in ((tc, 3), (tq, 4)):
                if t.device != s.device or t.dtype != s.dtype or tuple(t.shape) != (n_save, s.n, w) or not t.is_contiguous():
                    raise ValueError(f"out tensors must be contiguous {s.dtype} of shape ({n_save}, {s.n}, 3) and ({n_save}, {s.n}, 4) on {s.device}")
        else:
            tc = torch.empty((n_save, s.n, 3), dtype=s.dtype, device=s.device) if n_save else None
            tq = torch.empty((n_save, s.n, 4), dtype=s.dtype, device=s.device) if n_save else None
        et = torch.zeros((n_save, TRACE_WIDTH), dtype=torch.float64, device=s.device) if (n_save and want_energy) else None
        _lib.check(
            self._lib.mythos_langevin_advance(self._h, int(n_steps), int(save_every), _lib.ptr(tc), _lib.ptr(tq), _lib.ptr(et), _stream(s.device)),
            "langevin_advance",
        )
        if out is not None and n_save:
            _touched(tc, tq)
        return tc, tq, et

    def store(self, center, quat, p_lin, p_ang) -> None:
        rc = self._lib.mythos_langevin_store(self._h, *self._state_ptrs(center, quat, p_lin, p_ang), _stream(self.system.device))
        _touched(center, quat, p_lin, p_ang)
        _lib.check(rc, "langevin_store")

    @_MdIntegrator.step.setter
    def step(self, value: int) -> None:
        _lib.check(self._lib.mythos_langevin_set_step(self._h, int(value)), "set_step")

    def set_seed(self, seed: int) -> None:
        _lib.check(self._lib.mythos_langevin_set_seed(self._h, C.c_uint64(int(seed) & (2**64 - 1))), "set_seed")


class MartiniSystem:

    N_TERMS = 3

    def __init__(self, types, sigma, eps, bonds, bond_k, bond_r0, angles, angle_k, angle_t0, angle_kind=0, r_cut=1.1,
                 dtype=torch.float32, device=None):
        lib = _lib.load()
        if _lib.device_count() == 0 or not torch.cuda.is_available():
            raise _lib.MythosHipError("no HIP device visible: the mythos_amd HIP path has no CPU fallback")
        self.device = torch.device("cuda", torch.cuda.current_device()) if device is None else torch.device(device)
        self.dtype = dtype
        types = np.ascontiguousarray(types, dtype=np.int32)
        self.n = int(types.shape[0])
        sigma = np.ascontiguousarray(sigma, dtype=np.float64)
        eps = np.ascontiguousarray(eps, dtype=np.float64)
        n_types = int(sigma.shape[0])
        bonds = np.ascontiguousarray(bonds, dtype=np.int32).reshape(-1, 2)
        angles = np.ascontiguousarray(angles, dtype=np.int32).reshape(-1, 3)
        self.n_types, self.n_bonds, self.n_angles = n_types, int(bonds.shape[0]), int(angles.shape[0])
        f = lambda a: np.ascontiguousarray(a, dtype=np.float64)
        bond_k, bond_r0, angle_k, angle_t0 = f(bond_k), f(bond_r0), f(angle_k), f(angle_t0)
        dp = lambda a: a.ctypes.data_as(_lib.c_double_p)
        self._h = lib.mythos_martini_create(
            self.n, types.ctypes.data_as(_lib.c_int_p), n_types, dp(sigma), dp(eps), int(bonds.shape[0]),
            bonds.ctypes.data_as(_lib.c_int_p), dp(bond_k), dp(bond_r0), int(angles.shape[0]),
            angles.ctypes.data_as(_lib.c_int_p), dp(angle_k), dp(angle_t0), int(angle_kind), float(r_cut),
            _dtype_code(dtype), self.device.index or 0,
        )
        if not self._h:
            raise _lib.MythosHipError(f"mythos_martini_create: {_lib.last_error()}")
        self._lib = lib

    def close(self):
        if getattr(self, "_h", None):
            self._lib.mythos_martini_destroy(self._h)
            self._h = None

    def __del__(self):
        try:
            self.close()
        except Exception:
            pass

    def energy(self, pos: torch.Tensor, box: torch.Tensor, grads: bool = False):
        single = pos.dim() == 2
        if single:
            pos, box = pos[None], torch.as_tensor(box).reshape(1, 3)
        if pos.device != self.device or pos.dtype != self.dtype or tuple(pos.shape[1:]) != (self.n, 3):
            raise ValueError(f"pos must be a {self.dtype} tensor of shape (F, {self.n}, 3) on {self.device}")
        pos = pos.contiguous()
        box = torch.as_tensor(box, dtype=self.dtype, device=self.device).reshape(-1, 3)
        if box.shape[0] == 1 and pos.shape[0] > 1:
            box = box.expand(pos.shape[0], 3)
        box = box.contiguous()
        nf = pos.shape[0]
        e = torch.empty((nf, 3), dtype=torch.float64, device=self.device)
        g = torch.empty_like(pos) if grads else None
        _lib.check(
            self._lib.mythos_martini_energy(self._h, _lib.ptr(pos), _lib.ptr(box), nf, _lib.ptr(e), _lib.ptr(g), _stream(self.device)),
            "martini_energy",
        )
        return (e[0], g[0] if grads else None) if single else (e, g)

    def param_grads(self, pos: torch.Tensor, box: torch.Tensor, lj: bool = True, bonds: bool = True, angles: bool = True):
        if pos.dim() == 2:
            pos, box = pos[None], torch.as_tensor(box).reshape(1, 3)
        if pos.device != self.device or pos.dtype != self.dtype or tuple(pos.shape[1:]) != (self.n, 3):
            raise ValueError(f"pos must be a {self.dtype} tensor of shape (F, {self.n}, 3) on {self.device}")
        pos = pos.contiguous()
        box = torch.as_tensor(box, dtype=self.dtype, device=self.device).reshape(-1, 3)
        if box.shape[0] == 1 and pos.shape[0] > 1:
            box = box.expand(pos.shape[0], 3)
        box = box.contiguous()
        nf = pos.shape[0]

        def buf(on, *shape):
            return torch.zeros((nf, *shape), dtype=torch.float64, device=self.device) if on else None

        out = {"sigma": buf(lj, self.n_types, self.n_types), "eps": buf(lj, self.n_types, self.n_types),
               "bond_k": buf(bonds, self.n_bonds), "bond_r0": buf(bonds, self.n_bonds),
               "angle_k": buf(angles, self.n_angles), "angle_t0": buf(angles, self.n_angles)}
        _lib.check(
            self._lib.mythos_martini_param_grads(
                self._h, _lib.ptr(pos), _lib.ptr(box), nf, _lib.ptr(out["sigma"]), _lib.ptr(out["eps"]),
                _lib.ptr(out["bond_k"]), _lib.ptr(out["bond_r0"]), _lib.ptr(out["angle_k"]), _lib.ptr(out["angle_t0"]),
                _stream(self.device)),
            "martini_param_grads",
        )
        return out


class MartiniLangevinIntegrator(_MdIntegrator):

    KB = 0.0083144626
    _prefix = "mythos_martini_langevin"

    def __init__(self, system: MartiniSystem, dt, kT, gamma, mass=None, seed=0):
        self.system = system
        self._lib = system._lib
        mptr = None
        if mass is not None:
            mass = np.ascontiguousarray(mass, dtype=np.float64)
            if mass.shape != (system.n,):
                raise ValueError(f"mass must have shape ({system.n},)")
            mptr = mass.ctypes.data_as(_lib.c_double_p)
        self._h = self._lib.mythos_martini_langevin_create(system._h, float(dt), float(kT), float(gamma), mptr, int(seed))
        if not self._h:
            raise _lib.MythosHipError(f"mythos_martini_langevin_create: {_lib.last_error()}")

    def set_neighbor_policy(self, skin: float, every: int) -> None:
        _lib.check(self._lib.mythos_martini_langevin_set_neighbor_policy(self._h, float(skin), int(every)), "set_neighbor_policy")

    def set_inner_list(self, margin: float, every: int) -> None:
        _lib.check(self._lib.mythos_martini_langevin_set_inner_list(self._h, float(margin), int(every)), "set_inner_list")

    def init_velocities(self) -> torch.Tensor:
        v = torch.empty((self.system.n, 3), dtype=self.system.dtype, device=self.system.device)
        _lib.check(self._lib.mythos_martini_langevin_init_velocities(self._h, _lib.ptr(v), _stream(self.system.device)), "init_velocities")
        return v

    def _check_state(self, pos, vel):
        s = self.system
        for t, name in ((pos, "pos"), (vel, "vel")):
            if t.device != s.device or t.dtype != s.dtype or tuple(t.shape) != (s.n, 3) or not t.is_contiguous():
                raise ValueError(f"{name} must be a contiguous {s.dtype} tensor of shape ({s.n}, 3) on {s.device}")

    def _rows(self, n_steps: int, save_every: int, want_energy: bool):
        s = self.system
        ns = n_steps // save_every if save_every > 0 else 0
        traj = torch.empty((ns, s.n, 3), dtype=s.dtype, device=s.device) if ns else None
        et = torch.zeros((ns, 4), dtype=torch.float64, device=s.device) if (ns and want_energy) else None
        return traj, et

    def run(self, pos, vel, box, n_steps: int, save_every: int = 0, want_energy: bool = True):
        s = self.system
        self._check_state(pos, vel)
        box = np.ascontiguousarray(np.asarray(box, dtype=np.float64).reshape(3))
        traj, et = self._rows(n_steps, save_every, want_energy)
        rc = self._lib.mythos_martini_langevin_run(
            self._h, _lib.ptr(pos), _lib.ptr(vel), box.ctypes.data_as(_lib.c_double_p), int(n_steps), int(save_every),
            _lib.ptr(traj), _lib.ptr(et), _stream(s.device))
        _touched(pos, vel)
        _lib.check(rc, "martini_langevin_run")
        return traj, et

    def load(self, pos, vel, box) -> None:
        self._check_state(pos, vel)
        box = np.ascontiguousarray(np.asarray(box, dtype=np.float64).reshape(3))
        _lib.check(self._lib.mythos_martini_langevin_load(self._h, _lib.ptr(pos), _lib.ptr(vel), box.ctypes.data_as(_lib.c_double_p),
                                                          _stream(self.system.device)), "martini_langevin_load")

    def advance(self, n_steps: int, save_every: int = 0, want_energy: bool = True):
        traj, et = self._rows(n_steps, save_every, want_energy)
        _lib.check(self._lib.mythos_martini_langevin_advance(self._h, int(n_steps), int(save_every), _lib.ptr(traj), _lib.ptr(et),
                                                             _stream(self.system.device)), "martini_langevin_advance")
        return traj, et

    def store(self, pos, vel) -> None:
        self._check_state(pos, vel)
        rc = self._lib.mythos_martini_langevin_store(self._h, _lib.ptr(pos), _lib.ptr(vel), _stream(self.system.device))
        _touched(pos, vel)
        _lib.check(rc, "martini_langevin_store")

    def rows(self, pruned: bool = False):
        stride = C.c_int(0)
        which = 1 if pruned else 0
        _lib.check(self._lib.mythos_martini_langevin_get_rows(self._h, which, None, None, C.byref(stride)), "get_rows")
        rows = np.empty((self.system.n, stride.value), dtype=np.int32)
        lens = np.empty(self.system.n, dtype=np.int32)
        _lib.check(self._lib.mythos_martini_langevin_get_rows(self._h, which, rows.ctypes.data_as(C.POINTER(C.c_int32)),
                                                              lens.ctypes.data_as(C.POINTER(C.c_int32)), C.byref(stride)), "get_rows")
        return rows, lens

    def neighbor_stats(self) -> tuple[int, float]:
        mx, mean = C.c_int(0), C.c_double(0.0)
        _lib.check(self._lib.mythos_martini_langevin_neighbor_stats(self._h, C.byref(mx), C.byref(mean)), "neighbor_stats")
        return mx.value, mean.value
```

Baseline: 69790 steps/s.

## Add dual-range pruned inner neighbour list for Langevin MD steps

Builds the outer Verlet list with a larger skin (skin plus margin), then periodically prunes it into a tighter inner list with a smaller margin that the MD step kernel iterates over. The step kernel's displacement check uses the inner margin and inner reference positions. Full rebuilds happen less often while each step touches fewer pair entries. The cost is an extra prune kernel every few steps, a larger outer list, and more state. It is enabled by default when the lane count is the default and rebuild_every is at least 20.

Result: slower. 68350 steps/s (-2.1%).

```diff
diff --git a/include/mythos_hip.h b/include/mythos_hip.h
--- a/include/mythos_hip.h
+++ b/include/mythos_hip.h
@@ -76,6 +76,11 @@
 
 int mythos_langevin_set_neighbor_policy(mythos_sim_t* sim, double r_cut, double skin, int every);
 
+int mythos_langevin_set_inner_list(mythos_sim_t* sim, double margin, int every);
+int mythos_langevin_get_inner_list(const mythos_sim_t* sim, double* margin, int* every);
+int mythos_langevin_get_rows(const mythos_sim_t* sim, int which, int32_t* rows, int32_t* row_len, int32_t* row_close,
+                             int* stride);
+
 int mythos_langevin_init_momenta(mythos_sim_t* sim, void* p_lin, void* p_ang, mythos_stream_t stream);
 
 int mythos_langevin_run(mythos_sim_t* sim, void* center, void* quat, void* p_lin, void* p_ang, int n_steps,
@@ -115,7 +120,8 @@
   MYTHOS_DEBUG_MD_DENSE = 4,
   MYTHOS_DEBUG_MD_ITEMS_BIG = 5,
   MYTHOS_DEBUG_MD_LANES = 6,
-  MYTHOS_DEBUG_KEYS = 7
+  MYTHOS_DEBUG_MD_INNER = 7,
+  MYTHOS_DEBUG_KEYS = 8
 };
 int mythos_debug_set(int key, int64_t value);
 int64_t mythos_debug_get(int key);
diff --git a/mythos_amd/_lib.py b/mythos_amd/_lib.py
--- a/mythos_amd/_lib.py
+++ b/mythos_amd/_lib.py
@@ -61,6 +61,9 @@
         "mythos_langevin_create": (V, [V, C.c_double, C.c_double, C.c_double, C.c_double, C.c_double, c_double_p, C.c_uint64]),
         "mythos_langevin_destroy": (None, [V]),
         "mythos_langevin_set_neighbor_policy": (C.c_int, [V, C.c_double, C.c_double, C.c_int]),
+        "mythos_langevin_set_inner_list": (C.c_int, [V, C.c_double, C.c_int]),
+        "mythos_langevin_get_inner_list": (C.c_int, [V, c_double_p, C.POINTER(C.c_int)]),
+        "mythos_langevin_get_rows": (C.c_int, [V, C.c_int, C.POINTER(C.c_int32), C.POINTER(C.c_int32), C.POINTER(C.c_int32), C.POINTER(C.c_int)]),
         "mythos_langevin_init_momenta": (C.c_int, [V, V, V, V]),
         "mythos_langevin_run": (C.c_int, [V, V, V, V, V, C.c_int, C.c_int, V, V, V, V]),
         "mythos_langevin_load": (C.c_int, [V, V, V, V, V, V]),
@@ -146,6 +149,9 @@
     "mythos_langevin_create",
     "mythos_langevin_destroy",
     "mythos_langevin_set_neighbor_policy",
+    "mythos_langevin_set_inner_list",
+    "mythos_langevin_get_inner_list",
+    "mythos_langevin_get_rows",
     "mythos_langevin_init_momenta",
     "mythos_langevin_run",
     "mythos_langevin_load",
@@ -213,7 +219,8 @@
     raise MythosHipError(msg)
 
 
-DEBUG_KEYS = {"cell_bucket_cap": 0, "energy_list_cap": 1, "md_segment": 2, "md_overflow_at": 3, "md_dense": 4, "md_items_big": 5, "md_lanes": 6}
+DEBUG_KEYS = {"cell_bucket_cap": 0, "energy_list_cap": 1, "md_segment": 2, "md_overflow_at": 3, "md_dense": 4, "md_items_big": 5, "md_lanes": 6,
+              "md_inner": 7}
 
 
 def debug_set(key: str, value: int) -> None:
diff --git a/mythos_amd/csrc/langevin.hip b/mythos_amd/csrc/langevin.hip
--- a/mythos_amd/csrc/langevin.hip
+++ b/mythos_amd/csrc/langevin.hip
@@ -52,6 +52,8 @@
   if (s->d_chunk_order) (void)hipFree(s->d_chunk_order);
   if (s->d_chunk_keys) (void)hipFree(s->d_chunk_keys);
   if (s->d_epart) (void)hipFree(s->d_epart);
+  for (void* u : {(void*)s->inner.d_rows, (void*)s->inner.d_len, s->inner.ref_pos, s->inner.ref_off, s->inner.ref_a1})
+    if (u) (void)hipFree(u);
   md_run_destroy(*s);
   delete s;
 }
@@ -66,6 +68,56 @@
   s->rebuild_every = every;
   s->list_fitted = false;
   s->list_valid = false;
+  return MYTHOS_OK;
+}
+
+int mythos_langevin_set_inner_list(mythos_sim_t* s, double margin, int every) {
+  if (!s || !(margin == margin)) {
+    set_error("mythos_langevin_set_inner_list: invalid argument");
+    return MYTHOS_ERR_INVALID_ARGUMENT;
+  }
+  s->inner_asked = true;
+  s->want_margin = margin;
+  s->want_every = every;
+  s->list_fitted = false;
+  s->list_valid = false;
+  return MYTHOS_OK;
+}
+
+int mythos_langevin_get_inner_list(const mythos_sim_t* s, double* margin, int* every) {
+  if (!s) {
+    set_error("mythos_langevin_get_inner_list: invalid argument");
+    return MYTHOS_ERR_INVALID_ARGUMENT;
+  }
+  if (margin) *margin = s->in_margin;
+  if (every) *every = s->in_every;
+  return MYTHOS_OK;
+}
+
+int mythos_langevin_get_rows(const mythos_sim_t* s, int which, int32_t* rows, int32_t* row_len, int32_t* row_close, int* stride) {
+  if (!s || (which != 0 && which != 1)) {
+    set_error("mythos_langevin_get_rows: invalid argument");
+    return MYTHOS_ERR_INVALID_ARGUMENT;
+  }
+  const mythos_system* sys = s->sys;
+  if (stride) *stride = sys->list.stride;
+  if (!rows && !row_len && !row_close) return MYTHOS_OK;
+  const bool have = which == 0 ? (sys->nbrs_set && sys->list.d_rows != nullptr)
+                               : (s->list_valid && s->in_every > 0 && s->inner.d_rows != nullptr && s->inner.stride == sys->list.stride);
+  if (!have) {
+    set_error(which == 0 ? "mythos_langevin_get_rows: no list has been built"
+                         : "mythos_langevin_get_rows: no inner rows (switched off, or no step taken since the setting)");
+    return MYTHOS_ERR_NOT_READY;
+  }
+  MYTHOS_HIP_TRY(hipSetDevice(sys->device));
+  MYTHOS_HIP_TRY(hipDeviceSynchronize());
+  const int* d_rows = which == 0 ? sys->list.d_rows : s->inner.d_rows;
+  const int* d_len = which == 0 ? sys->d_row_len : s->inner.d_len;
+  const int* d_close = which == 0 ? row_close_of(sys) : s->inner.d_close;
+  const size_t n = (size_t)sys->n;
+  if (rows) MYTHOS_HIP_TRY(hipMemcpy(rows, d_rows, n * sys->list.stride * sizeof(int), hipMemcpyDeviceToHost));
+  if (row_len) MYTHOS_HIP_TRY(hipMemcpy(row_len, d_len, n * sizeof(int), hipMemcpyDeviceToHost));
+  if (row_close) MYTHOS_HIP_TRY(hipMemcpy(row_close, d_close, n * sizeof(int), hipMemcpyDeviceToHost));
   return MYTHOS_OK;
 }
 
diff --git a/mythos_amd/csrc/langevin_core.inc b/mythos_amd/csrc/langevin_core.inc
--- a/mythos_amd/csrc/langevin_core.inc
+++ b/mythos_amd/csrc/langevin_core.inc
@@ -977,6 +977,12 @@
   int param_epoch = 0;
   int lanes = kMdG;
   int chunk_cap = 0;
+  mythos::InnerRows inner;
+  bool inner_asked = false;
+  double want_margin = 0;
+  int want_every = 0;
+  double in_margin = 0;
+  int in_every = 0;
   int* d_chunk_order = nullptr;
   unsigned long long* d_chunk_keys = nullptr;
   double* d_epart = nullptr;
@@ -1001,7 +1007,8 @@
     K.inv_inertia[k] = R(1.0 / s->inertia[k]);
     K.c2_r[k] = R(std::sqrt(s->kT * (1.0 - c1r * c1r) * s->inertia[k]));
   }
-  K.skin_half_sq = R(s->rebuild_every > 0 ? 0.25 * s->skin * s->skin : -1.0);
+  const double room = s->in_every > 0 ? s->in_margin : s->skin;
+  K.skin_half_sq = R(s->rebuild_every > 0 ? 0.25 * room * room : -1.0);
   return K;
 }
 
@@ -1059,6 +1066,41 @@
   (void)hipDeviceGetAttribute(&cus, hipDeviceAttributeMultiprocessorCount, sys->device);
   const int grid16 = (sys->n + 15) / 16;
   return 2 * grid16 <= 3 * cus ? 16 : 8;
+}
+
+static void md_inner_resolve(mythos_sim* sim) {
+  double margin = 0;
+  int every = 0;
+  if (sim->rebuild_every > 0 && debug_value(MYTHOS_DEBUG_MD_INNER) != 1) {
+    if (sim->inner_asked)
+      margin = sim->want_margin, every = sim->want_every;
+    else if (sim->lanes == kMdG && sim->rebuild_every >= 20)
+      margin = sim->skin / 3.0, every = sim->rebuild_every / 5;
+  }
+  const bool on = margin > 0 && margin < sim->skin && every >= 1;
+  sim->in_margin = on ? margin : 0.0;
+  sim->in_every = on ? every : 0;
+}
+
+template <typename R>
+static int md_inner_reserve(mythos_sim* sim) {
+  InnerRows& in = sim->inner;
+  const mythos_system* sys = sim->sys;
+  const size_t n = (size_t)sys->n, v4 = sizeof(typename Vec4T<R>::type) * n;
+  if (!in.d_len) {
+    MYTHOS_HIP_TRY(hipMalloc((void**)&in.d_len, 2 * n * sizeof(int)));
+    in.d_close = in.d_len + n;
+    MYTHOS_HIP_TRY(hipMalloc(&in.ref_pos, v4));
+    MYTHOS_HIP_TRY(hipMalloc(&in.ref_off, v4));
+    MYTHOS_HIP_TRY(hipMalloc(&in.ref_a1, v4));
+  }
+  if (!in.d_rows || in.stride != sys->list.stride) {
+    if (in.d_rows) (void)hipFree(in.d_rows);
+    in.d_rows = nullptr, in.stride = 0;
+    MYTHOS_HIP_TRY(hipMalloc((void**)&in.d_rows, n * sys->list.stride * sizeof(int)));
+    in.stride = sys->list.stride;
+  }
+  return 0;
 }
 
 template <typename R, int MODEL>
@@ -1114,7 +1156,7 @@
   const int prio_on = (sizeof(R) == 8 && grid > 3 * sim_cus) ? 0 : 1;
   const R* Pdev = device_params_of<R>(sys);
   const BoxT<R> box = make_box<R>(sys);
-  const LangevinConst<R> K = make_const<R>(sim);
+  LangevinConst<R> K = make_const<R>(sim);
   const MdCut<R> cut = make_cut<R>(sys);
   const Frame<R> fr[2] = {frame_of<R>(sim, 0), frame_of<R>(sim, 1)};
   if (sim->param_epoch != sys->param_epoch) {
@@ -1138,15 +1180,19 @@
     const R kick_close = R(row.kick_close);
     R* tc = ((save || row.save_next) && traj_center) ? traj_center + (size_t)row.sidx * n * 3 : nullptr;
     R* tq = ((save || row.save_next) && traj_quat) ? traj_quat + (size_t)row.sidx * n * 4 : nullptr;
-    const V4* ref = (const V4*)sys->d_ref_pos;
-    const V4* ref_off = (const V4*)sys->d_ref_off;
-    const V4* ref_a1 = (const V4*)sys->d_ref_a1;
+    const bool in_on = sim->in_every > 0;
+    const int* w_rows = in_on ? sim->inner.d_rows : sys->list.d_rows;
+    const int* w_len = in_on ? sim->inner.d_len : sys->d_row_len;
+    const int* w_close = in_on ? sim->inner.d_close : row_close_of(sys);
+    const V4* ref = (const V4*)(in_on ? sim->inner.ref_pos : sys->d_ref_pos);
+    const V4* ref_off = (const V4*)(in_on ? sim->inner.ref_off : sys->d_ref_off);
+    const V4* ref_a1 = (const V4*)(in_on ? sim->inner.ref_a1 : sys->d_ref_a1);
     auto launch_pseq = [&](auto save_tag, auto items_tag, hipEvent_t ea, hipEvent_t eb) {
       constexpr bool SV = decltype(save_tag)::value;
       constexpr int IT = decltype(items_tag)::value;
       auto go = [&](auto lanes_tag) {
         hipExtLaunchKernelGGL((md_step_kernel<R, MODEL, SV, IT, true, false, decltype(lanes_tag)::value>), dim3(grid), dim3(kMdBlock), 0, st, ea, eb, 0,
-                              Pdev, box, K, cut, n, fr[cur], fr[cur ^ 1], sys->list.d_rows, sys->d_row_len, row_close_of(sys),
+                              Pdev, box, K, cut, n, fr[cur], fr[cur ^ 1], w_rows, w_len, w_close,
                               sys->list.stride, sys->extra_bonds ? 1 : 0, kick_close, row.do_step, sim->seed, (uint64_t)(sim->step + k), ref,
                               ref_off, ref_a1, sim->d_flags, tc, tq, sim->d_epart, sim->d_chunk_order, halt_words, k, 0, prio_on, pseq);
       };
@@ -1157,7 +1203,7 @@
       constexpr int IT = decltype(items_tag)::value;
       auto go = [&](auto dense_tag, auto lanes_tag) {
         hipExtLaunchKernelGGL((md_step_kernel<R, MODEL, SV, IT, false, decltype(dense_tag)::value, decltype(lanes_tag)::value>), dim3(grid), dim3(kMdBlock), 0, st, ea, eb, 0,
-                              Pdev, box, K, cut, n, fr[cur], fr[cur ^ 1], sys->list.d_rows, sys->d_row_len, row_close_of(sys),
+                              Pdev, box, K, cut, n, fr[cur], fr[cur ^ 1], w_rows, w_len, w_close,
                               sys->list.stride, sys->extra_bonds ? 1 : 0, kick_close, row.do_step, sim->seed, (uint64_t)(sim->step + k), ref,
                               ref_off, ref_a1, sim->d_flags, tc, tq, sim->d_epart, sim->d_chunk_order, halt_words, k, 0, prio_on, PseqView<R>{});
       };
@@ -1192,13 +1238,24 @@
       hipLaunchKernelGGL(reduce_trace_kernel<kTraceWidth>, dim3(1), dim3(256), 0, st, sim->d_epart, blocks,
                          e_trace + (size_t)row.sidx * kTraceWidth);
   };
+  auto settle_inner = [&]() {
+    md_inner_resolve(sim);
+    K = make_const<R>(sim);
+  };
   auto rebuild = [&](int buf) -> int {
     if ((++sim->builds & 63) == 0)
       if (int rc = update_chunk_order<R>(sim, fr[buf].p0, blocks, st)) return rc;
-    return rows_build_device(sys, fr[buf].p0, true, sim->r_cut, sim->skin, fr[buf].p3, fr[buf].p1, true, st);
+    settle_inner();
+    return rows_build_device(sys, fr[buf].p0, true, sim->r_cut, sim->skin + sim->in_margin, fr[buf].p3, fr[buf].p1, true, st);
   };
   auto rebuild_until_fit = [&](int buf) -> int {
-    return rows_build_until_fit(sys, fr[buf].p0, true, sim->r_cut, sim->skin, fr[buf].p3, fr[buf].p1, true, true, st);
+    settle_inner();
+    return rows_build_until_fit(sys, fr[buf].p0, true, sim->r_cut, sim->skin + sim->in_margin, fr[buf].p3, fr[buf].p1, true, true, st);
+  };
+  auto prune = [&](int buf) -> int {
+    if (sim->in_every <= 0) return 0;
+    if (int rc = md_inner_reserve<R>(sim)) return rc;
+    return rows_prune_device(sys, sim->inner, fr[buf].p0, fr[buf].p3, fr[buf].p1, sim->r_cut, sim->in_margin, sim->skin, st);
   };
   auto on_abort = [&]() -> int {
     if (!sim->items_big) {
@@ -1218,9 +1275,13 @@
   d.dynamic_list = dynamic_list;
   d.halt_words = halt_words;
   d.row_stride = &sys->list.stride;
+  d.inner_every = &sim->in_every;
+  if (sim->inner_asked && sim->want_margin > 0 && sim->want_every >= 1)
+    d.give_up_hint = ", or the margin of the inner rows (" + std::to_string(sim->want_margin) + ") for one prune launch in " +
+                     std::to_string(sim->want_every) + " steps";
   d.skin = sim->skin;
   d.st = st;
-  return md_drive(*sim, d, launch_step, rebuild, rebuild_until_fit, on_abort);
+  return md_drive(*sim, d, launch_step, rebuild, rebuild_until_fit, on_abort, prune);
 }
 
 template <typename R>
diff --git a/mythos_amd/csrc/martini_md.hip b/mythos_amd/csrc/martini_md.hip
--- a/mythos_amd/csrc/martini_md.hip
+++ b/mythos_amd/csrc/martini_md.hip
@@ -626,7 +626,8 @@
         if (int rc = list_build_until_fit(sim->list, n, build, true, "mythos_martini_langevin_run: neighbour build", st)) return rc;
         return ensure_inner();
       },
-      [] { return 0; });
+      [] { return 0; },
+      [](int) { return 0; });
 }
 
 template <typename R>
diff --git a/mythos_amd/csrc/md_driver.h b/mythos_amd/csrc/md_driver.h
--- a/mythos_amd/csrc/md_driver.h
+++ b/mythos_amd/csrc/md_driver.h
@@ -90,6 +90,7 @@
   bool dynamic_list;
   int* halt_words;
   const int* row_stride;
+  const int* inner_every = nullptr;
   double skin;
   std::string give_up_hint;
   hipStream_t st;
@@ -106,9 +107,9 @@
   hipEvent_t ea, eb;
 };
 
-template <class Launch, class Rebuild, class RebuildUntilFit, class OnAbort>
+template <class Launch, class Rebuild, class RebuildUntilFit, class OnAbort, class Prune>
 static int md_drive(MdRun& run, const MdDrive& d, Launch&& launch, Rebuild&& rebuild, RebuildUntilFit&& rebuild_until_fit,
-                    OnAbort&& on_abort) {
+                    OnAbort&& on_abort, Prune&& prune) {
   const bool closes = d.close || (d.energy_rows && d.n_steps > 0 && d.n_steps % d.save_every == 0);
   const int n_launch = closes ? d.n_steps + 1 : d.n_steps;
   if (n_launch == 0) return MYTHOS_OK;
@@ -120,8 +121,10 @@
     if (!run.list_fitted) {
       if (int rc = rebuild_until_fit(cur0)) return rc;
       run.list_fitted = true;
+      if (int rc = prune(cur0)) return rc;
     } else if (!run.list_valid) {
       if (int rc = rebuild(cur0)) return rc;
+      if (int rc = prune(cur0)) return rc;
     } else {
       built_at = -run.since_build;
     }
@@ -169,6 +172,9 @@
           debug_clear(MYTHOS_DEBUG_MD_OVERFLOW_AT);
           MYTHOS_HIP_TRY(hipMemsetD32Async((hipDeviceptr_t)d.halt_words, *d.row_stride + 1, 1, st));
         }
+        if (int rc = prune(cur)) return fail(k, rc);
+      } else if (d.dynamic_list && d.inner_every && *d.inner_every > 0 && k > built_at && (k - built_at) % *d.inner_every == 0) {
+        if (int rc = prune(cur)) return fail(k, rc);
       }
       row.kick_close = (k == 0 && !was_open) ? 0.0f : 0.5f;
       row.do_step = last ? 0 : 1;
@@ -217,6 +223,7 @@
     if (d.dynamic_list) {
       if (int rc = rebuild_until_fit(cur)) return fail(ran, rc);
       built_at = k;
+      if (int rc = prune(cur)) return fail(ran, rc);
     }
   }
   run.last_recoveries = recoveries;
diff --git a/mythos_amd/csrc/mythos_internal.h b/mythos_amd/csrc/mythos_internal.h
--- a/mythos_amd/csrc/mythos_internal.h
+++ b/mythos_amd/csrc/mythos_internal.h
@@ -60,6 +60,14 @@
   int cell_bucket_cap;
   int cell_phase = 0;
   explicit VerletRows(int bucket_cap) : cell_bucket_cap(bucket_cap) {}
+};
+
+struct InnerRows {
+  int* d_rows = nullptr;
+  int* d_len = nullptr;
+  int* d_close = nullptr;
+  void *ref_pos = nullptr, *ref_off = nullptr, *ref_a1 = nullptr;
+  int stride = 0;
 };
 
 }
@@ -177,5 +185,7 @@
 int rows_build_until_fit(mythos_system* sys, const void* center, bool center_is_vec4, double r_cut, double skin,
                          const void* backbone_offsets, const void* base_vectors, bool write_refs, bool headroom,
                          hipStream_t stream);
+int rows_prune_device(mythos_system* sys, const InnerRows& in, const void* p0, const void* p3, const void* p1, double r_cut,
+                      double margin, double skin, hipStream_t stream);
 
 }
diff --git a/mythos_amd/csrc/neighbors.hip b/mythos_amd/csrc/neighbors.hip
--- a/mythos_amd/csrc/neighbors.hip
+++ b/mythos_amd/csrc/neighbors.hip
@@ -47,35 +47,39 @@
   R g_ba, g_st;
 };
 
+struct PairClass {
+  bool close, far;
+};
+template <typename R>
+__device__ __forceinline__ R norm2_fma(R x, R y, R z) {
+  return fma(x, x, fma(y, y, z * z));
+}
 template <typename R, class A>
-__device__ __forceinline__ bool far_in_range_v(const SiteCrit<R>& sc, const A& oi, const A& oj, const V3<R>& d) {
-  const V3<R> e{d.x + oj[0] - oi[0], d.y + oj[1] - oi[1], d.z + oj[2] - oi[2]};
-  return dot(e, e) < sc.rbb2;
-}
-template <typename R>
-__device__ __forceinline__ bool far_in_range(const SiteCrit<R>& sc, int i, int j, const V3<R>& d) {
-  if (!sc.off) return true;
-  return far_in_range_v(sc, sc.off + 4 * i, sc.off + 4 * j, d);
-}
-
-template <typename R, class A>
-__device__ __forceinline__ bool site_close_v(const SiteCrit<R>& sc, const A& ai, const A& oi, const A& aj, const A& oj, const V3<R>& d) {
-  const V3<R> da{aj[0] - ai[0], aj[1] - ai[1], aj[2] - ai[2]};
-  V3<R> e = d;
-  axpy(e, sc.g_ba, da);
-  if (dot(e, e) < sc.rbase2) return true;
-  e = d;
-  axpy(e, sc.g_st, da);
-  if (dot(e, e) < sc.rstack2) return true;
-  e = V3<R>{d.x + sc.g_ba * aj[0] - oi[0], d.y + sc.g_ba * aj[1] - oi[1], d.z + sc.g_ba * aj[2] - oi[2]};
-  if (dot(e, e) < sc.rkb2) return true;
-  e = V3<R>{d.x + oj[0] - sc.g_ba * ai[0], d.y + oj[1] - sc.g_ba * ai[1], d.z + oj[2] - sc.g_ba * ai[2]};
-  return dot(e, e) < sc.rkb2;
-}
-template <typename R>
-__device__ __forceinline__ bool site_close(const SiteCrit<R>& sc, int i, int j, const V3<R>& d) {
-  if (!sc.off) return true;
-  return site_close_v(sc, sc.a1 + 4 * i, sc.off + 4 * i, sc.a1 + 4 * j, sc.off + 4 * j, d);
+__device__ __forceinline__ PairClass classify_pair(const SiteCrit<R>& sc, const BoxT<R>& box, R rc2, R rcl2, R xi, R yi, R zi,
+                                                   R xj, R yj, R zj, const A& ai, const A& oi, const A& aj, const A& oj) {
+  R dx = xj - xi, dy = yj - yi, dz = zj - zi;
+  if (box.on) {
+    dx = fma(-box.l[0], m_rint(dx * box.il[0]), dx);
+    dy = fma(-box.l[1], m_rint(dy * box.il[1]), dy);
+    dz = fma(-box.l[2], m_rint(dz * box.il[2]), dz);
+  }
+  PairClass c{false, false};
+  const R r2 = norm2_fma(dx, dy, dz);
+  if (!(r2 < rc2)) return c;
+  if (!sc.off) {
+    c.close = r2 < rcl2;
+    c.far = !c.close;
+    return c;
+  }
+  if (r2 < rcl2) {
+    const R ax = aj[0] - ai[0], ay = aj[1] - ai[1], az = aj[2] - ai[2];
+    c.close = norm2_fma(fma(sc.g_ba, ax, dx), fma(sc.g_ba, ay, dy), fma(sc.g_ba, az, dz)) < sc.rbase2 ||
+              norm2_fma(fma(sc.g_st, ax, dx), fma(sc.g_st, ay, dy), fma(sc.g_st, az, dz)) < sc.rstack2 ||
+              norm2_fma(fma(sc.g_ba, aj[0], dx) - oi[0], fma(sc.g_ba, aj[1], dy) - oi[1], fma(sc.g_ba, aj[2], dz) - oi[2]) < sc.rkb2 ||
+              norm2_fma(fma(-sc.g_ba, ai[0], dx + oj[0]), fma(-sc.g_ba, ai[1], dy + oj[1]), fma(-sc.g_ba, ai[2], dz + oj[2])) < sc.rkb2;
+  }
+  if (!c.close) c.far = norm2_fma(dx + oj[0] - oi[0], dy + oj[1] - oi[1], dz + oj[2] - oi[2]) < sc.rbb2;
+  return c;
 }
 
 template <typename R, bool VEC4>
@@ -101,13 +105,11 @@
       const int j = j0 + lane;
       bool hit = false;
       if (j < n && j != i && j != bp.x && j != bp.y && j != bp.z && j != bp.w) {
-        V3<R> d{pos[S * j] - ci.x, pos[S * j + 1] - ci.y, pos[S * j + 2] - ci.z};
-        d = min_image(d, box);
-        const R r2 = dot(d, d);
-        if (r2 < rc2) {
-          const bool cl = r2 < rcl2 && site_close(sc, i, j, d);
-          hit = (pass == 0) ? cl : (!cl && far_in_range(sc, i, j, d));
-        }
+        const R* z = pos;
+        const PairClass pc = classify_pair(sc, box, rc2, rcl2, ci.x, ci.y, ci.z, pos[S * j], pos[S * j + 1], pos[S * j + 2],
+                                           sc.off ? sc.a1 + 4 * (size_t)i : z, sc.off ? sc.off + 4 * (size_t)i : z,
+                                           sc.off ? sc.a1 + 4 * (size_t)j : z, sc.off ? sc.off + 4 * (size_t)j : z);
+        hit = (pass == 0) ? pc.close : pc.far;
       }
       const unsigned long long m = __ballot(hit);
       if (hit) {
@@ -218,18 +220,12 @@
           mine = jx == s_c[grp][lo][0] && jy == s_c[grp][lo][1] && jz == s_c[grp][lo][2];
         }
         if (mine) {
-          V3<R> d{xj - ci.x, yj - ci.y, zj - ci.z};
-          d = min_image(d, box);
-          const R r2 = dot(d, d);
-          if (r2 < rc2) {
-            if (site_stride) {
-              hit_c = r2 < rcl2 && site_close_v(sc, ai, oi, aj, oj, d);
-              hit_f = !hit_c && far_in_range_v(sc, oi, oj, d);
-            } else {
-              hit_c = r2 < rcl2 && site_close(sc, i, j, d);
-              hit_f = !hit_c && far_in_range(sc, i, j, d);
-            }
+          if (!site_stride && sc.off) {
+#pragma unroll
+            for (int a = 0; a < 3; ++a) oj[a] = sc.off[4 * (size_t)j + a], aj[a] = sc.a1[4 * (size_t)j + a];
           }
+          const PairClass pc = classify_pair(sc, box, rc2, rcl2, ci.x, ci.y, ci.z, xj, yj, zj, ai, oi, aj, oj);
+          hit_c = pc.close, hit_f = pc.far;
         }
       }
     }
@@ -276,14 +272,8 @@
 }
 
 template <typename R>
-static int build_cells_typed(mythos_system* sys, const R* pos, bool vec4, double rl, double skin, const R* off,
-                             const R* a1, bool write_refs, hipStream_t st) {
-  R* ref_pos = write_refs ? (R*)sys->d_ref_pos : nullptr;
-  R* ref_off = write_refs ? (R*)sys->d_ref_off : nullptr;
-  R* ref_a1 = write_refs ? (R*)sys->d_ref_a1 : nullptr;
-  const int n = sys->n;
-  const double rcl = sys->params_set ? std::min(rl, oxdna_close_range(sys) + skin) : rl;
-  int* d_close = row_close_of(sys);
+static SiteCrit<R> site_criteria(const mythos_system* sys, double rl, double skin, const R* off, const R* a1, double& rcl) {
+  rcl = sys->params_set ? std::min(rl, oxdna_close_range(sys) + skin) : rl;
   double rbb = rl;
   if (off && sys->params_set) {
     rbb = oxdna_param_max(sys, NEXC_BACKBONE_RC);
@@ -304,6 +294,91 @@
     sc.g_ba = R(0.5 * (Pd[GEO_BASE] + Pr[GEO_BASE]));
     sc.g_st = R(0.5 * (Pd[GEO_STACK] + Pr[GEO_STACK]));
   }
+  return sc;
+}
+
+template <typename R, int G>
+__global__ __launch_bounds__(256) void prune_rows_kernel(int n, const typename Vec4T<R>::type* __restrict__ p0,
+                                                          const typename Vec4T<R>::type* __restrict__ p3,
+                                                          const typename Vec4T<R>::type* __restrict__ p1, const BoxT<R> box,
+                                                          R rc2, R rcl2, const SiteCrit<R> sc, const int* __restrict__ rows,
+                                                          const int* __restrict__ row_len, int row_stride,
+                                                          const typename Vec4T<R>::type* __restrict__ ref_pos,
+                                                          const typename Vec4T<R>::type* __restrict__ ref_off,
+                                                          const typename Vec4T<R>::type* __restrict__ ref_a1, R outer_half_sq,
+                                                          R gb_dna, R gb_rna, int* __restrict__ halt, int* __restrict__ rows_in,
+                                                          int* __restrict__ len_in, int* __restrict__ close_in,
+                                                          typename Vec4T<R>::type* __restrict__ in_pos,
+                                                          typename Vec4T<R>::type* __restrict__ in_off,
+                                                          typename Vec4T<R>::type* __restrict__ in_a1) {
+  using V4 = typename Vec4T<R>::type;
+  constexpr int NG = 256 / G;
+  extern __shared__ int s_seg_all[];
+  const int grp = threadIdx.x / G, l = threadIdx.x % G;
+  const int gshift = (threadIdx.x & 63) & ~(G - 1);
+  const int i = blockIdx.x * NG + grp;
+  if (i >= n) return;
+  int* s_close = s_seg_all + (size_t)grp * 2 * row_stride;
+  int* s_far = s_close + row_stride;
+  const V4 c = p0[i], o = p3[i], a = p1[i];
+  const R oi[3] = {o.x, o.y, o.z}, ai[3] = {a.x, a.y, a.z};
+  const int* row = rows + (size_t)i * row_stride;
+  const int len = min(row_len[i], row_stride);
+  int out_c = 0, out_f = 0;
+  constexpr unsigned int kGroupMask = (G == 32) ? 0xffffffffu : ((1u << G) - 1u);
+  for (int s0 = ROW_BONDED_SLOTS; s0 < len; s0 += G) {
+    const int s = s0 + l;
+    bool hit_c = false, hit_f = false;
+    int e = 0;
+    if (s < len) {
+      e = row[s];
+      const int j = e & ROW_INDEX_MASK;
+      const V4 cj = p0[j], ov = p3[j], av = p1[j];
+      const R oj[3] = {ov.x, ov.y, ov.z}, aj[3] = {av.x, av.y, av.z};
+      const PairClass pc = classify_pair(sc, box, rc2, rcl2, c.x, c.y, c.z, cj.x, cj.y, cj.z, ai, oi, aj, oj);
+      hit_c = pc.close, hit_f = pc.far;
+    }
+    const unsigned int mc = (unsigned int)(__ballot(hit_c) >> gshift) & kGroupMask;
+    const unsigned int mf = (unsigned int)(__ballot(hit_f) >> gshift) & kGroupMask;
+    const unsigned int below = (1u << l) - 1u;
+    if (hit_c) s_close[out_c + __popc(mc & below)] = e;
+    if (hit_f) s_far[out_f + __popc(mf & below)] = e;
+    out_c += __popc(mc);
+    out_f += __popc(mf);
+  }
+  __builtin_amdgcn_wave_barrier();
+  __builtin_amdgcn_fence(__ATOMIC_ACQ_REL, "wavefront");
+  const int n_close = ROW_BONDED_SLOTS + out_c;
+  int* dst = rows_in + (size_t)i * row_stride;
+  group_sort_to_row<G>(s_close, out_c, dst + ROW_BONDED_SLOTS, row_stride - ROW_BONDED_SLOTS, l);
+  group_sort_to_row<G>(s_far, out_f, dst + n_close, row_stride - n_close, l);
+  if (l == 0) {
+#pragma unroll
+    for (int k = 0; k < ROW_BONDED_SLOTS; ++k) dst[k] = row[k];
+    len_in[i] = n_close + out_f;
+    close_in[i] = n_close;
+    in_pos[i] = c, in_off[i] = o, in_a1[i] = a;
+    const V4 r0 = ref_pos[i], f0 = ref_off[i], a0 = ref_a1[i];
+    const R dx = c.x - r0.x, dy = c.y - r0.y, dz = c.z - r0.z;
+    const R bx = dx + (o.x - f0.x), by = dy + (o.y - f0.y), bz = dz + (o.z - f0.z);
+    const R gb = ((((int)c.w) >> 3) & 1) ? gb_rna : gb_dna;
+    const R sx = dx + gb * (a.x - a0.x), sy = dy + gb * (a.y - a0.y), sz = dz + gb * (a.z - a0.z);
+    if (dx * dx + dy * dy + dz * dz > outer_half_sq || bx * bx + by * by + bz * bz > outer_half_sq ||
+        sx * sx + sy * sy + sz * sz > outer_half_sq)
+      atomicMax(halt, 1);
+  }
+}
+
+template <typename R>
+static int build_cells_typed(mythos_system* sys, const R* pos, bool vec4, double rl, double skin, const R* off,
+                             const R* a1, bool write_refs, hipStream_t st) {
+  R* ref_pos = write_refs ? (R*)sys->d_ref_pos : nullptr;
+  R* ref_off = write_refs ? (R*)sys->d_ref_off : nullptr;
+  R* ref_a1 = write_refs ? (R*)sys->d_ref_a1 : nullptr;
+  const int n = sys->n;
+  double rcl;
+  const SiteCrit<R> sc = site_criteria<R>(sys, rl, skin, off, a1, rcl);
+  int* d_close = row_close_of(sys);
   VerletRows& L = sys->list;
   CellGrid<R> g;
   const bool cells = cell_grid(g, n, rl, sys->has_box ? sys->box : nullptr);
@@ -365,6 +440,38 @@
   return 0;
 }
 
+template <typename R>
+static int prune_typed(mythos_system* sys, const InnerRows& in, const void* p0, const void* p3, const void* p1, double r_cut,
+                       double margin, double skin, hipStream_t st) {
+  using V4 = typename Vec4T<R>::type;
+  const int n = sys->n;
+  const double rl = r_cut + margin;
+  double rcl;
+  const SiteCrit<R> sc = site_criteria<R>(sys, rl, margin, (const R*)p3, (const R*)p1, rcl);
+  const double* Pd = oxdna_param_set(sys, 0);
+  const double* Pr = oxdna_param_set(sys, sys->param_sets() == 1 ? 0 : 1);
+  constexpr int kPerBlock = 256 / kRowG;
+  const VerletRows& L = sys->list;
+  const size_t lds = (size_t)kPerBlock * 2 * L.stride * sizeof(int);
+  hipLaunchKernelGGL((prune_rows_kernel<R, kRowG>), dim3((n + kPerBlock - 1) / kPerBlock), dim3(256), lds, st, n, (const V4*)p0,
+                     (const V4*)p3, (const V4*)p1, make_box<R>(sys), R(rl * rl), R(rcl * rcl), sc, (const int*)L.d_rows,
+                     (const int*)sys->d_row_len, L.stride, (const V4*)sys->d_ref_pos, (const V4*)sys->d_ref_off,
+                     (const V4*)sys->d_ref_a1, R(0.25 * skin * skin), R(Pd[GEO_BASE]), R(Pr[GEO_BASE]), L.d_overflow, in.d_rows,
+                     in.d_len, in.d_close, (V4*)in.ref_pos, (V4*)in.ref_off, (V4*)in.ref_a1);
+  MYTHOS_HIP_TRY(hipGetLastError());
+  return 0;
+}
+
+int rows_prune_device(mythos_system* sys, const InnerRows& in, const void* p0, const void* p3, const void* p1, double r_cut,
+                      double margin, double skin, hipStream_t stream) {
+  if (!in.d_rows || in.stride != sys->list.stride || !sys->params_set) {
+    set_error("inner rows: not allocated at the stride of the Verlet rows");
+    return MYTHOS_ERR_NOT_READY;
+  }
+  return sys->dtype == MYTHOS_F32 ? prune_typed<float>(sys, in, p0, p3, p1, r_cut, margin, skin, stream)
+                                  : prune_typed<double>(sys, in, p0, p3, p1, r_cut, margin, skin, stream);
+}
+
 int rows_build_until_fit(mythos_system* sys, const void* center, bool center_is_vec4, double r_cut, double skin,
                          const void* backbone_offsets, const void* base_vectors, bool write_refs, bool headroom,
                          hipStream_t stream) {
diff --git a/mythos_amd/hip_system.py b/mythos_amd/hip_system.py
--- a/mythos_amd/hip_system.py
+++ b/mythos_amd/hip_system.py
@@ -268,6 +268,24 @@
             "set_neighbor_policy",
         )
 
+    def set_inner_list(self, margin: float, every: int) -> None:
+        _lib.check(self._lib.mythos_langevin_set_inner_list(self._h, float(margin), int(every)), "set_inner_list")
+
+    def inner_list(self):
+        m, e = C.c_double(0.0), C.c_int(0)
+        _lib.check(self._lib.mythos_langevin_get_inner_list(self._h, C.byref(m), C.byref(e)), "get_inner_list")
+        return (m.value, e.value) if e.value > 0 else None
+
+    def rows(self, inner: bool = False):
+        n, which, stride = self.system.n, 1 if inner else 0, C.c_int(0)
+        _lib.check(self._lib.mythos_langevin_get_rows(self._h, which, None, None, None, C.byref(stride)), "get_rows")
+        rows = np.empty((n, stride.value), dtype=np.int32)
+        lens, close = np.empty(n, dtype=np.int32), np.empty(n, dtype=np.int32)
+        p32 = C.POINTER(C.c_int32)
+        _lib.check(self._lib.mythos_langevin_get_rows(self._h, which, rows.ctypes.data_as(p32), lens.ctypes.data_as(p32),
+                                                      close.ctypes.data_as(p32), C.byref(stride)), "get_rows")
+        return rows, lens, close
+
     def set_unfused(self, on: bool = True) -> None:
         _lib.check(self._lib.mythos_langevin_set_option(self._h, 0, 1 if on else 0), "set_option(unfused)")
 
```
